# AssafSinger94/dino-tracker

Hardware: NVIDIA H100
Metric: query-points/sec (854x476, T=50) (higher is better)
Workload: dtype f32

## Files before the change

dino_tracker_b200/_lib.py:

```python
import ctypes
import os
import struct
import warnings
from ctypes import POINTER, Structure, c_char_p, c_float, c_int, c_size_t, c_ulonglong, c_void_p

import torch

from . import build as _build

_LIB = None


class Geom(Structure):
    _fields_ = [("H", c_int), ("W", c_int), ("patch", c_int), ("stride", c_int), ("radius", c_int),
                ("h", c_int), ("w", c_int)]


class HeadWeights(Structure):
    _fields_ = [("w1", c_float * 9 * 16), ("b1", c_float * 16), ("w2", c_float * 9 * 16), ("b2", c_float)]


class Features(Structure):
    _fields_ = [("tpc", c_void_p), ("norms", c_void_p), ("hi", c_void_p), ("lo", c_void_p), ("T", c_int), ("C", c_int),
                ("q8", c_void_p), ("q_fac", c_void_p), ("q_rho", c_void_p), ("hilo", c_void_p)]


class VitConfig(Structure):
    _fields_ = [("depth", c_int), ("dim", c_int), ("heads", c_int), ("tap_layer", c_int), ("patch", c_int), ("stride", c_int),
                ("attn_materialized", c_int), ("gemm_f16", c_int), ("gemm_pair", c_int), ("swiglu_hidden", c_int),
                ("facet", c_int)]


class VitWeights(Structure):
    _fields_ = [("patch_w", c_void_p), ("patch_b", c_void_p), ("cls_pos", c_void_p), ("pos", c_void_p),
                ("blocks", POINTER(c_void_p))]


class FlowVideo(Structure):
    _fields_ = [("fwd", c_void_p), ("bwd", c_void_p), ("T", c_int), ("H", c_int), ("W", c_int)]


RAFT_NCONV = 45


class RaftWeights(Structure):
    _fields_ = [("w_hi", c_void_p * RAFT_NCONV), ("w_lo", c_void_p * RAFT_NCONV), ("bias", c_void_p * RAFT_NCONV),
                ("scale", c_float * RAFT_NCONV)]


class DinotrkError(RuntimeError):
    pass


_P = c_void_p
SIGNATURES = {
    "dinotrk_version": (c_int, []),
    "dinotrk_last_error": (c_char_p, []),
    "dinotrk_launch_count": (c_ulonglong, []),
    "dinotrk_make_geom": (c_int, [c_int, c_int, c_int, c_int, c_int, POINTER(Geom)]),
    "dinotrk_pack_features": (c_int, [_P, _P, _P, c_int, c_int, c_int, _P]),
    "dinotrk_unpack_features": (c_int, [_P, _P, c_int, c_int, c_int, _P]),
    "dinotrk_token_norms": (c_int, [_P, _P, c_int, c_int, c_int, _P]),
    "dinotrk_sample_descriptors": (c_int, [_P, c_int, c_int, POINTER(Geom), _P, c_int, _P, c_int, c_int, _P, _P, _P]),
    "dinotrk_split_fp16": (c_int, [_P, _P, _P, c_size_t, _P]),
    "dinotrk_split_hilo": (c_int, [_P, _P, c_size_t, c_int, _P]),
    "dinotrk_quantise_s8": (c_int, [_P, _P, c_size_t, c_int, c_int, _P, _P, _P, _P, _P]),
    "dinotrk_split_range": (c_int, [_P, c_size_t, _P, c_size_t, _P, _P]),
    "dinotrk_split_faithful": (c_int, [c_float, c_float, c_int]),
    "dinotrk_corr_track_workspace_bytes": (c_size_t, [c_int, c_int, c_int, POINTER(Geom)]),
    "dinotrk_corr_track": (c_int, [POINTER(Features), POINTER(Geom), POINTER(HeadWeights), _P, _P, _P, _P, _P, _P,
                                   c_int, c_int, c_int, _P, _P, c_int, c_int, _P, c_size_t, _P]),
    "dinotrk_corr_maps_workspace_bytes": (c_size_t, [c_int, c_int, c_int]),
    "dinotrk_map_stride": (c_int, [POINTER(Geom)]),
    "dinotrk_corr_maps": (c_int, [POINTER(Features), POINTER(Geom), _P, _P, _P, _P, _P, _P, c_int, c_int, c_int,
                                  _P, _P, c_size_t, _P]),
    "dinotrk_head": (c_int, [_P, c_int, POINTER(Geom), POINTER(HeadWeights), _P, _P, c_int, c_int, _P, _P, _P]),
    "dinotrk_sample_backward": (c_int, [c_int, c_int, POINTER(Geom), _P, c_int, _P, c_int, c_int, _P, _P, _P]),
    "dinotrk_track_backward_workspace_bytes": (c_size_t, [c_int, c_int, POINTER(Geom)]),
    "dinotrk_track_backward": (c_int, [POINTER(Features), POINTER(Geom), POINTER(HeadWeights), _P, _P, c_int, _P, _P, _P, _P, _P,
                                       _P, c_int, _P, _P, _P, c_size_t, _P]),
    "dinotrk_infer_workspace_bytes": (c_size_t, [c_int, c_int, POINTER(Geom), c_int, c_int]),
    "dinotrk_infer_set_overlap": (c_int, [c_int]),
    "dinotrk_infer_set_path": (c_int, [c_int]),
    "dinotrk_xw_head_set_window_only": (c_int, [c_int]),
    "dinotrk_infer_set_coarse": (c_int, [c_int]),
    "dinotrk_infer_last_stats": (c_int, [POINTER(ctypes.c_longlong), c_int]),
    "dinotrk_infer_max_chunks": (c_size_t, [c_int, c_int, c_int]),
    "dinotrk_xw_coarse_keys_workspace_bytes": (c_size_t, [c_int, c_int, POINTER(Geom)]),
    "dinotrk_xw_coarse_keys": (c_int, [POINTER(Features), POINTER(Geom), _P, c_int, _P, _P, _P, _P, c_int, _P, _P, _P, c_size_t,
                                       _P]),
    "dinotrk_xw_coarse_keys_i8": (c_int, [POINTER(Features), POINTER(Geom), _P, _P, _P, c_int, _P, _P, _P, c_int, _P, _P, _P, _P,
                                          c_size_t, _P]),
    "dinotrk_xw_box_gemm": (c_int, [POINTER(Features), POINTER(Geom), _P, _P, c_int, _P, _P, _P, _P, c_int, c_int, _P, _P]),
    "dinotrk_infer_plan": (c_int, [c_int, c_int, c_int, _P, c_int, _P, _P, c_int, _P]),
    "dinotrk_infer_anchor_gcap": (c_int, [c_int, c_int]),
    "dinotrk_infer_plan_anchors": (c_int, [c_int, c_int, _P, _P, _P, c_int, c_int, _P, _P, c_int, _P]),
    "dinotrk_infer": (c_int, [POINTER(Features), POINTER(Geom), POINTER(HeadWeights), _P, c_int, c_float, c_float,
                              c_int, c_int, c_int, c_int, _P, _P, _P, _P, _P, c_size_t, _P]),
    "dinotrk_traj_cos_sims": (c_int, [_P, c_int, c_int, POINTER(Geom), _P, _P, c_int, _P, _P, c_size_t, _P]),
    "dinotrk_delta_workspace_bytes": (c_size_t, [c_int, c_int, c_int, POINTER(c_int)]),
    "dinotrk_delta_refine": (c_int, [_P, c_int, c_int, c_int, POINTER(c_int), POINTER(c_void_p), POINTER(c_void_p), _P,
                                     _P, _P, c_int, c_int, _P, _P, _P, c_size_t, _P]),
    "dinotrk_vit_workspace_bytes": (c_size_t, [POINTER(VitConfig), POINTER(Geom), c_int]),
    "dinotrk_vit_attention": (c_int, [_P, _P, _P, c_int, c_int, c_int, c_int, _P, _P]),
    "dinotrk_vit_attention_f16": (c_int, [_P, _P, _P, c_int, c_int, c_int, c_int, _P, _P]),
    "dinotrk_vit_stage": (c_int, [c_int, POINTER(VitConfig), POINTER(Geom), c_int, _P, _P, _P, _P, _P, _P, _P, _P, c_size_t,
                                  _P]),
    "dinotrk_vit_forward": (c_int, [_P, c_int, POINTER(Geom), POINTER(VitConfig), POINTER(VitWeights), _P, _P, c_size_t, _P]),
    "dinotrk_best_buddies_workspace_bytes": (c_size_t, [c_int, c_int]),
    "dinotrk_best_buddies_pairs": (c_int, [POINTER(Features), POINTER(Geom), _P, _P, c_int, _P, _P, _P, c_size_t, _P]),
    "dinotrk_bb_mutual": (c_int, [_P, _P, c_int, c_int, _P, _P]),
    "dinotrk_bb_nms": (c_int, [_P, c_int, POINTER(Geom), c_float, c_float, c_int, _P, _P, _P]),
    "dinotrk_profile_classes": (c_int, []),
    "dinotrk_profile_class_name": (c_char_p, [c_int]),
    "dinotrk_profile_enable": (None, [c_int]),
    "dinotrk_profile_collect": (c_int, [POINTER(ctypes.c_double), POINTER(c_ulonglong), c_int]),
    "dinotrk_delta_refine_allgather": (c_int, [_P, c_int, c_int, c_int, POINTER(c_int), POINTER(c_void_p), POINTER(c_void_p), _P,
                                               _P, _P, c_int, c_int, _P, _P, _P, c_size_t, POINTER(c_void_p), c_int, c_size_t, _P]),
    "dinotrk_delta_refine_tc": (c_int, [_P, c_int, c_int, c_int, POINTER(c_int), POINTER(c_void_p), POINTER(c_void_p),
                                        POINTER(c_void_p), _P, _P, _P, c_int, c_int, _P, _P, _P, c_size_t, POINTER(c_void_p),
                                        c_int, c_size_t, _P]),
    "dinotrk_delta_train_saved_bytes": (c_size_t, [c_int, c_int, c_int, POINTER(c_int)]),
    "dinotrk_delta_train_forward_workspace_bytes": (c_size_t, [c_int, c_int, c_int, POINTER(c_int)]),
    "dinotrk_delta_train_backward_workspace_bytes": (c_size_t, [c_int, c_int, c_int, POINTER(c_int)]),
    "dinotrk_delta_train_forward": (c_int, [_P, c_int, c_int, c_int, POINTER(c_int), POINTER(c_void_p), POINTER(c_void_p),
                                            POINTER(c_void_p), POINTER(c_void_p), POINTER(c_void_p), POINTER(c_void_p),
                                            POINTER(c_void_p), c_int, c_float, c_float, _P, _P, c_int, c_int, _P, _P, c_size_t,
                                            _P, c_size_t, _P]),
    "dinotrk_delta_train_backward": (c_int, [_P, c_int, c_int, c_int, POINTER(c_int), POINTER(c_void_p), POINTER(c_void_p),
                                             POINTER(c_void_p), POINTER(c_void_p), c_int, _P, _P, c_int, c_int, _P, _P, c_size_t,
                                             POINTER(c_void_p), POINTER(c_void_p), POINTER(c_void_p), POINTER(c_void_p), _P,
                                             c_size_t, _P]),
    "dinotrk_peer_alloc": (c_int, [c_size_t, POINTER(c_void_p), ctypes.c_char_p]),
    "dinotrk_peer_open": (c_int, [ctypes.c_char_p, POINTER(c_void_p)]),
    "dinotrk_peer_close": (c_int, [_P]),
    "dinotrk_peer_free": (c_int, [_P]),
    "dinotrk_occlusion": (c_int, [_P, _P, _P, c_int, c_int, c_float, c_float, _P, _P]),
    "dinotrk_flow_masks": (c_int, [POINTER(FlowVideo), c_float, _P, _P]),
    "dinotrk_traj_workspace_bytes": (c_size_t, [c_int, c_int, c_int]),
    "dinotrk_traj_chain": (c_int, [POINTER(FlowVideo), _P, c_int, c_float, c_int, _P, _P, c_float, _P, _P, c_size_t, _P]),
    "dinotrk_traj_emit": (c_int, [POINTER(FlowVideo), c_int, _P, _P, c_size_t, _P]),
    "dinotrk_traj_nearest_workspace_bytes": (c_size_t, [c_int, c_int, c_int, c_int]),
    "dinotrk_traj_nearest": (c_int, [_P, c_int, c_int, c_int, c_int, c_float, c_float, _P, _P, c_size_t, _P]),
    "dinotrk_of_filter": (c_int, [_P, c_int, c_int, _P, c_int, c_int, c_int, _P, _P, _P, _P, _P, c_int, c_int, _P, _P]),
    "dinotrk_pca_workspace_bytes": (c_size_t, [ctypes.c_longlong, c_int, c_int]),
    "dinotrk_pca_stats": (c_int, [_P, ctypes.c_longlong, c_int, c_int, _P, _P, _P, c_size_t, _P]),
    "dinotrk_pca_power": (c_int, [_P, ctypes.c_longlong, c_int, c_int, _P, _P, _P, _P, _P, _P, c_size_t, _P]),
    "dinotrk_fg_mask": (c_int, [_P, c_int, c_int, c_int, c_int, c_int, _P, _P, c_float, c_int, c_int, _P, _P, _P, _P, c_size_t,
                                _P]),
    "dinotrk_mask_upsample": (c_int, [_P, c_int, c_int, c_int, c_int, c_int, _P, _P]),
    "dinotrk_traj_split_workspace_bytes": (c_size_t, [c_int]),
    "dinotrk_traj_split_count": (c_int, [_P, c_int, c_int, _P, c_int, c_int, c_int, POINTER(c_int), _P, c_size_t, _P]),
    "dinotrk_traj_split_emit": (c_int, [_P, c_int, c_int, _P, _P, _P, c_size_t, _P]),
    "dinotrk_bb_contrastive_cos_stride": (c_int, [c_int]),
    "dinotrk_bb_contrastive_forward_workspace_bytes": (c_size_t, [c_int, c_int, c_int, c_int, c_int]),
    "dinotrk_bb_contrastive_forward": (c_int, [_P, c_int, c_int, c_int, _P, _P, c_int, _P, _P, _P, _P, c_int, c_float, _P, _P,
                                               _P, c_size_t, _P]),
    "dinotrk_bb_contrastive_backward_workspace_bytes": (c_size_t, [c_int, c_int, c_int, c_int, _P, _P, _P, _P, c_int]),
    "dinotrk_bb_contrastive_backward": (c_int, [_P, c_int, c_int, c_int, _P, _P, c_int, _P, _P, _P, _P, c_int, c_float, _P, _P,
                                                _P, _P, _P, _P, _P, _P, _P, _P, c_size_t, _P]),
    "dinotrk_sampler_workspace_bytes": (c_size_t, [c_int]),
    "dinotrk_sampler_prepare_count": (c_int, [_P, c_int, c_int, POINTER(c_int), _P, c_size_t, _P]),
    "dinotrk_sampler_prepare_emit": (c_int, [_P, c_int, c_int, _P, _P, _P, c_size_t, _P]),
    "dinotrk_sampler_count": (c_int, [_P, c_int, c_int, _P, c_int, POINTER(c_int), _P, c_size_t, _P]),
    "dinotrk_sampler_select": (c_int, [_P, c_int, c_int, _P, c_int, _P, c_int, _P, _P, _P, c_size_t, _P]),
    "dinotrk_sampler_gather": (c_int, [_P, c_int, _P, _P, c_int, _P, _P, _P]),
    "dinotrk_randperm_prefix": (c_int, [_P, c_size_t, ctypes.c_int64, ctypes.c_int64, _P]),
    "dinotrk_cycle_mask_workspace_bytes": (c_size_t, [c_int, c_int]),
    "dinotrk_cycle_mask_scan": (c_int, [_P, c_int, c_int, _P, _P, _P, c_size_t, _P]),
    "dinotrk_cycle_select": (c_int, [_P, c_int, c_int, c_int, _P, _P, c_int, _P, _P, _P]),
    "dinotrk_cycle_unnorm": (c_int, [_P, _P, c_int, c_int, c_int, _P, _P, _P]),
    "dinotrk_cycle_keep": (c_int, [_P, _P, c_int, c_int, c_int, c_float, _P, _P, _P, _P]),
    "dinotrk_emb_reg_workspace_bytes": (c_size_t, [c_int, c_int]),
    "dinotrk_emb_reg_forward": (c_int, [_P, _P, c_int, c_int, c_int, _P, _P, _P, c_size_t, _P]),
    "dinotrk_emb_reg_backward": (c_int, [_P, _P, c_int, c_int, c_int, _P, _P, _P, _P, _P]),
    "dinotrk_raft_encode_workspace_bytes": (c_size_t, [c_int, c_int]),
    "dinotrk_raft_encode": (c_int, [_P, c_int, c_int, c_int, c_int, POINTER(RaftWeights), _P, _P, _P, c_size_t, _P]),
    "dinotrk_raft_flow_workspace_bytes": (c_size_t, [c_int, c_int, c_int]),
    "dinotrk_raft_flow": (c_int, [_P, _P, _P, _P, c_int, c_int, c_int, c_int, POINTER(c_int), c_int, c_int,
                                  POINTER(RaftWeights), _P, _P, c_size_t, _P]),
}


def lib_path():
    return _build.LIB_PATH


def load(build_if_missing=True):
    global _LIB
    if _LIB is not None:
        return _LIB
    path = lib_path()
    if not os.path.exists(path):
        if not build_if_missing:
            raise DinotrkError(f"{path} is missing: run `python -c 'import __graft_entry__ as g; g.build()'`")
        _build.build()
    lib = ctypes.CDLL(path)
    for name, (res, args) in SIGNATURES.items():
        fn = getattr(lib, name)
        fn.restype = res
        fn.argtypes = args
    if lib.dinotrk_version() < 100:
        raise DinotrkError("libdinotrk.so is older than the Python binding")
    _LIB = lib
    return lib


def check(rc, what="dinotrk"):
    if rc != 0:
        raise DinotrkError(f"{what} failed ({rc}): {load().dinotrk_last_error().decode()}")


def ptr(t):
    if t is None:
        return None
    assert t.is_cuda and t.is_contiguous(), "device pointers must come from contiguous CUDA tensors"
    return c_void_p(t.data_ptr())


def stream_ptr(device=None):
    return c_void_p(torch.cuda.current_stream(device).cuda_stream)


def on_device(fn):
    import functools

    @functools.wraps(fn)
    def wrapped(self, *a, **kw):
        with torch.cuda.device(self._dev):
            return fn(self, *a, **kw)
    return wrapped


def require_cuda(device):
    if not torch.cuda.is_available():
        raise DinotrkError("dino_tracker_b200 needs a CUDA device (sm_90a); there is no CPU fallback")
    dev = torch.device(device)
    if dev.type != "cuda":
        raise DinotrkError(f"dino_tracker_b200 runs on CUDA only, got device={device!r}")
    return dev


def make_features(tpc, norms, hi=None, lo=None, quant=None, hilo=None):
    f = Features()
    f.tpc, f.norms = tpc.data_ptr(), norms.data_ptr()
    f.hi = hi.data_ptr() if hi is not None else None
    f.lo = lo.data_ptr() if lo is not None else None
    f.T, f.C = tpc.shape[0], tpc.shape[2]
    if quant is not None:
        f.q8, f.q_fac, f.q_rho = (t.data_ptr() for t in quant)
    f.hilo = hilo.data_ptr() if hilo is not None else None
    f._keep = (tpc, norms, hi, lo, quant, hilo)
    return f


def quantise_s8(x, norms, rows_per_group, stream):
    C = x.shape[-1]
    rows = x.numel() // C
    q = torch.empty(x.shape, device=x.device, dtype=torch.int8)
    fac = torch.empty(x.shape[:-1], device=x.device, dtype=torch.float32)
    rho = torch.empty(x.shape[:-1], device=x.device, dtype=torch.float32)
    rho_max = torch.empty(-(-rows // rows_per_group), device=x.device, dtype=torch.float32)
    check(load().dinotrk_quantise_s8(ptr(x), ptr(norms), rows, C, rows_per_group, ptr(q), ptr(fac), ptr(rho), ptr(rho_max),
                                     stream), "quantise_s8")
    return q, fac, rho, rho_max


S8_MAX_C = 2048


def quantise_features(tpc, norms, stream):
    T, P, C = tpc.shape
    if C % 16 or C > S8_MAX_C:
        return None
    q, fac, _, rho_f = quantise_s8(tpc, norms, P, stream)
    return q, fac, rho_f


def split_range(tpc, norms, stream):
    lib = load()
    rng = torch.empty(2, device=tpc.device, dtype=torch.float32)
    check(lib.dinotrk_split_range(ptr(tpc), tpc.numel(), ptr(norms), norms.numel(), ptr(rng), stream), "split_range")
    max_abs, min_norm = rng.tolist()
    return max_abs, min_norm, bool(lib.dinotrk_split_faithful(max_abs, min_norm, tpc.shape[-1]))


def split_fp16(x, stream):
    hi = torch.empty(x.shape, device=x.device, dtype=torch.float16)
    lo = torch.empty(x.shape, device=x.device, dtype=torch.float16)
    check(load().dinotrk_split_fp16(ptr(x), ptr(hi), ptr(lo), x.numel(), stream), "split_fp16")
    return hi, lo


def split_hilo(x, stream):
    C = x.shape[-1]
    hilo = torch.empty(x.shape[:-1] + (64 * (-(-C // 32)),), device=x.device, dtype=torch.float16)
    check(load().dinotrk_split_hilo(ptr(x), ptr(hilo), x.numel() // C, C, stream), "split_hilo")
    return hilo


def split_features(tpc, norms, stream):
    max_abs, min_norm, ok = split_range(tpc, norms, stream)
    if not ok:
        warnings.warn(f"feature video outside the fp16 split's faithful range (max |x| = {max_abs:.3g}, smallest token "
                      f"norm = {min_norm:.3g}, C = {tpc.shape[-1]}): its contractions run on the exact-fp32 path",
                      RuntimeWarning, stacklevel=3)
        return None, None
    return split_fp16(tpc, stream)


def make_geom(H, W, patch=14, stride=7, radius=35):
    g = Geom()
    check(load().dinotrk_make_geom(H, W, patch, stride, radius, ctypes.byref(g)), "make_geom")
    return g


def profile_enable(on=True):
    load().dinotrk_profile_enable(1 if on else 0)


def profile_collect():
    lib = load()
    n = lib.dinotrk_profile_classes()
    ms = (ctypes.c_double * n)()
    cnt = (c_ulonglong * n)()
    check(lib.dinotrk_profile_collect(ms, cnt, n), "profile_collect")
    return {lib.dinotrk_profile_class_name(i).decode(): (ms[i], int(cnt[i])) for i in range(n) if cnt[i]}


def infer_stats():
    a = (ctypes.c_longlong * 10)()
    check(load().dinotrk_infer_last_stats(a, 10), "infer_last_stats")
    rho_f = struct.unpack("<f", struct.pack("<I", int(a[7])))[0]
    return {"anchor_maps": int(a[0]), "exact_window": int(a[1]), "full_map": int(a[2]), "pipeline": "exact-window" if a[3] else "full-map",
            "full_map_by_certificate": int(a[4]), "contraction": "fp16x3" if a[5] else "fp32",
            "coarse": "int8" if a[6] else "fp16", "coarse_rho_f": rho_f, "desc_in_place": int(a[8]), "desc_gathered": int(a[9])}


def launch_count():
    return int(load().dinotrk_launch_count())
```

dino_tracker_b200/csrc/inference.cu:

```cuda
#include <algorithm>
#include <vector>

#include "common.cuh"
#include "corr.cuh"
#include "head.cuh"
#include "sample.cuh"
#include "xwin.cuh"

namespace dtk {

constexpr int TC2_BM_ROWS = 256;

__global__ void sample_query_kernel(const float* __restrict__ tpc, int T, int C, int P, int h, int w, PointAffine pa,
                                    const float* __restrict__ qp, float* __restrict__ desc, float* __restrict__ dnorm) {
  int n = blockIdx.x;
  float x = __fadd_rn(__fmul_rn(pa.aw, qp[n * 3 + 0]), pa.bw);
  float y = __fadd_rn(__fmul_rn(pa.ah, qp[n * 3 + 1]), pa.bh);
  int tq = (int)qp[n * 3 + 2];
  tq = min(max(tq, 0), T - 1);
  TriCorners c = tri_setup(x, y, 0.f, 2, h, w);
  sample_point(tpc, C, P, c, tq, -1, desc + (size_t)n * C, dnorm + n);
}

__global__ void index_traj_kernel(const int* __restrict__ grp_frame, const int* __restrict__ grp_row0,
                                  const int* __restrict__ grp_map0, int n_groups, int n_maps, int T,
                                  int* __restrict__ out_index, float* __restrict__ traj) {
  int j = blockIdx.x * blockDim.x + threadIdx.x;
  if (j >= n_maps) return;
  const int lo = last_le(n_groups, j, grp_map0);
  int n = grp_row0[lo] + (j - grp_map0[lo]);
  int t = grp_frame[lo];
  out_index[j] = n * T + t;
  traj[((size_t)n * T + t) * 3 + 2] = (float)t;
}

__global__ void traj_cos_kernel(const float* __restrict__ tpc, int T, int C, int P, int h, int w, PointAffine pa,
                                const float* __restrict__ traj, const float* __restrict__ qp,
                                float* __restrict__ cos_out) {
  extern __shared__ __align__(16) float sm[];
  __shared__ float nrm[2];
  __shared__ float red[SAMPLE_THREADS / 32];
  const int n = blockIdx.y, i = blockIdx.x;
  int tq = (int)qp[n * 3 + 2];
  tq = min(max(tq, 0), T - 1);
  for (int which = 0; which < 2; ++which) {
    const float* pt = traj + ((size_t)n * T + (which == 0 ? tq : i)) * 3;
    float x = __fadd_rn(__fmul_rn(pa.aw, pt[0]), pa.bw);
    float y = __fadd_rn(__fmul_rn(pa.ah, pt[1]), pa.bh);
    TriCorners c = tri_setup(x, y, pt[2], T, h, w);
    sample_point(tpc, C, P, c, c.z0, c.z1, sm + which * C, nrm + which);
    __syncthreads();
  }
  const float nq = fmaxf(nrm[0], 1e-8f), ni = fmaxf(nrm[1], 1e-8f);
  float acc = 0.f;
  for (int c = threadIdx.x; c < C; c += SAMPLE_THREADS) acc = fmaf(__fdiv_rn(sm[c], nq), __fdiv_rn(sm[C + c], ni), acc);
  acc = warp_sum(acc);
  if ((threadIdx.x & 31) == 0) red[threadIdx.x >> 5] = acc;
  __syncthreads();
  if (threadIdx.x == 0) {
    float s = 0.f;
    for (int k = 0; k < SAMPLE_THREADS / 32; ++k) s += red[k];
    cos_out[(size_t)n * T + i] = s;
  }
}

constexpr int ANCHOR_LIST_THREADS = 256;
__global__ void __launch_bounds__(ANCHOR_LIST_THREADS)
anchor_lists_kernel(const float* __restrict__ cos_sims, int N, int T, float th, int* __restrict__ cnt,
                    int* __restrict__ qlist) {
  const int a = blockIdx.x;
  int base = 0;
  for (int n0 = 0; n0 < N; n0 += ANCHOR_LIST_THREADS) {
    const int n = n0 + threadIdx.x;
    const bool v = n < N && cos_sims[(size_t)n * T + a] >= th;
    int total;
    const int rank = block_rank<ANCHOR_LIST_THREADS>(v, &total);
    if (v) qlist[(size_t)a * N + base + rank] = n;
    base += total;
    __syncthreads();
  }
  if (threadIdx.x == 0) cnt[a] = base;
}

struct AnchorItem { int a, slot, i, n; };
__device__ __forceinline__ AnchorItem anchor_item(int j, int lo, int T, const int* __restrict__ qlist, int N,
                                                  const int* __restrict__ grp_frame, const int* __restrict__ grp_map0,
                                                  const int* __restrict__ grp_item0) {
  AnchorItem it;
  it.a = grp_frame[lo];
  const int uu = grp_item0[lo] + (j - grp_map0[lo]);
  it.slot = uu / T; it.i = uu - it.slot * T;
  it.n = qlist[(size_t)it.a * N + it.slot];
  return it;
}

struct NoAnchor {};
__device__ __forceinline__ int slot_frame(int z, int i0, int a) { return z == 0 ? a : i0 + z - 1; }
__device__ __forceinline__ int slot_frame(int z, int i0, NoAnchor) { return i0 + z - 1; }
struct SetSample { TriCorners c; int f0, f1; };
template <class Anchor>
__device__ __forceinline__ SetSample frame_set_sample(const float* __restrict__ pt, int i, int T, int frame_batch, int h, int w,
                                                      const PointAffine& pa, Anchor a) {
  const int i0 = (i / frame_batch) * frame_batch, e = min(i0 + frame_batch, T);
  float x = __fadd_rn(__fmul_rn(pa.aw, pt[0]), pa.bw);
  float y = __fadd_rn(__fmul_rn(pa.ah, pt[1]), pa.bh);
  SetSample s;
  s.c = tri_setup(x, y, (float)(i - i0 + 1), e - i0 + 1, h, w);
  s.f0 = slot_frame(s.c.z0, i0, a);
  s.f1 = s.c.z1 < 0 ? -1 : slot_frame(s.c.z1, i0, a);
  return s;
}

__global__ void sample_anchor_kernel(const float* __restrict__ tpc, int T, int C, int P, int h, int w, PointAffine pa,
                                     const float* __restrict__ traj, const int* __restrict__ qlist, int N,
                                     const int* __restrict__ grp_frame, const int* __restrict__ grp_map0,
                                     const int* __restrict__ grp_item0, int n_groups, int frame_batch,
                                     float* __restrict__ desc, float* __restrict__ dnorm, int* __restrict__ out_index,
                                     __half* __restrict__ desc_hi, __half* __restrict__ desc_lo) {
  const int j = blockIdx.x;
  const AnchorItem it = anchor_item(j, last_le(n_groups, j, grp_map0), T, qlist, N, grp_frame, grp_map0, grp_item0);
  const SetSample s = frame_set_sample(traj + ((size_t)it.n * T + it.i) * 3, it.i, T, frame_batch, h, w, pa, it.a);
  sample_point(tpc, C, P, s.c, s.f0, s.f1, desc + (size_t)j * C, dnorm + j, desc_hi ? desc_hi + (size_t)j * C : nullptr,
               desc_lo ? desc_lo + (size_t)j * C : nullptr);
  if (threadIdx.x == 0) out_index[j] = (it.n * T + it.a) * T + it.i;
}

__device__ __forceinline__ float quant_desc(const __half* hi, const __half* lo, int C, const float* norm, int8_t* q, float* fac) {
  __syncthreads();
  if (threadIdx.x >= 32) return 0.f;
  const float nrm = *norm;
  return xw_quant_row([&](int k) {
    const uint2 a = *reinterpret_cast<const uint2*>(hi + k), b = *reinterpret_cast<const uint2*>(lo + k);
    const float2 a0 = __half22float2(*reinterpret_cast<const __half2*>(&a.x)), a1 = __half22float2(*reinterpret_cast<const __half2*>(&a.y));
    const float2 b0 = __half22float2(*reinterpret_cast<const __half2*>(&b.x)), b1 = __half22float2(*reinterpret_cast<const __half2*>(&b.y));
    return make_float4(a0.x + b0.x, a0.y + b0.y, a1.x + b1.x, a1.y + b1.y);
  }, C, nrm, q, fac);
}

__global__ void sample_unique_kernel(const float* __restrict__ tpc, int T, int C, int P, int h, int w, PointAffine pa,
                                     const float* __restrict__ traj, int frame_batch, __half* __restrict__ u_hi,
                                     __half* __restrict__ u_lo, float* __restrict__ u_norm, int* __restrict__ u_flag,
                                     int8_t* __restrict__ u_q8, float* __restrict__ u_fac, float* __restrict__ u_rho) {
  const int u = blockIdx.x;
  const SetSample s = frame_set_sample(traj + (size_t)u * 3, u % T, T, frame_batch, h, w, pa, NoAnchor{});
  bool slot0 = false;
#pragma unroll
  for (int k = 0; k < 4; ++k) slot0 = slot0 || (s.c.z0 == 0 && s.c.tok[k] >= 0 && s.c.wxy[k][0] != 0.f);
  if (threadIdx.x == 0) u_flag[u] = slot0 ? 1 : 0;
  if (slot0) return;
  sample_point(tpc, C, P, s.c, s.f0, s.f1, nullptr, u_norm + u, u_hi + (size_t)u * C, u_lo + (size_t)u * C);
  if (u_q8) {
    const float r = quant_desc(u_hi + (size_t)u * C, u_lo + (size_t)u * C, C, u_norm + u, u_q8 + (size_t)u * C, u_fac + u);
    if (threadIdx.x == 0) u_rho[u] = r;
  }
}

__global__ void anchor_scalars_kernel(int T, const int* __restrict__ qlist, int N, const int* __restrict__ grp_frame,
                                      const int* __restrict__ grp_row0, const int* __restrict__ grp_map0,
                                      const int* __restrict__ grp_item0, int n_groups, int n_maps, int n_unique, int chunk_row0,
                                      const float* __restrict__ u_norm, const int* __restrict__ u_flag,
                                      const float* __restrict__ u_rho, const float* __restrict__ rho_f, float eps_slack, bool with_eps,
                                      int* __restrict__ out_index, int* __restrict__ arow, float* __restrict__ dnorm,
                                      float* __restrict__ desc_eps) {
  const int j = blockIdx.x * blockDim.x + threadIdx.x;
  if (j >= n_maps) return;
  const int lo = last_le(n_groups, j, grp_map0);
  const AnchorItem it = anchor_item(j, lo, T, qlist, N, grp_frame, grp_map0, grp_item0);
  const size_t u = (size_t)it.n * T + it.i;
  out_index[j] = (it.n * T + it.a) * T + it.i;
  const int r0 = grp_row0[lo];
  arow[j] = r0 < n_unique ? r0 + (j - grp_map0[lo]) : chunk_row0 + j;
  if (u_flag[u]) return;
  dnorm[j] = u_norm[u];
  if (with_eps) desc_eps[j] = xw_eps_s8(u_rho[u], rho_f[it.a], eps_slack);
}

__global__ void gather_anchor_kernel(const float* __restrict__ tpc, int T, int C, int P, int h, int w, PointAffine pa,
                                     const float* __restrict__ traj, const int* __restrict__ qlist, int N,
                                     const int* __restrict__ grp_frame, const int* __restrict__ grp_row0,
                                     const int* __restrict__ grp_map0, const int* __restrict__ grp_item0, int n_groups,
                                     int n_unique, int map_lo, int frame_batch, const __half* __restrict__ u_hi,
                                     const __half* __restrict__ u_lo, const int* __restrict__ u_flag,
                                     float* __restrict__ dnorm, __half* __restrict__ desc_hi,
                                     __half* __restrict__ desc_lo, const int8_t* __restrict__ u_q8,
                                     const float* __restrict__ u_fac, const float* __restrict__ rho_f, float eps_slack,
                                     int8_t* __restrict__ desc_q8, float* __restrict__ desc_fac,
                                     float* __restrict__ desc_eps) {
  const int j = map_lo + blockIdx.x;
  const int lo = last_le(n_groups, j, grp_map0);
  if (grp_row0[lo] < n_unique) return;
  const AnchorItem it = anchor_item(j, lo, T, qlist, N, grp_frame, grp_map0, grp_item0);
  const size_t u = (size_t)it.n * T + it.i;
  if (!u_flag[u]) {
    const uint4* sh = reinterpret_cast<const uint4*>(u_hi + u * C);
    const uint4* sl = reinterpret_cast<const uint4*>(u_lo + u * C);
    uint4* dh = reinterpret_cast<uint4*>(desc_hi + (size_t)j * C);
    uint4* dl = reinterpret_cast<uint4*>(desc_lo + (size_t)j * C);
    for (int k = threadIdx.x; k < C / 8; k += blockDim.x) { dh[k] = __ldg(sh + k); dl[k] = __ldg(sl + k); }
    if (desc_q8) {
      const uint4* sq = reinterpret_cast<const uint4*>(u_q8 + u * C);
      uint4* dq = reinterpret_cast<uint4*>(desc_q8 + (size_t)j * C);
      for (int k = threadIdx.x; k < C / 16; k += blockDim.x) dq[k] = __ldg(sq + k);
      if (threadIdx.x == 0) desc_fac[j] = u_fac[u];
    }
    return;
  }
  const SetSample s = frame_set_sample(traj + u * 3, it.i, T, frame_batch, h, w, pa, it.a);
  sample_point(tpc, C, P, s.c, s.f0, s.f1, nullptr, dnorm + j, desc_hi + (size_t)j * C, desc_lo + (size_t)j * C);
  if (desc_q8) {
    const float r = quant_desc(desc_hi + (size_t)j * C, desc_lo + (size_t)j * C, C, dnorm + j, desc_q8 + (size_t)j * C, desc_fac + j);
    if (threadIdx.x == 0) desc_eps[j] = xw_eps_s8(r, rho_f[it.a], eps_slack);
  }
}

constexpr int OCC_THREADS = 256;
__global__ void occlusion_kernel(const float* __restrict__ traj, const float* __restrict__ cos_sims,
                                 const float* __restrict__ anchors, int T, float anchor_th, float cos_th,
                                 uint8_t* __restrict__ occ) {
  extern __shared__ float sm[];
  float* med = sm;
  int* alist = reinterpret_cast<int*>(sm + T);
  float* ax = sm + 2 * T;
  float* ay = sm + 3 * T;
  const int lane = threadIdx.x & 31, warp = threadIdx.x >> 5, nw = OCC_THREADS / 32;
  float* col = sm + 4 * T + warp * T;
  __shared__ int M;
  __shared__ float th_s;
  const int n = blockIdx.x;
  if (threadIdx.x == 0) {
    int m = 0;
    for (int a = 0; a < T; ++a)
      if (cos_sims[(size_t)n * T + a] >= anchor_th) {
        alist[m] = a;
        ax[m] = traj[((size_t)n * T + a) * 3 + 0];
        ay[m] = traj[((size_t)n * T + a) * 3 + 1];
        ++m;
      }
    M = m;
  }
  __syncthreads();
  const int m = M, want = (m - 1) / 2;
  for (int i = warp; i < T; i += nw) {
    for (int p = lane; p < m; p += 32) {
      const float* g = anchors + (((size_t)n * T + alist[p]) * T + i) * 2;
      float dx = __fsub_rn(g[0], ax[p]), dy = __fsub_rn(g[1], ay[p]);
      col[p] = sqrtf(__fadd_rn(__fmul_rn(dx, dx), __fmul_rn(dy, dy)));
    }
    __syncwarp();
    for (int p = lane; p < m; p += 32) {
      const float dp = col[p];
      int rank = 0;
      for (int q = 0; q < m; ++q) {
        float dq = col[q];
        rank += (dq < dp) || (dq == dp && q < p);
      }
      if (rank == want) med[i] = dp;
    }
    __syncwarp();
  }
  __syncthreads();
  if (threadIdx.x == 0) {
    float th = -INFINITY;
    for (int p = 0; p < m; ++p) th = fmaxf(th, med[alist[p]]);
    th_s = th;
  }
  __syncthreads();
  for (int i = threadIdx.x; i < T; i += blockDim.x)
    occ[(size_t)n * T + i] = (m > 0 && (med[i] > th_s || cos_sims[(size_t)n * T + i] < cos_th)) ? 1 : 0;
}

struct GroupBuf {
  std::vector<int> v;
  int cap, n;
  bool overflow = false;
  explicit GroupBuf(int c) : v((size_t)5 * c), cap(c), n(0) {}
  void clear() { n = 0; }
  void push(int frame, int row0, int m, int map0, int item0) {
    if (n >= cap) { overflow = true; return; }
    v[n] = frame; v[cap + n] = row0; v[2 * cap + n] = m; v[3 * cap + n] = map0; v[4 * cap + n] = item0; ++n;
  }
};

struct ChunkMeta { int used, maxm, n_groups; bool no_thin; int n_gathered, gather_lo, gather_hi; };
constexpr int XW_INPLACE_PAD_DIV = 16;
constexpr int XW_INPLACE_MIN_ROWS = TC2_BM_ROWS - TC2_BM_ROWS / (XW_INPLACE_PAD_DIV + 1);
struct AnchorRows { const int* qlist; const unsigned char* qflag; int gather_row0, ring, ring_stride; };
static bool plan_chunks(int kind, int T, int N, const int* cnt, int ch_all, int gcap, std::vector<ChunkMeta>& metas,
                        std::vector<int>& plan_host, int align = 1, int first_cap = 0, const AnchorRows* rows = nullptr) {
  int ch = ch_all;
  metas.clear(); plan_host.clear();
  GroupBuf gb(gcap);
  int n_gathered = 0, gather_lo = 0, gather_hi = 0;
  auto commit_chunk = [&](int used) {
    bool no_thin = true;
    int maxm = 0;
    for (int k = 0; k < gb.n; ++k) {
      no_thin = no_thin && gb.v[2 * gb.cap + k] > STREAM_MAX_M;
      maxm = std::max(maxm, gb.v[2 * gb.cap + k]);
    }
    metas.push_back(ChunkMeta{used, maxm, gb.n, no_thin, n_gathered, gather_lo, gather_hi});
    plan_host.insert(plan_host.end(), gb.v.begin(), gb.v.end());
    n_gathered = gather_lo = gather_hi = 0;
  };
  auto push_span = [&](int a, int map0, int m, int item0) {
    if (!rows) { gb.push(a, map0, m, map0, item0); return; }
    const int* ql = rows->qlist + (size_t)a * N;
    const int chunk_row0 = rows->gather_row0 + (int)(metas.size() % rows->ring) * rows->ring_stride;
    const int s0 = item0 / T, s1 = (item0 + m) / T;
    int gs = -1;
    auto close_gathered = [&](int s_end) {
      if (gs < 0) return;
      const int gm = (s_end - gs) * T, gmap = map0 + (gs - s0) * T;
      gb.push(a, chunk_row0 + gmap, gm, gmap, gs * T);
      if (n_gathered == 0) gather_lo = gmap;
      n_gathered += gm; gather_hi = gmap + gm;
      gs = -1;
    };
    for (int s = s0; s < s1;) {
      const bool flagged = rows->qflag[ql[s]] != 0;
      int e = s + 1;
      while (!flagged && e < s1 && ql[e] == ql[e - 1] + 1 && !rows->qflag[ql[e]]) ++e;
      const int r = (e - s) * T, pad = (r + TC2_BM_ROWS - 1) / TC2_BM_ROWS * TC2_BM_ROWS - r;
      if (!flagged && (long long)pad * XW_INPLACE_PAD_DIV <= r) {
        close_gathered(s);
        gb.push(a, ql[s] * T, r, map0 + (s - s0) * T, s * T);
      } else if (gs < 0) {
        gs = s;
      }
      s = e;
    }
    close_gathered(s1);
  };
  if (kind == 0) {
    int t = 0, row = 0;
    while (t < T) {
      gb.clear();
      int used = 0;
      while (t < T && used < ch && gb.n < gcap) {
        int m = N - row;
        if (m > ch - used) m = ch - used;
        gb.push(t, row, m, used, 0);
        used += m; row += m;
        if (row == N) { row = 0; ++t; }
      }
      commit_chunk(used);
    }
  } else {
    int a = 0;
    long long item = 0;
    while (a < T) {
      gb.clear();
      int used = 0;
      ch = (metas.empty() && first_cap > 0 && first_cap < ch_all) ? first_cap : ch_all;
      while (a < T && used < ch && gb.n < gcap) {
        long long tot = (long long)cnt[a] * T;
        long long m = tot - item;
        if (m > ch - used) {
          m = (long long)((ch - used) / align) * align;
          if (m == 0 && used > 0) break;
          if (m == 0) m = align;
        }
        if (m > 0) {
          push_span(a, used, (int)m, (int)item);
          used += (int)m; item += m;
        }
        if (item >= tot) { item = 0; ++a; }
      }
      if (used == 0) break;
      commit_chunk(used);
    }
  }
  return !gb.overflow;
}

struct CellPlan {
  std::vector<int> v;
  std::vector<size_t> first;
  std::vector<int> tiles;
  int max_m = 0;
};
static void plan_cells(int T, int gcap, const std::vector<ChunkMeta>& metas, const std::vector<int>& plan_host, CellPlan& cp) {
  const int nb = (T + XW_MAX_CELL - 1) / XW_MAX_CELL, rb = (T + nb - 1) / nb;
  cp.v.clear(); cp.first.assign(1, 0); cp.tiles.clear(); cp.max_m = 0;
  std::vector<int> r0, mm, fr, gr, ar;
  for (size_t k = 0; k < metas.size(); ++k) {
    const int* gb = plan_host.data() + k * 5 * gcap;
    r0.clear(); mm.clear(); fr.clear(); gr.clear(); ar.clear();
    int pre = 0;
    for (int g = 0; g < metas[k].n_groups; ++g) {
      const int frame = gb[g], row0 = gb[gcap + g], m = gb[2 * gcap + g], map0 = gb[3 * gcap + g];
      cp.tiles.push_back(pre);
      pre += (m + TC2_BM_ROWS - 1) / TC2_BM_ROWS;
      for (int s0 = 0; s0 < m; s0 += T)
        for (int b = 0; b < T; b += rb) {
          const int cm = std::min(rb, T - b);
          r0.push_back(map0 + s0 + b); mm.push_back(cm); fr.push_back(frame); gr.push_back(g); ar.push_back(row0 + s0 + b);
          cp.max_m = std::max(cp.max_m, cm);
        }
    }
    for (int g = metas[k].n_groups; g <= gcap; ++g) cp.tiles.push_back(pre);
    const size_t n = r0.size();
    cp.v.insert(cp.v.end(), r0.begin(), r0.end());
    cp.v.insert(cp.v.end(), mm.begin(), mm.end());
    cp.v.insert(cp.v.end(), fr.begin(), fr.end());
    cp.v.insert(cp.v.end(), gr.begin(), gr.end());
    cp.v.insert(cp.v.end(), ar.begin(), ar.end());
    cp.first.push_back(cp.first.back() + n);
  }
}

struct InferAsync {
  cudaStream_t side;
  cudaEvent_t fork, join, sample[2], gemm[2];
};
static int g_overlap_mode = -1;
struct InferAsyncSlot { InferAsync ia; int state; };
static InferAsync* infer_async() {
  static PerDev<InferAsyncSlot> slots;
  if (g_overlap_mode == 0) return nullptr;
  InferAsyncSlot& slot = slots.get();
  InferAsync& ia = slot.ia;
  if (slot.state == 0) {
    slot.state = -1;
    if (cudaStreamCreateWithFlags(&ia.side, cudaStreamNonBlocking) != cudaSuccess) return nullptr;
    cudaEvent_t* evs[] = {&ia.fork, &ia.join, &ia.sample[0], &ia.sample[1], &ia.gemm[0], &ia.gemm[1]};
    for (cudaEvent_t* ev : evs)
      if (cudaEventCreateWithFlags(ev, cudaEventDisableTiming) != cudaSuccess) return nullptr;
    slot.state = 1;
  }
  return slot.state == 1 ? &ia : nullptr;
}

constexpr int XW_RING = 4;
constexpr int XW_PROBE_MAPS = 4096;
constexpr int INFER_A_COUNTED = 16;
constexpr int XW_CNT_A = 2 * XW_RING, XW_CNT_MINNORM = XW_CNT_A + INFER_A_COUNTED;
struct XwAsync {
  int state;
  cudaEvent_t sample[XW_RING], done[XW_RING], freed[XW_RING];
  int* host_cnt;
};
static XwAsync* xw_async() {
  static PerDev<XwAsync> slots;
  XwAsync& xa = slots.get();
  if (xa.state == 0) {
    xa.state = -1;
    for (int k = 0; k < XW_RING; ++k) {
      if (cudaEventCreateWithFlags(&xa.sample[k], cudaEventDisableTiming) != cudaSuccess) return nullptr;
      if (cudaEventCreateWithFlags(&xa.done[k], cudaEventDisableTiming) != cudaSuccess) return nullptr;
      if (cudaEventCreateWithFlags(&xa.freed[k], cudaEventDisableTiming) != cudaSuccess) return nullptr;
    }
    if (cudaHostAlloc(&xa.host_cnt, (XW_CNT_MINNORM + 4) * sizeof(int), cudaHostAllocDefault) != cudaSuccess) return nullptr;
    xa.state = 1;
  }
  return xa.state == 1 ? &xa : nullptr;
}
static int g_xw_path = -1;
static int g_xw_coarse = -1;
namespace infer_stat {
enum { anchor_maps, exact_window, full_map, pipeline, full_map_by_certificate, contraction, coarse, coarse_rho_f,
       desc_in_place, desc_gathered, count };
}
static long long g_infer_stats[infer_stat::count] = {};
constexpr int XW_S8_PROBE_QUEUE_DIV = 16;

struct AnchorChoice {
  XwAsync* xa = nullptr;
  bool xw = false;
  bool probe = false;
  bool s8 = false;

  AnchorChoice(const FeatView& fv, const dinotrk_geom& g) {
    if (fv.tensor() && disc_fits_box(g) && g_xw_path != 0) xa = xw_async();
    xw = xa != nullptr;
    probe = g_xw_path < 0;
  }
  static bool q8_rows(const FeatView& fv) { return fv.s8() && g_xw_coarse != 0 && fv.C % 16 == 0 && fv.C <= XW_S8_MAX_C; }
  void after_sync(int C, int n_counted_A, long long maps_A) {
    if (!xw) return;
    float mn;
    memcpy(&mn, xa->host_cnt + XW_CNT_MINNORM, sizeof(float));
    if (!(mn >= split_min_norm(C))) xw = false;
    if (xw && probe && n_counted_A > 0) {
      long long unc = 0;
      for (int k = 0; k < n_counted_A; ++k) unc += xa->host_cnt[XW_CNT_A + k];
      if (unc * 4 > maps_A) xw = false;
    }
  }
  int coarse_pass(const FeatView& fv, float rho_max) {
    DTK_CHECK_ARG(g_xw_coarse != 1 || !xw || fv.s8(), "infer: int8 coarse pass forced without the int8 features");
    s8 = xw && fv.s8() && g_xw_coarse != 0;
    DTK_CHECK_ARG(!s8 || (fv.C % 16 == 0 && fv.C <= XW_S8_MAX_C), "infer: int8 coarse pass needs C %% 16 == 0 and C <= %d",
                  XW_S8_MAX_C);
    if (g_xw_coarse < 0 && !(rho_max <= XW_S8_RHO_MAX)) s8 = false;
    return DINOTRK_OK;
  }
  bool probe_says_full_maps(long long by_certificate, long long queued, int maps) {
    if (by_certificate * 4 > maps) return true;
    if (s8 && g_xw_coarse < 0 && queued * XW_S8_PROBE_QUEUE_DIV > maps) s8 = false;
    return false;
  }
};

struct CorrTrackWs {
  float* maps; CorrMapsWs corr; int* hscratch;
  CorrTrackWs(Arena& ar, int total_maps, int n_groups, int C, int map_stride)
      : maps(ar.take<float>((size_t)total_maps * map_stride)), corr(ar, total_maps, n_groups, C),
        hscratch(ar.take<int>(total_maps + 1)) {}
};

struct ChunkBufs {
  float* maps; float* desc; float* norm; int* plan; float* split; int* hscratch; unsigned long long* tkeys;
  ChunkBufs() = default;
  ChunkBufs(Arena& ar, int C, int N, int P, int ms, int ch, int gcap) {
    maps = ar.take<float>((size_t)ch * ms);
    desc = ar.take<float>((size_t)ch * C);
    norm = ar.take<float>(ch);
    plan = ar.take<int>(gcap + 1);
    split = ar.take<float>(corr_tc_workspace_bytes(ch > N ? ch : N, C) / 4);
    hscratch = ar.take<int>(ch + 1);
    tkeys = ar.take<unsigned long long>((size_t)ch * cdiv(P, CORR_TILE));
  }
};

struct XwSet {
  int row0; float* norm; int* out_index; int* arow; float* eps; XwChunk xc;
  XwSet() = default;
  XwSet(Arena& ar, int row0_, float* u_norm, int P, int ch, int gcap) : row0(row0_), norm(u_norm + row0_) {
    out_index = ar.take<int>(ch);
    arow = ar.take<int>(ch);
    eps = ar.take<float>(ch);
    xc = XwChunk(ar, ch, (size_t)ch + 2, cdiv(P, XW_TILE), gcap);
  }
};

struct InferWs {
  float* descA; float* normA;
  ChunkBufs cb[2];
  int* out_index_ring[4];
  int* d_groups; int* d_cnt; int* d_qlist;
  size_t xw_rows;
  __half* u_hi; __half* u_lo; int8_t* u_q8; float* u_norm; float* u_fac; int* u_flag; float* u_rho;
  float* d_rnorms; unsigned* d_minnorm;
  XwSet xr[XW_RING];
  int cell_nb;
  int* d_cells; int* d_tiles;
  int sg_cap;
  int* d_cgrp; int* d_splan; int* d_cntA;
  InferWs(Arena& ar, int T, int C, int N, int P, int ms, int ch, int gcap, size_t max_chunks) {
    descA = ar.take<float>((size_t)N * C);
    normA = ar.take<float>(N);
    for (ChunkBufs& b : cb) b = ChunkBufs(ar, C, N, P, ms, ch, gcap);
    for (int*& r : out_index_ring) r = ar.take<int>(ch);
    d_groups = ar.take<int>(max_chunks * 5 * gcap);
    d_cnt = ar.take<int>(T);
    d_qlist = ar.take<int>((size_t)T * N);
    const int n_unique = N * T;
    xw_rows = (size_t)n_unique + (size_t)XW_RING * ch;
    u_hi = ar.take<__half>(xw_rows * C);
    u_lo = ar.take<__half>(xw_rows * C);
    u_q8 = ar.take<int8_t>(xw_rows * C);
    u_norm = ar.take<float>(xw_rows);
    u_fac = ar.take<float>(xw_rows);
    u_flag = ar.take<int>((size_t)N * T);
    u_rho = ar.take<float>((size_t)N * T);
    d_rnorms = ar.take<float>((size_t)T * P);
    d_minnorm = ar.take<unsigned>(4);
    for (int k = 0; k < XW_RING; ++k) xr[k] = XwSet(ar, n_unique + k * ch, u_norm, P, ch, gcap);
    cell_nb = (T + XW_MAX_CELL - 1) / XW_MAX_CELL;
    d_cells = ar.take<int>((size_t)N * T * cell_nb * 5 + 16);
    d_tiles = ar.take<int>(max_chunks * (gcap + 1));
    sg_cap = (int)std::min<size_t>(max_chunks * (size_t)gcap, 16384);
    d_cgrp = ar.take<int>((size_t)4 * sg_cap);
    d_splan = ar.take<int>((size_t)sg_cap + 1);
    d_cntA = ar.take<int>(64);
  }
};

struct InferCtx {
  const FeatView& fv; const dinotrk_geom& g; const dinotrk_head_weights& hw;
  InferWs& ws; cudaStream_t st;
  int T, C, N, P, ms, ch, gcap, fb;
  size_t max_chunks;
  PointAffine pa;
  std::vector<ChunkMeta> metas;
  std::vector<int> plan_host;
  int upload_plan() {
    DTK_CHECK_ARG(metas.size() <= max_chunks, "infer: chunk plan exceeds its bound (%zu > %zu)", metas.size(), max_chunks);
    if (!plan_host.empty())
      DTK_CUDA(cudaMemcpyAsync(ws.d_groups, plan_host.data(), plan_host.size() * sizeof(int), cudaMemcpyHostToDevice, st));
    return DINOTRK_OK;
  }
  struct Grp { const int *f, *r, *m, *map0, *item; };
  Grp grp_of(size_t k) const {
    const int* b = ws.d_groups + k * 5 * gcap;
    return Grp{b, b + gcap, b + 2 * gcap, b + 3 * gcap, b + 4 * gcap};
  }
};

static int infer_trajectories(InferCtx& c, const float* query_points, float* traj, int& n_counted) {
  NvtxRange nv("dinotrk.infer.A.trajectories");
  InferWs& ws = c.ws;
  const bool tensor = c.fv.tensor();
  {
    ProfRange pr(PROF_SAMPLE, c.st);
    sample_query_kernel<<<c.N, SAMPLE_THREADS, 0, c.st>>>(c.fv.tpc, c.T, c.C, c.P, c.g.h, c.g.w, c.pa, query_points, ws.descA,
                                                           ws.normA);
    DTK_LAUNCHED();
  }
  if (tensor) {
    for (int k = 0; k < 2; ++k) {
      const DescSplit a(ws.cb[k].split, c.N, c.C);
      int rc = corr_hilo(c.fv) ? launch_split_hilo(ws.descA, a.hi, c.N, c.C, c.st)
                               : launch_split_f16(ws.descA, a.hi, a.lo, (size_t)c.N * c.C, c.st);
      if (rc) return rc;
    }
  }
  plan_chunks(0, c.T, c.N, nullptr, c.ch, c.gcap, c.metas, c.plan_host);
  int rc = c.upload_plan();
  if (rc) return rc;
  for (size_t k = 0; k < c.metas.size(); ++k) {
    const ChunkMeta& cm = c.metas[k];
    const ChunkBufs& b = ws.cb[k & 1];
    const InferCtx::Grp gp = c.grp_of(k);
    {
      ProfRange pr(PROF_MISC, c.st);
      index_traj_kernel<<<cdiv(cm.used, 256), 256, 0, c.st>>>(gp.f, gp.r, gp.map0, cm.n_groups, cm.used, c.T,
                                                              ws.out_index_ring[k & 3], traj);
      DTK_LAUNCHED();
    }
    CorrAssist as;
    as.tkeys = tensor ? b.tkeys : nullptr; as.zero_word = b.hscratch; as.split_ready = tensor; as.no_thin = cm.no_thin;
    rc = launch_corr_maps(c.fv, ws.descA, c.N, ws.normA, gp.f, gp.r, gp.m, gp.map0, cm.n_groups, cm.used, cm.maxm, b.maps, c.ms,
                          b.plan, b.split, c.st, as);
    if (rc) return rc;
    rc = launch_head(b.maps, cm.used, c.ms, c.g, c.hw, ws.out_index_ring[k & 3], traj, 3, 0, nullptr, b.hscratch, c.st, as.tkeys,
                     true);
    if (rc) return rc;
    if (k < INFER_A_COUNTED)
      DTK_CUDA(cudaMemcpyAsync(ws.d_cntA + k, b.hscratch, sizeof(int), cudaMemcpyDeviceToDevice, c.st));
  }
  n_counted = (int)std::min<size_t>(c.metas.size(), INFER_A_COUNTED);
  return DINOTRK_OK;
}

struct ExactWindow {
  InferCtx& c;
  const AnchorChoice& choice;
  const CellPlan& cp;
  bool ovl;
  cudaStream_t sb;
  const float* traj;
  float* anchors;
  int q_rows = 0, q_groups = 0;

  XwCells cells_of(size_t k) const {
    XwCells x;
    const int n = (int)(cp.first[k + 1] - cp.first[k]);
    const int* base = c.ws.d_cells + 5 * cp.first[k];
    x.row0 = base; x.m = base + n; x.frame = base + 2 * n; x.group = base + 3 * n; x.arow = base + 4 * n;
    x.n_cells = n; x.max_m = cp.max_m;
    return x;
  }
  int sample(size_t k) {
    InferWs& ws = c.ws;
    const ChunkMeta& cm = c.metas[k];
    const XwSet& x = ws.xr[k % XW_RING];
    const InferCtx::Grp gp = c.grp_of(k);
    if (ovl && k >= XW_RING) DTK_CUDA(cudaStreamWaitEvent(sb, choice.xa->freed[k % XW_RING], 0));
    {
      ProfRange pr(PROF_SAMPLE, sb);
      anchor_scalars_kernel<<<cdiv(cm.used, 256), 256, 0, sb>>>(c.T, ws.d_qlist, c.N, gp.f, gp.r, gp.map0, gp.item, cm.n_groups,
                                                               cm.used, c.N * c.T, x.row0, ws.u_norm, ws.u_flag, ws.u_rho,
                                                               c.fv.q_rho, xw_s8_slack(c.C), choice.s8, x.out_index, x.arow,
                                                               x.norm, x.eps);
      DTK_LAUNCHED();
      if (cm.n_gathered > 0) {
        const size_t r0 = (size_t)x.row0;
        gather_anchor_kernel<<<cm.gather_hi - cm.gather_lo, SAMPLE_THREADS, 0, sb>>>(
            c.fv.tpc, c.T, c.C, c.P, c.g.h, c.g.w, c.pa, traj, ws.d_qlist, c.N, gp.f, gp.r, gp.map0, gp.item, cm.n_groups,
            c.N * c.T, cm.gather_lo, c.fb, ws.u_hi, ws.u_lo, ws.u_flag, x.norm, ws.u_hi + r0 * c.C, ws.u_lo + r0 * c.C, ws.u_q8,
            ws.u_fac, c.fv.q_rho, xw_s8_slack(c.C), choice.s8 ? ws.u_q8 + r0 * c.C : nullptr, ws.u_fac + r0, x.eps);
        DTK_LAUNCHED();
      }
    }
    if (ovl) DTK_CUDA(cudaEventRecord(choice.xa->sample[k % XW_RING], sb));
    return DINOTRK_OK;
  }
  int flush() {
    if (q_rows == 0) return DINOTRK_OK;
    const ChunkBufs& b = c.ws.cb[0];
    CorrAssist as;
    as.tkeys = b.tkeys; as.zero_word = b.hscratch; as.split_ready = true; as.no_thin = true; as.all_wide = true; as.small_tiles = true;
    const int* cg = c.ws.d_cgrp;
    const int sg = c.ws.sg_cap;
    int rc = launch_corr_maps(c.fv, nullptr, c.ch, b.norm, cg, cg + sg, cg + 2 * sg, cg + 3 * sg, q_groups, q_rows, q_rows,
                              b.maps, c.ms, c.ws.d_splan, b.split, c.st, as);
    if (rc) return rc;
    rc = launch_head(b.maps, q_rows, c.ms, c.g, c.hw, c.ws.out_index_ring[0], anchors, 2, 0, nullptr, b.hscratch, c.st, b.tkeys,
                     true);
    q_rows = q_groups = 0;
    return rc;
  }
  int finish(size_t j) {
    InferWs& ws = c.ws;
    XwAsync* xa = choice.xa;
    DTK_CUDA(cudaEventSynchronize(xa->done[j % XW_RING]));
    const int n_slow = xa->host_cnt[2 * (j % XW_RING)];
    g_infer_stats[infer_stat::full_map_by_certificate] += xa->host_cnt[2 * (j % XW_RING) + 1];
    const ChunkMeta& cm = c.metas[j];
    const XwSet& x = ws.xr[j % XW_RING];
    const InferCtx::Grp gp = c.grp_of(j);
    DTK_CHECK_ARG(n_slow >= 0 && n_slow <= cm.used, "infer: corrupt full-map queue (%d of %d)", n_slow, cm.used);
    g_infer_stats[infer_stat::exact_window] += cm.used - n_slow; g_infer_stats[infer_stat::full_map] += n_slow;
    if (n_slow > 0) {
      if (q_rows + n_slow > c.ch || q_groups + cm.n_groups > ws.sg_cap) {
        int rc = flush();
        if (rc) return rc;
      }
      const ChunkBufs& b = ws.cb[0];
      const DescSplit d(b.split, c.ch, c.C);
      int rc = launch_xw_compact(nullptr, ws.u_hi, ws.u_lo, x.arow, x.norm, x.out_index, c.C, gp.f, gp.map0, cm.n_groups, n_slow,
                                 x.xc, nullptr, d.hi, d.lo, b.norm, ws.out_index_ring[0], ws.d_cgrp, ws.sg_cap, c.st, q_rows,
                                 q_groups, corr_hilo(c.fv));
      if (rc) return rc;
      q_rows += n_slow; q_groups += cm.n_groups;
    }
    DTK_CUDA(cudaEventRecord(xa->freed[j % XW_RING], c.st));
    return DINOTRK_OK;
  }
};

static int anchors_exact_window(InferCtx& c, AnchorChoice& choice, const float* traj, float* anchors, size_t& done) {
  InferWs& ws = c.ws;
  const cudaStream_t st = c.st;
  XwAsync* xa = choice.xa;
  CellPlan cp;
  plan_cells(c.T, c.gcap, c.metas, c.plan_host, cp);
  DTK_CHECK_ARG(cp.first.back() * 5 <= (size_t)c.N * c.T * ws.cell_nb * 5 + 16, "infer: cell plan exceeds its bound");
  if (!cp.v.empty()) DTK_CUDA(cudaMemcpyAsync(ws.d_cells, cp.v.data(), cp.v.size() * sizeof(int), cudaMemcpyHostToDevice, st));
  if (!cp.tiles.empty()) DTK_CUDA(cudaMemcpyAsync(ws.d_tiles, cp.tiles.data(), cp.tiles.size() * sizeof(int), cudaMemcpyHostToDevice, st));
  InferAsync* ia = infer_async();
  const bool ovl = ia != nullptr && c.metas.size() > 1;
  ExactWindow pipe{c, choice, cp, ovl, ovl ? ia->side : st, traj, anchors};
  if (ovl) {
    DTK_CUDA(cudaEventRecord(ia->fork, st));
    DTK_CUDA(cudaStreamWaitEvent(pipe.sb, ia->fork, 0));
  }
  int rc;
  if (!c.metas.empty() && (rc = pipe.sample(0))) return rc;
  size_t n_finished = 0;
  done = c.metas.size();
  for (size_t k = 0; k < c.metas.size(); ++k) {
    const ChunkMeta& cm = c.metas[k];
    const XwSet& x = ws.xr[k % XW_RING];
    const InferCtx::Grp gp = c.grp_of(k);
    const XwCells cells = pipe.cells_of(k);
    if (ovl) DTK_CUDA(cudaStreamWaitEvent(st, xa->sample[k % XW_RING], 0));
    const float* eps = choice.s8 ? x.eps : nullptr;
    g_infer_stats[infer_stat::desc_in_place] += cm.used - cm.n_gathered; g_infer_stats[infer_stat::desc_gathered] += cm.n_gathered;
    if ((rc = launch_xw_coarse(c.fv, ws.u_hi, (int)ws.xw_rows, ws.u_norm, gp.f, gp.r, gp.m, gp.map0, ws.d_tiles + k * (c.gcap + 1),
                               cm.n_groups, cm.used / TC2_BM_ROWS + cm.n_groups, x.xc, st, ws.d_rnorms,
                               choice.s8 ? ws.u_q8 : nullptr, ws.u_fac))) return rc;
    if ((rc = launch_xw_plan(cells, x.norm, cm.n_groups, c.g, x.xc, st, cm.used, split_min_norm(c.C), eps))) return rc;
    if ((rc = launch_xw_gemm(c.fv, c.g, ws.u_hi, ws.u_lo, (int)ws.xw_rows, cells, x.xc, st))) return rc;
    if ((rc = launch_xw_head(c.fv, c.g, c.hw, cells, x.norm, gp.map0, cm.used, x.out_index, anchors, 2, 0, x.xc, st, cm.n_groups,
                             eps)))
      return rc;
    DTK_CUDA(cudaMemcpyAsync(xa->host_cnt + 2 * (k % XW_RING), x.xc.slow_cnt + cm.n_groups, 2 * sizeof(int), cudaMemcpyDeviceToHost, st));
    DTK_CUDA(cudaEventRecord(xa->done[k % XW_RING], st));
    if (k == 0 && choice.probe && c.metas.size() > 1) {
      if ((rc = pipe.finish(0))) return rc;
      n_finished = 1;
      if (choice.probe_says_full_maps(g_infer_stats[infer_stat::full_map_by_certificate], g_infer_stats[infer_stat::full_map], cm.used)) {
        done = 1;
        break;
      }
      g_infer_stats[infer_stat::coarse] = choice.s8 ? 1 : 0;
    }
    if (k + 1 < c.metas.size() && (rc = pipe.sample(k + 1))) return rc;
    while (n_finished + 2 <= k)
      if ((rc = pipe.finish(n_finished++))) return rc;
  }
  while (n_finished < done)
    if ((rc = pipe.finish(n_finished++))) return rc;
  if ((rc = pipe.flush())) return rc;
  if (ovl) {
    DTK_CUDA(cudaEventRecord(ia->join, pipe.sb));
    DTK_CUDA(cudaStreamWaitEvent(st, ia->join, 0));
  }
  return DINOTRK_OK;
}

static int anchors_full_map(InferCtx& c, size_t k0, const float* traj, float* anchors) {
  InferWs& ws = c.ws;
  const cudaStream_t st = c.st;
  const bool tensor = c.fv.tensor();
  FeatView fv_split = c.fv;
  fv_split.hilo = nullptr;
  InferAsync* ia = infer_async();
  const bool ovl = ia != nullptr && c.metas.size() > k0 + 1;
  const cudaStream_t sb = ovl ? ia->side : st;
  if (ovl) {
    DTK_CUDA(cudaEventRecord(ia->fork, st));
    DTK_CUDA(cudaStreamWaitEvent(sb, ia->fork, 0));
  }
  auto sample = [&](size_t k) -> int {
    const ChunkMeta& cm = c.metas[k];
    const ChunkBufs& b = ws.cb[k & 1];
    const InferCtx::Grp gp = c.grp_of(k);
    if (ovl && k >= k0 + 2) DTK_CUDA(cudaStreamWaitEvent(sb, ia->gemm[k & 1], 0));
    {
      ProfRange pr(PROF_SAMPLE, sb);
      const DescSplit d(b.split, cm.used, c.C);
      __half* d_hi = tensor ? reinterpret_cast<__half*>(d.hi) : nullptr;
      __half* d_lo = tensor ? reinterpret_cast<__half*>(d.lo) : nullptr;
      sample_anchor_kernel<<<cm.used, SAMPLE_THREADS, 0, sb>>>(c.fv.tpc, c.T, c.C, c.P, c.g.h, c.g.w, c.pa, traj, ws.d_qlist, c.N,
                                                              gp.f, gp.map0, gp.item, cm.n_groups, c.fb, b.desc, b.norm,
                                                              ws.out_index_ring[k & 3], d_hi, d_lo);
      DTK_LAUNCHED();
    }
    if (ovl) DTK_CUDA(cudaEventRecord(ia->sample[k & 1], sb));
    return DINOTRK_OK;
  };
  auto head_full = [&](size_t j) {
    const ChunkBufs& b = ws.cb[j & 1];
    return launch_head(b.maps, c.metas[j].used, c.ms, c.g, c.hw, ws.out_index_ring[j & 3], anchors, 2, 0, nullptr, b.hscratch,
                       st, tensor ? b.tkeys : nullptr, true, 2);
  };
  int rc;
  if (k0 < c.metas.size() && (rc = sample(k0))) return rc;
  for (size_t k = k0; k < c.metas.size(); ++k) {
    const ChunkMeta& cm = c.metas[k];
    const ChunkBufs& b = ws.cb[k & 1];
    const InferCtx::Grp gp = c.grp_of(k);
    if (ovl) DTK_CUDA(cudaStreamWaitEvent(st, ia->sample[k & 1], 0));
    if (k >= k0 + 2 && (rc = head_full(k - 2))) return rc;
    CorrAssist as;
    as.tkeys = tensor ? b.tkeys : nullptr; as.zero_word = b.hscratch; as.split_ready = tensor; as.no_thin = cm.no_thin;
    rc = launch_corr_maps(fv_split, b.desc, cm.used, b.norm, gp.f, gp.r, gp.m, gp.map0, cm.n_groups, cm.used, cm.maxm, b.maps,
                          c.ms, b.plan, b.split, st, as);
    if (rc) return rc;
    if (ovl) DTK_CUDA(cudaEventRecord(ia->gemm[k & 1], st));
    if (k + 1 < c.metas.size() && (rc = sample(k + 1))) return rc;
    rc = launch_head(b.maps, cm.used, c.ms, c.g, c.hw, ws.out_index_ring[k & 3], anchors, 2, 0, nullptr, b.hscratch, st, as.tkeys,
                     true, 1);
    if (rc) return rc;
  }
  for (size_t j = std::max(k0, c.metas.size() >= 2 ? c.metas.size() - 2 : 0); j < c.metas.size(); ++j)
    if ((rc = head_full(j))) return rc;
  return DINOTRK_OK;
}

static int infer_anchors(InferCtx& c, const float* traj, const float* cos_sims, float anchor_th, float* anchors, int n_counted_A) {
  NvtxRange nv("dinotrk.infer.C.anchors");
  InferWs& ws = c.ws;
  const cudaStream_t st = c.st;
  const int T = c.T, N = c.N;
  {
    ProfRange pr(PROF_ANCHOR_LIST, st);
    anchor_lists_kernel<<<T, ANCHOR_LIST_THREADS, 0, st>>>(cos_sims, N, T, anchor_th, ws.d_cnt, ws.d_qlist);
    DTK_LAUNCHED();
  }
  AnchorChoice choice(c.fv, c.g);
  XwAsync* xa = choice.xa;
  if (xa) {
    int rc = launch_xw_rnorms(c.fv, ws.d_rnorms, ws.d_minnorm, st);
    if (rc) return rc;
    DTK_CUDA(cudaMemcpyAsync(xa->host_cnt + XW_CNT_MINNORM, ws.d_minnorm, sizeof(unsigned), cudaMemcpyDeviceToHost, st));
    if (n_counted_A > 0)
      DTK_CUDA(cudaMemcpyAsync(xa->host_cnt + XW_CNT_A, ws.d_cntA, (size_t)n_counted_A * sizeof(int), cudaMemcpyDeviceToHost, st));
  }
  std::vector<int> cnt(T);
  DTK_CUDA(cudaMemcpyAsync(cnt.data(), ws.d_cnt, (size_t)T * sizeof(int), cudaMemcpyDeviceToHost, st));
  std::vector<float> rho_f(c.fv.s8() ? T : 0);
  if (c.fv.s8()) DTK_CUDA(cudaMemcpyAsync(rho_f.data(), c.fv.q_rho, (size_t)T * sizeof(float), cudaMemcpyDeviceToHost, st));
  std::vector<int> qlist_h, uflag_h;
  if (choice.xw) {
    {
      ProfRange pr(PROF_SAMPLE, st);
      sample_unique_kernel<<<N * T, SAMPLE_THREADS, 0, st>>>(c.fv.tpc, T, c.C, c.P, c.g.h, c.g.w, c.pa, traj, c.fb, ws.u_hi, ws.u_lo,
                                                             ws.u_norm, ws.u_flag, AnchorChoice::q8_rows(c.fv) ? ws.u_q8 : nullptr,
                                                             ws.u_fac, ws.u_rho);
      DTK_LAUNCHED();
    }
    qlist_h.resize((size_t)T * N); uflag_h.resize((size_t)N * T);
    DTK_CUDA(cudaMemcpyAsync(qlist_h.data(), ws.d_qlist, qlist_h.size() * sizeof(int), cudaMemcpyDeviceToHost, st));
    DTK_CUDA(cudaMemcpyAsync(uflag_h.data(), ws.u_flag, uflag_h.size() * sizeof(int), cudaMemcpyDeviceToHost, st));
  }
  DTK_CUDA(cudaStreamSynchronize(st));
  choice.after_sync(c.C, n_counted_A, (long long)N * T);
  long long maps_C = 0;
  for (int a = 0; a < T; ++a) maps_C += (long long)cnt[a] * T;
  long long* stats = g_infer_stats;
  stats[infer_stat::anchor_maps] = maps_C; stats[infer_stat::exact_window] = 0; stats[infer_stat::full_map] = 0;
  stats[infer_stat::pipeline] = choice.xw ? 1 : 0; stats[infer_stat::full_map_by_certificate] = 0;
  stats[infer_stat::contraction] = c.fv.tensor() ? 1 : 0; stats[infer_stat::desc_in_place] = 0; stats[infer_stat::desc_gathered] = 0;
  float rho_max = 0.f;
  for (float r : rho_f) rho_max = std::max(rho_max, r);
  int rc = choice.coarse_pass(c.fv, rho_max);
  if (rc) return rc;
  unsigned bits;
  memcpy(&bits, &rho_max, sizeof(bits));
  stats[infer_stat::coarse] = choice.s8 ? 1 : 0; stats[infer_stat::coarse_rho_f] = bits;
  const int probe_cap = choice.probe ? std::max(T, (XW_PROBE_MAPS / T) * T) : 0;
  size_t k0 = 0;
  if (choice.xw) {
    std::vector<unsigned char> qflag(N, 0);
    for (size_t u = 0; u < uflag_h.size(); ++u)
      if (uflag_h[u]) qflag[u / T] = 1;
    const AnchorRows rows{qlist_h.data(), qflag.data(), N * T, XW_RING, c.ch};
    DTK_CHECK_ARG(plan_chunks(1, T, N, cnt.data(), c.ch, c.gcap, c.metas, c.plan_host, T, probe_cap, &rows),
                  "infer: a chunk of the anchor phase has more than %d groups", c.gcap);
    if ((rc = c.upload_plan())) return rc;
    if ((rc = anchors_exact_window(c, choice, traj, anchors, k0))) return rc;
    if (k0 == c.metas.size()) return DINOTRK_OK;
    stats[infer_stat::pipeline] = 0; stats[infer_stat::coarse] = 0;
    plan_chunks(1, T, N, cnt.data(), c.ch, c.gcap, c.metas, c.plan_host, T, probe_cap);
  } else {
    plan_chunks(1, T, N, cnt.data(), c.ch, c.gcap, c.metas, c.plan_host);
  }
  if ((rc = c.upload_plan())) return rc;
  return anchors_full_map(c, k0, traj, anchors);
}

}

using namespace dtk;

extern "C" {

int dinotrk_infer_set_path(int path) {
  DTK_CHECK_ARG(path >= -1 && path <= 1, "infer_set_path: -1 (automatic), 0 (full-map GEMM + head) or 1 (coarse pass + exact window)");
  g_xw_path = path;
  return DINOTRK_OK;
}

int dinotrk_infer_set_coarse(int mode) {
  DTK_CHECK_ARG(mode >= -1 && mode <= 1, "infer_set_coarse: -1 (automatic), 0 (fp16) or 1 (int8)");
  g_xw_coarse = mode;
  return DINOTRK_OK;
}

int dinotrk_infer_last_stats(long long* out, int n) {
  DTK_CHECK_ARG(out && n >= 4, "infer_last_stats: need at least 4 slots");
  for (int i = 0; i < (n < infer_stat::count ? n : infer_stat::count); ++i) out[i] = g_infer_stats[i];
  return DINOTRK_OK;
}

static int infer_chunk_maps(int chunk_maps) { return chunk_maps > 0 ? chunk_maps : 4096; }
static int infer_chunk_eff(int chunk_maps, int T) { const int c = infer_chunk_maps(chunk_maps); return c > T ? c : T; }
static int infer_gcap(int T, int ch) { return T + 2 + 2 * (ch / XW_INPLACE_MIN_ROWS + 1); }
static size_t infer_max_chunks(int T, int N, size_t ch) {
  size_t cap = (ch / (size_t)T) * (size_t)T;
  if (cap < (size_t)T) cap = T;
  return ((size_t)N * T * T + cap - 1) / cap + 2;
}

size_t dinotrk_infer_max_chunks(int T, int N, int chunk_maps) {
  const size_t ch = (size_t)infer_chunk_maps(chunk_maps);
  return ((size_t)N * T * T + ch - 1) / ch + 2;
}

int dinotrk_infer_plan(int kind, int T, int N, const int* anchor_counts, int chunk_maps, int* groups, int* meta,
                       int max_chunks, int* n_chunks) {
  DTK_CHECK_ARG((kind == 0 || kind == 1) && T > 0 && N >= 0 && n_chunks, "infer_plan: bad arguments");
  DTK_CHECK_ARG(kind == 0 || anchor_counts, "infer_plan: kind 1 needs the per-frame anchor counts");
  const int ch = infer_chunk_maps(chunk_maps), gcap = T + 2;
  std::vector<ChunkMeta> metas;
  std::vector<int> plan_host;
  plan_chunks(kind, T, N, anchor_counts, ch, gcap, metas, plan_host);
  *n_chunks = (int)metas.size();
  DTK_CHECK_ARG((int)metas.size() <= max_chunks || (!groups && !meta), "infer_plan: %zu chunks, room for %d", metas.size(), max_chunks);
  if (groups) std::copy(plan_host.begin(), plan_host.end(), groups);
  if (meta)
    for (size_t k = 0; k < metas.size(); ++k) {
      meta[4 * k] = metas[k].used; meta[4 * k + 1] = metas[k].maxm; meta[4 * k + 2] = metas[k].n_groups;
      meta[4 * k + 3] = metas[k].no_thin ? 1 : 0;
    }
  return DINOTRK_OK;
}

int dinotrk_infer_anchor_gcap(int T, int chunk_maps) { return T > 0 ? infer_gcap(T, infer_chunk_eff(chunk_maps, T)) : 0; }

int dinotrk_infer_plan_anchors(int T, int N, const int* anchor_counts, const int* qlist, const unsigned char* query_flag,
                               int chunk_maps, int probe, int* groups, int* meta, int max_chunks, int* n_chunks) {
  DTK_CHECK_ARG(T > 0 && N >= 0 && anchor_counts && qlist && query_flag && n_chunks, "infer_plan_anchors: bad arguments");
  for (int a = 0; a < T; ++a) {
    DTK_CHECK_ARG(anchor_counts[a] >= 0 && anchor_counts[a] <= N, "infer_plan_anchors: count of frame %d out of range", a);
    for (int k = 0; k < anchor_counts[a]; ++k)
      DTK_CHECK_ARG(qlist[(size_t)a * N + k] >= 0 && qlist[(size_t)a * N + k] < N, "infer_plan_anchors: query out of range");
  }
  const int ch = infer_chunk_eff(chunk_maps, T), gcap = infer_gcap(T, ch);
  const AnchorRows rows{qlist, query_flag, N * T, XW_RING, ch};
  std::vector<ChunkMeta> metas;
  std::vector<int> plan_host;
  const bool fits = plan_chunks(1, T, N, anchor_counts, ch, gcap, metas, plan_host, T,
                                probe ? std::max(T, (XW_PROBE_MAPS / T) * T) : 0, &rows);
  DTK_CHECK_ARG(fits, "infer_plan_anchors: a chunk has more than %d groups", gcap);
  *n_chunks = (int)metas.size();
  DTK_CHECK_ARG((int)metas.size() <= max_chunks || (!groups && !meta), "infer_plan_anchors: %zu chunks, room for %d", metas.size(), max_chunks);
  if (groups) std::copy(plan_host.begin(), plan_host.end(), groups);
  if (meta)
    for (size_t k = 0; k < metas.size(); ++k) {
      meta[5 * k] = metas[k].used; meta[5 * k + 1] = metas[k].maxm; meta[5 * k + 2] = metas[k].n_groups;
      meta[5 * k + 3] = metas[k].no_thin ? 1 : 0; meta[5 * k + 4] = metas[k].n_gathered;
    }
  return DINOTRK_OK;
}

int dinotrk_infer_set_overlap(int mode) {
  DTK_CHECK_ARG(mode >= -1 && mode <= 1, "infer_set_overlap: mode must be -1 (default), 0 or 1");
  g_overlap_mode = mode;
  return DINOTRK_OK;
}

size_t dinotrk_corr_track_workspace_bytes(int total_maps, int n_groups, int C, const dinotrk_geom* g) {
  if (!g) return 0;
  return align_up(layout_end<CorrTrackWs>(total_maps, n_groups, C, dinotrk_map_stride(g)), 256) + 1024;
}

int dinotrk_corr_track(const dinotrk_features* feat, const dinotrk_geom* g,
                       const dinotrk_head_weights* hw, const float* desc, const float* desc_norm,
                       const int* grp_frame, const int* grp_row0, const int* grp_m, const int* grp_map0,
                       int n_groups, int total_maps, int max_group_m, const int* out_index, float* out,
                       int out_stride, int out_mode, void* workspace, size_t workspace_bytes, void* stream) {
  DTK_CHECK_ARG(feat && feat->tpc && feat->norms && g && hw && desc && desc_norm && grp_frame && grp_row0 && grp_m &&
                grp_map0 && out, "corr_track: null pointer");
  const int C = feat->C;
  DTK_CHECK_ARG(feat->T > 0 && C > 0 && C % 4 == 0 && n_groups >= 0 && total_maps >= 0, "corr_track: bad sizes");
  DTK_CHECK_ARG((feat->hi == nullptr) == (feat->lo == nullptr), "corr_track: hi and lo must be given together");
  DTK_CHECK_ARG(workspace && workspace_bytes >= dinotrk_corr_track_workspace_bytes(total_maps, n_groups, C, g),
                "corr_track: workspace too small");
  if (total_maps == 0) return DINOTRK_OK;
  const int ms = dinotrk_map_stride(g);
  Arena ar(workspace);
  const CorrTrackWs ws(ar, total_maps, n_groups, C, ms);
  cudaStream_t st = (cudaStream_t)stream;
  int rc = launch_corr_maps(make_view(*feat, *g), desc, total_maps, desc_norm, grp_frame, grp_row0, grp_m, grp_map0,
                            n_groups, total_maps, max_group_m, ws.maps, ms, ws.corr.plan, ws.corr.split, st);
  if (rc) return rc;
  return launch_head(ws.maps, total_maps, ms, *g, *hw, out_index, out, out_stride, out_mode, nullptr, ws.hscratch, st);
}


size_t dinotrk_infer_workspace_bytes(int T, int C, const dinotrk_geom* g, int N, int chunk_maps) {
  if (!g) return 0;
  const int ch = infer_chunk_eff(chunk_maps, T);
  const size_t end = layout_end<InferWs>(T, C, N, g->h * g->w, dinotrk_map_stride(g), ch, infer_gcap(T, ch),
                                         infer_max_chunks(T, N, (size_t)ch));
  return align_up(end, 256) + 25088;
}

int dinotrk_traj_cos_sims(const float* tpc, int T, int C, const dinotrk_geom* g, const float* traj,
                          const float* query_points, int N, float* cos_sims, void* workspace,
                          size_t workspace_bytes, void* stream) {
  (void)workspace; (void)workspace_bytes;
  DTK_CHECK_ARG(tpc && g && traj && query_points && cos_sims, "traj_cos_sims: null pointer");
  DTK_CHECK_ARG(T > 0 && C > 0 && C % 4 == 0 && N >= 0, "traj_cos_sims: bad sizes");
  if (N == 0) return DINOTRK_OK;
  size_t smem = (size_t)2 * C * sizeof(float);
  static PerDev<size_t> attr_dev;
  size_t& attr = attr_dev.get();
  if (smem > 48 * 1024 && smem > attr) {
    DTK_CUDA(cudaFuncSetAttribute(traj_cos_kernel, cudaFuncAttributeMaxDynamicSharedMemorySize, (int)smem));
    attr = smem;
  }
  ProfRange pr(PROF_COS, (cudaStream_t)stream);
  traj_cos_kernel<<<dim3(T, N), SAMPLE_THREADS, smem, (cudaStream_t)stream>>>(
      tpc, T, C, g->h * g->w, g->h, g->w, make_point_affine(*g), traj, query_points, cos_sims);
  DTK_LAUNCHED();
  return DINOTRK_OK;
}

int dinotrk_occlusion(const float* traj, const float* cos_sims, const float* anchors, int N, int T,
                      float anchor_th, float cos_th, uint8_t* occ, void* stream) {
  DTK_CHECK_ARG(traj && cos_sims && anchors && occ && N >= 0 && T > 0, "occlusion: bad args");
  if (N == 0) return DINOTRK_OK;
  size_t smem = (size_t)(4 + OCC_THREADS / 32) * T * sizeof(float);
  DTK_CHECK_ARG(smem <= 200 * 1024, "occlusion: T=%d too large", T);
  static PerDev<size_t> attr_dev;
  size_t& attr = attr_dev.get();
  if (smem > 48 * 1024 && smem > attr) {
    DTK_CUDA(cudaFuncSetAttribute(occlusion_kernel, cudaFuncAttributeMaxDynamicSharedMemorySize, (int)smem));
    attr = smem;
  }
  ProfRange pr(PROF_OCCLUSION, (cudaStream_t)stream);
  occlusion_kernel<<<N, OCC_THREADS, smem, (cudaStream_t)stream>>>(traj, cos_sims, anchors, T, anchor_th, cos_th, occ);
  DTK_LAUNCHED();
  return DINOTRK_OK;
}

int dinotrk_infer(const dinotrk_features* feat, const dinotrk_geom* g,
                  const dinotrk_head_weights* hw, const float* query_points, int N, float anchor_th, float cos_th,
                  int frame_batch, int start_phase, int stop_after, int chunk_maps, float* traj, float* cos_sims,
                  float* anchors,
                  uint8_t* occ, void* workspace, size_t workspace_bytes, void* stream) {
  DTK_CHECK_ARG(feat && feat->tpc && feat->norms && g && hw && query_points && traj, "infer: null pointer");
  const int T = feat->T, C = feat->C;
  DTK_CHECK_ARG(T > 0 && C > 0 && C % 4 == 0 && N >= 0, "infer: bad sizes");
  DTK_CHECK_GRID(*g, "infer");
  DTK_CHECK_ARG((feat->hi == nullptr) == (feat->lo == nullptr), "infer: hi and lo must be given together");
  const FeatView fv = make_view(*feat, *g);
  DTK_CHECK_ARG(start_phase >= 0 && start_phase <= stop_after && stop_after <= 3,
                "infer: need 0 <= start_phase <= stop_after <= 3");
  DTK_CHECK_ARG((stop_after < 1 || cos_sims) && (stop_after < 2 || anchors) && (stop_after < 3 || occ),
                "infer: missing output buffer for the requested phases");
  DTK_CHECK_ARG(workspace && workspace_bytes >= dinotrk_infer_workspace_bytes(T, C, g, N, chunk_maps),
                "infer: workspace too small (%zu < %zu)", workspace_bytes,
                dinotrk_infer_workspace_bytes(T, C, g, N, chunk_maps));
  if (N == 0) return DINOTRK_OK;
  const int P = g->h * g->w, ms = dinotrk_map_stride(g);
  const int ch = infer_chunk_eff(chunk_maps, T);
  const int fb = frame_batch > 0 ? (frame_batch < T ? frame_batch : T) : T;
  const int gcap = infer_gcap(T, ch);
  const size_t max_chunks = infer_max_chunks(T, N, (size_t)ch);
  Arena ar(workspace);
  InferWs ws(ar, T, C, N, P, ms, ch, gcap, max_chunks);
  DTK_CHECK_ARG(ws.xw_rows <= 0x7fffffffu, "infer: %zu descriptor rows exceed the row index", ws.xw_rows);
  InferCtx c{fv, *g, *hw, ws, (cudaStream_t)stream, T, C, N, P, ms, ch, gcap, fb, max_chunks, make_point_affine(*g)};

  int rc, n_counted_A = 0;
  if (start_phase <= 0 && (rc = infer_trajectories(c, query_points, traj, n_counted_A))) return rc;
  if (stop_after < 1) return DINOTRK_OK;
  if (start_phase <= 1) {
    NvtxRange nv("dinotrk.infer.B.cos_sims");
    if ((rc = dinotrk_traj_cos_sims(feat->tpc, T, C, g, traj, query_points, N, cos_sims, nullptr, 0, stream))) return rc;
  }
  if (stop_after < 2) return DINOTRK_OK;
  if (start_phase <= 2 && (rc = infer_anchors(c, traj, cos_sims, anchor_th, anchors, n_counted_A))) return rc;
  if (stop_after < 3) return DINOTRK_OK;
  NvtxRange nv("dinotrk.infer.D.occlusion");
  return dinotrk_occlusion(traj, cos_sims, anchors, N, T, anchor_th, cos_th, occ, stream);
}

}
```

dino_tracker_b200/csrc/xwin.cu:

```cuda
#include <cuda_fp16.h>

#include "common.cuh"
#include "corr.cuh"
#include "head.cuh"
#include "tcgemm.cuh"
#include "xwin.cuh"

namespace dtk {

constexpr int XW_GEMM_BN = 2 * XW_TILE;

template <class Acc>
struct CoarseEpi {
  static constexpr bool kFragment = true;
  static constexpr bool kS8 = std::is_same<Acc, int>::value;
  const float* rnorms;
  const float* desc_norm;
  const int* grp_map0;
  unsigned long long* key1;
  float* max2;
  int n_tiles, P;

  struct Pre { float2 col; float dv; int map0; };
  __device__ __forceinline__ Pre begin(const TcTile& tl, int t, int r) const {
    const float* rn = rnorms + (size_t)tl.batch * P;
    const int c0 = tl.n0 + t, c1 = c0 + XW_TILE;
    const int rr = r + 8 * ((threadIdx.x & 3) >> 1);
    Pre p;
    p.col = make_float2(c0 < P ? __ldg(rn + c0) : 0.f, c1 < P ? __ldg(rn + c1) : 0.f);
    p.dv = rr < tl.m ? __ldg(desc_norm + tl.row0 + rr) : 0.f;
    p.map0 = __ldg(grp_map0 + tl.g);
    return p;
  }
  static __device__ __forceinline__ float as_float(Acc a) {
    if constexpr (kS8) return __int_as_float(a); else return a;
  }
  static __device__ __forceinline__ Acc from_float(float v) {
    if constexpr (kS8) return __float_as_int(v); else return v;
  }
  template <bool EDGE>
  __device__ __forceinline__ void fold_max(float (&m1)[2], int kh, const float* cols, int n0, int fc,
                                           Acc (&acc)[XW_GEMM_BN / 2]) const {
#pragma unroll
    for (int ii = 0; ii < XW_TILE / 8; ++ii) {
      const int i = kh * XW_TILE / 8 + ii;
      const float2 rnv = tc::lds_f2(tc::smem_u32(cols + fc + 8 * i));
      const int col = n0 + 8 * i + fc;
      const bool ok0 = !EDGE || col < P, ok1 = !EDGE || col + 1 < P;
#pragma unroll
      for (int h = 0; h < 2; ++h) {
        const float a = ok0 ? (float)acc[4 * i + 2 * h] * rnv.x : -INFINITY;
        const float b = ok1 ? (float)acc[4 * i + 2 * h + 1] * rnv.y : -INFINITY;
        acc[4 * i + 2 * h] = from_float(a);
        acc[4 * i + 2 * h + 1] = from_float(b);
        m1[h] = fmaxf(m1[h], fmaxf(a, b));
      }
    }
  }
  __device__ __forceinline__ void scan(float m1, int h, int kh, const Acc (&acc)[XW_GEMM_BN / 2], float& pos,
                                       float& m2) const {
    pos = 0.f;
    m2 = -INFINITY;
#pragma unroll
    for (int ii = XW_TILE / 8 - 1; ii >= 0; --ii) {
      const int i = kh * XW_TILE / 8 + ii;
#pragma unroll
      for (int j = 1; j >= 0; --j)
        asm("{\n\t.reg .pred p;\n\t"
            "setp.eq.f32 p, %2, %3;\n\t"
            "@p fma.rn.f32 %0, %0, 0f3B000000, %4;\n\t"
            "@!p max.f32 %1, %1, %2;\n\t}"
            : "+f"(pos), "+f"(m2)
            : "f"(as_float(acc[4 * i + 2 * h + j])), "f"(m1), "f"((float)(8 * i + j + 1)));
    }
  }
  __device__ __forceinline__ void fragment(const TcTile& tl, int r, int fc, Acc (&acc)[XW_GEMM_BN / 2], const float* cols,
                                           const Pre& pre) const {
    const int q = threadIdx.x & 3, n0 = tl.n0;
    const bool edge = n0 + XW_GEMM_BN > P;
    float o1, o2;
    int otok;
#pragma unroll
    for (int kh = 0; kh < 2; ++kh) {
      float m1[2] = {-INFINITY, -INFINITY};
      if (edge) fold_max<true>(m1, kh, cols, n0, fc, acc);
      else fold_max<false>(m1, kh, cols, n0, fc, acc);
#pragma unroll
      for (int h = 0; h < 2; ++h) {
#pragma unroll
        for (int sh = 1; sh <= 2; sh <<= 1) m1[h] = fmaxf(m1[h], __shfl_xor_sync(0xffffffffu, m1[h], sh));
        float pos, m2;
        scan(m1[h], h, kh, acc, pos, m2);
        const int ip = (int)pos;
        int tok = ip ? n0 + fc + ip - 1 : 0x7fffffff;
        int cnt = (ip != 0) + ((float)ip != pos);
#pragma unroll
        for (int sh = 1; sh <= 2; sh <<= 1) {
          tok = min(tok, __shfl_xor_sync(0xffffffffu, tok, sh));
          cnt += __shfl_xor_sync(0xffffffffu, cnt, sh);
          m2 = fmaxf(m2, __shfl_xor_sync(0xffffffffu, m2, sh));
        }
        if ((q & 1) == kh && (q >> 1) == h) {
          o1 = m1[h];
          o2 = cnt > 1 ? m1[h] : m2;
          otok = tok;
        }
      }
    }
    const int rr = r + 8 * (q >> 1), nt = n0 / XW_TILE + (q & 1);
    if (rr >= tl.m || nt >= n_tiles) return;
    const float rdn = kS8 ? pre.dv : __fdividef(1.f, fmaxf(pre.dv, XW_MIN_NORM));
    const size_t off = (size_t)(pre.map0 + rr) * n_tiles + nt;
    key1[off] = ((unsigned long long)__float_as_uint(fmaxf(o1 * rdn, 0.f)) << 32) | (unsigned)(0x7fffffff - otok);
    max2[off] = fmaxf(o2 * rdn, 0.f);
  }
};

__global__ void xw_rnorm_kernel(const float* __restrict__ norms, float* __restrict__ rnorms, size_t n, unsigned* __restrict__ min_bits) {
  float mn = INFINITY;
  for (size_t i = (size_t)blockIdx.x * blockDim.x + threadIdx.x; i < n; i += (size_t)gridDim.x * blockDim.x) {
    const float v = norms[i];
    rnorms[i] = __fdiv_rn(1.f, fmaxf(v, XW_MIN_NORM));
    mn = fminf(mn, v);
  }
#pragma unroll
  for (int o = 16; o > 0; o >>= 1) mn = fminf(mn, __shfl_xor_sync(0xffffffffu, mn, o));
  if ((threadIdx.x & 31) == 0) atomicMin(min_bits, __float_as_uint(fmaxf(mn, 0.f)));
}

int launch_xw_rnorms(const FeatView& fv, float* rnorms, unsigned* min_bits, cudaStream_t st) {
  const size_t n = (size_t)fv.T * fv.P;
  DTK_CUDA(cudaMemsetAsync(min_bits, 0x7f, sizeof(unsigned), st));
  ProfRange pr(PROF_XW_PLAN, st);
  xw_rnorm_kernel<<<num_sms() * 4, 256, 0, st>>>(fv.norms, rnorms, n, min_bits);
  DTK_LAUNCHED();
  return DINOTRK_OK;
}

int launch_xw_coarse(const FeatView& fv, const void* desc_hi, int desc_rows, const float* desc_norm, const int* grp_frame,
                     const int* grp_row0, const int* grp_m, const int* grp_map0, const int* tile_start, int n_groups,
                     int max_tiles, const XwChunk& xc, cudaStream_t st, const float* rnorms, const void* desc_q8,
                     const float* desc_fac) {
  static_assert(XW_GEMM_BN == 256 && XW_TILE == 128, "one m64n256 GEMM N tile = two 128-token key tiles (CoarseEpi::fragment)");
  TcProblem pb{grp_frame, grp_row0, grp_m, tile_start, n_groups, fv.P, fv.C};
  if (desc_q8) {
    DTK_CHECK_ARG(fv.s8() && fv.C % 16 == 0 && fv.C <= XW_S8_MAX_C, "int8 coarse pass: needs the int8 features, C %% 16 == 0 "
                  "and C <= %d", XW_S8_MAX_C);
    CoarseEpi<int> epi{fv.q_fac, desc_fac, grp_map0, xc.key1, xc.max2, cdiv(fv.P, XW_TILE), fv.P};
    return tc_launch<TcMode::S8, CoarseEpi<int>, XW_GEMM_BN, true>({desc_q8, nullptr, (uint64_t)desc_rows, 0, fv.q8, nullptr,
                                                                    (uint64_t)fv.T, 0}, pb, max_tiles, epi, st, PROF_XW_COARSE);
  }
  CoarseEpi<float> epi{rnorms, desc_norm, grp_map0, xc.key1, xc.max2, cdiv(fv.P, XW_TILE), fv.P};
  return tc_launch<TcMode::F16, CoarseEpi<float>, XW_GEMM_BN, true>({desc_hi, nullptr, (uint64_t)desc_rows, 0, fv.hi, nullptr,
                                                                     (uint64_t)fv.T, 0}, pb, max_tiles, epi, st, PROF_XW_COARSE);
}

constexpr int PLAN_WARPS = 8;
template <int KPL>
__global__ void __launch_bounds__(PLAN_WARPS * 32)
xw_cand_kernel(int n_maps, const float* __restrict__ desc_norm, float min_norm, int n_groups, int n_tiles,
               const unsigned long long* __restrict__ key1, const float* __restrict__ eps_map,
               const float* __restrict__ max2, int* __restrict__ cand, int* __restrict__ pinfo, int* __restrict__ slow_cnt) {
  const int lane = threadIdx.x & 31;
  const int gw = blockIdx.x * PLAN_WARPS + (threadIdx.x >> 5), nw = gridDim.x * PLAN_WARPS;
  if (gw == 0)
    for (int i = lane; i <= n_groups + 1; i += 32) slow_cnt[i] = 0;
  for (int map = gw; map < n_maps; map += nw) {
    const unsigned long long* k1 = key1 + (size_t)map * n_tiles;
    const float* k2 = max2 + (size_t)map * n_tiles;
    unsigned long long kk[KPL] = {};
    float v2[KPL] = {};
#pragma unroll
    for (int q = 0; q < KPL; ++q) {
      const int t = lane + 32 * q;
      if (t < n_tiles) { kk[q] = __ldg(k1 + t); v2[q] = __ldg(k2 + t); }
    }
    unsigned long long gk = kk[0];
#pragma unroll
    for (int q = 1; q < KPL; ++q) gk = gk > kk[q] ? gk : kk[q];
#pragma unroll
    for (int o = 16; o > 0; o >>= 1) { unsigned long long t = __shfl_xor_sync(0xffffffffu, gk, o); gk = t > gk ? t : gk; }
    const float gmax = __uint_as_float((unsigned)(gk >> 32));
    const int ptok = 0x7fffffff - (int)(gk & 0xffffffffu);
    const float eps = eps_map ? eps_map[map] : XW_EPS;
    const float th = gmax - 2.f * eps;
    bool amb = false;
    int ncand = 0;
#pragma unroll
    for (int q = 0; q < KPL; ++q) {
      const int t = lane + 32 * q;
      const bool in = t < n_tiles;
      const bool isc = in && __uint_as_float((unsigned)(kk[q] >> 32)) >= th;
      const unsigned cm = __ballot_sync(0xffffffffu, isc);
      amb = amb || __any_sync(0xffffffffu, in && v2[q] >= th);
      const int rank = ncand + __popc(cm & ((1u << lane) - 1u));
      if (isc && rank < XW_MAX_CAND) cand[(size_t)map * XW_MAX_CAND + rank] = 0x7fffffff - (int)(kk[q] & 0xffffffffu);
      ncand += __popc(cm);
    }
    amb = amb || ncand > XW_MAX_CAND || !(gmax > 4.f * eps) || !(desc_norm[map] >= min_norm);
    if (lane >= ncand && lane < XW_MAX_CAND) cand[(size_t)map * XW_MAX_CAND + lane] = -1;
    if (lane == 0) pinfo[map] = amb ? -1 - ptok : ptok;
  }
}

__global__ void __launch_bounds__(PLAN_WARPS * 32)
xw_cell_kernel(XwCells cells, int w, const int* __restrict__ cand, const int* __restrict__ pinfo, int* __restrict__ stat,
               int* __restrict__ cell_of, int2* __restrict__ box_org) {
  __shared__ short s_r[PLAN_WARPS][XW_MAX_CELL], s_c[PLAN_WARPS][XW_MAX_CELL];
  __shared__ unsigned char s_ok[PLAN_WARPS][XW_MAX_CELL];
  const int lane = threadIdx.x & 31, wid = threadIdx.x >> 5;
  const int gw = blockIdx.x * PLAN_WARPS + wid, nw = gridDim.x * PLAN_WARPS;
  for (int cell = gw; cell < cells.n_cells; cell += nw) {
    const int row0 = cells.row0[cell], m = cells.m[cell];
    int nv = 0;
    for (int r = lane; r < m; r += 32) {
      const int pi = __ldg(pinfo + row0 + r);
      const int ptok = pi >= 0 ? pi : -1 - pi;
      s_r[wid][r] = (short)(ptok / w);
      s_c[wid][r] = (short)(ptok - (ptok / w) * w);
      s_ok[wid][r] = pi >= 0 ? 1 : 0;
      nv += pi >= 0 ? 1 : 0;
      cell_of[row0 + r] = cell;
    }
    __syncwarp();
#pragma unroll
    for (int o = 16; o > 0; o >>= 1) nv += __shfl_xor_sync(0xffffffffu, nv, o);
    int med_r = -1, med_c = -1;
    if (nv > 0) {
      const int want = (nv - 1) / 2;
      for (int r = lane; r < m; r += 32) {
        if (!s_ok[wid][r]) continue;
        int rk_r = 0, rk_c = 0;
        const int vr = s_r[wid][r], vc = s_c[wid][r];
        for (int q = 0; q < m; ++q) {
          if (!s_ok[wid][q]) continue;
          rk_r += (s_r[wid][q] < vr) || (s_r[wid][q] == vr && q < r);
          rk_c += (s_c[wid][q] < vc) || (s_c[wid][q] == vc && q < r);
        }
        if (rk_r == want) med_r = vr;
        if (rk_c == want) med_c = vc;
      }
#pragma unroll
      for (int o = 16; o > 0; o >>= 1) {
        med_r = max(med_r, __shfl_xor_sync(0xffffffffu, med_r, o));
        med_c = max(med_c, __shfl_xor_sync(0xffffffffu, med_c, o));
      }
    }
    int n_fit = 0;
    for (int r = lane; r < m; r += 32) {
      const int map = row0 + r;
      bool fit = s_ok[wid][r] != 0;
      if (fit) {
        const int4 cd = __ldg(reinterpret_cast<const int4*>(cand) + map);
        const int ct[4] = {cd.x, cd.y, cd.z, cd.w};
#pragma unroll
        for (int q = 0; q < XW_MAX_CAND; ++q)
          if (ct[q] >= 0) {
            const int tr = ct[q] / w, tc_ = ct[q] - tr * w;
            fit = fit && abs(tr - med_r) <= XW_SLACK && abs(tc_ - med_c) <= XW_SLACK;
          }
      }
      stat[map] = fit ? 0 : 1;
      n_fit += fit ? 1 : 0;
    }
#pragma unroll
    for (int o = 16; o > 0; o >>= 1) n_fit += __shfl_xor_sync(0xffffffffu, n_fit, o);
    if (lane == 0)
      box_org[cell] = n_fit > 0 ? make_int2(med_r - XW_BOX / 2, med_c - XW_BOX / 2) : make_int2(0, INT_MIN);
    __syncwarp();
  }
}

int launch_xw_plan(const XwCells& cells, const float* desc_norm, int n_groups, const dinotrk_geom& g, const XwChunk& xc,
                   cudaStream_t st, int n_maps, float min_norm, const float* eps) {
  static_assert(XW_MAX_CAND == 4, "candidates are read as one int4");
  const int n_tiles = cdiv(g.h * g.w, XW_TILE);
  DTK_CHECK_GRID(g, "exact-window path");
  static_assert(DTK_GRID_MAX_TOKENS <= 256 * XW_TILE, "xw_cand_kernel keeps at most 8 keys per lane");
  DTK_CHECK_ARG(cells.max_m <= XW_MAX_CELL, "exact-window path: cell of %d rows", cells.max_m);
  if (cells.n_cells <= 0 || n_maps <= 0) return DINOTRK_OK;
  ProfRange pr(PROF_XW_PLAN, st);
  int grid = cdiv(n_maps, PLAN_WARPS);
  if (grid > num_sms() * 8) grid = num_sms() * 8;
  auto cand_kernel = n_tiles <= 64 ? xw_cand_kernel<2> : n_tiles <= 128 ? xw_cand_kernel<4> : xw_cand_kernel<8>;
  cand_kernel<<<grid, PLAN_WARPS * 32, 0, st>>>(n_maps, desc_norm, min_norm, n_groups, n_tiles, xc.key1, eps, xc.max2, xc.cand, xc.pinfo, xc.slow_cnt);
  DTK_LAUNCHED();
  grid = cdiv(cells.n_cells, PLAN_WARPS);
  if (grid > num_sms() * 8) grid = num_sms() * 8;
  xw_cell_kernel<<<grid, PLAN_WARPS * 32, 0, st>>>(cells, g.w, xc.cand, xc.pinfo, xc.stat, xc.cell_of, xc.box_org);
  DTK_LAUNCHED();
  return DINOTRK_OK;
}

template <int MB, bool HILO>
struct XwCfg {
  static constexpr int kBK = 32;
  static constexpr int kRow = 2 * kBK;
  static constexpr int kTokRow = HILO ? 2 * kRow : kRow;
  static constexpr int kBoxes = HILO ? 1 : 2;
  static constexpr int kDescBytes = MB * kRow;
  static constexpr int kTok0Bytes = XW_N0 * kTokRow, kTok1Bytes = XW_N1 * kTokRow;
  static constexpr int kTok0Tx = XW_ROWS0 * XW_BOX * kTokRow, kTok1Tx = XW_ROWS1 * XW_BOX * kTokRow;
  static constexpr int kTokOff = 2 * kDescBytes;
  static constexpr int kStageBytes = kTokOff + kBoxes * (MB == 64 ? kTok0Bytes + kTok1Bytes : kTok0Bytes);
  static constexpr int kStages = MB == 64 ? 3 : 4;
  static constexpr int kSmem = kStages * kStageBytes + 1024 + 256;
  static_assert(kStages * kStageBytes + 1024 + 256 <= 227 * 1024, "shared-memory ring too large");
  static_assert(kTokOff % 1024 == 0 && kTok0Bytes % 1024 == 0 && kTok1Bytes % 1024 == 0 && kStageBytes % 1024 == 0,
                "token boxes must start 1024-byte aligned");
};

template <int MB, bool HILO, int N>
__device__ __forceinline__ void xw_part(uint8_t* smem, uint64_t* full, uint64_t* empty, int& stage, int& phase, int KB,
                                        uint32_t d_off, uint32_t t_off, uint32_t t_half, float* __restrict__ xbox, int map0,
                                        int r0, int m) {
  using Cfg = XwCfg<MB, HILO>;
  constexpr int kTok = (N == XW_N0 ? XW_ROWS0 : XW_ROWS1) * XW_BOX;
  constexpr int kCol0 = N == XW_N0 ? 0 : XW_ROWS0 * XW_BOX;
  const int warp = threadIdx.x >> 5, lane = threadIdx.x & 31, t = threadIdx.x & 127;
  float acc[N / 2];
#pragma unroll
  for (int i = 0; i < N / 2; ++i) acc[i] = 0.f;
  int prev = -1;
  for (int kb = 0; kb < KB; ++kb) {
    tc::mbar_wait(&full[stage], phase);
    tc::wgmma_fence();
    const uint32_t sd = tc::smem_u32(smem + stage * Cfg::kStageBytes) + d_off;
    const uint32_t st = tc::smem_u32(smem + stage * Cfg::kStageBytes) + t_off;
#pragma unroll
    for (int ks = 0; ks < Cfg::kBK / 16; ++ks) {
      const uint32_t koff = ks * 32;
      const uint64_t d_hi = tc::smem_desc_sw64(sd + koff), d_lo = tc::smem_desc_sw64(sd + Cfg::kDescBytes + koff);
      const uint64_t t_hi = HILO ? tc::smem_desc_sw128(st + koff) : tc::smem_desc_sw64(st + koff);
      const uint64_t t_lo = HILO ? tc::smem_desc_sw128(st + Cfg::kRow + koff) : tc::smem_desc_sw64(st + t_half + koff);
      tc::wgmma_ss<false, N>(acc, d_lo, t_hi, 1u);
      tc::wgmma_ss<false, N>(acc, d_hi, t_lo, 1u);
      tc::wgmma_ss<false, N>(acc, d_hi, t_hi, 1u);
    }
    tc::wgmma_commit();
    tc::wgmma_wait<1>();
    if (prev >= 0 && t == 0) tc::mbar_arrive(&empty[prev]);
    prev = stage;
    if (++stage == Cfg::kStages) { stage = 0; phase ^= 1; }
  }
  tc::wgmma_wait<0>();
  tc::reg_fence(acc);
  if (prev >= 0 && t == 0) tc::mbar_arrive(&empty[prev]);
  const int fr = (warp & 3) * 16 + (lane >> 2), fc = 2 * (lane & 3);
#pragma unroll
  for (int h = 0; h < 2; ++h) {
    const int r = r0 + fr + 8 * h;
    if (r >= m) continue;
    float* dst = xbox + (size_t)(map0 + r) * XW_COLS + kCol0;
#pragma unroll
    for (int i = 0; i < N / 8; ++i) {
      const int j = 8 * i + fc;
      if (j + 1 < kTok) *reinterpret_cast<float2*>(dst + j) = make_float2(acc[4 * i + 2 * h], acc[4 * i + 2 * h + 1]);
      else if (j < kTok) dst[j] = acc[4 * i + 2 * h];
    }
  }
}

template <int MB, bool HILO>
__global__ void __launch_bounds__(TC_THREADS, 1)
xw_gemm_kernel(const __grid_constant__ CUtensorMap tmD_hi, const __grid_constant__ CUtensorMap tmD_lo,
               const __grid_constant__ CUtensorMap tm0_hi, const __grid_constant__ CUtensorMap tm0_lo,
               const __grid_constant__ CUtensorMap tm1_hi, const __grid_constant__ CUtensorMap tm1_lo, XwCells cells,
               const int2* __restrict__ box_org, float* __restrict__ xbox, int K) {
  using Cfg = XwCfg<MB, HILO>;
  extern __shared__ uint8_t smem_raw[];
  uint8_t* smem = reinterpret_cast<uint8_t*>((reinterpret_cast<uintptr_t>(smem_raw) + 1023) & ~(uintptr_t)1023);
  uint64_t* full = reinterpret_cast<uint64_t*>(smem + Cfg::kStages * Cfg::kStageBytes);
  uint64_t* empty = full + Cfg::kStages;

  const int warp = threadIdx.x >> 5, wg = threadIdx.x >> 7;
  const int KB = (K + Cfg::kBK - 1) / Cfg::kBK;

  if (threadIdx.x == 0) {
    tc::prefetch_tmap(&tmD_hi); tc::prefetch_tmap(&tmD_lo); tc::prefetch_tmap(&tm0_hi);
    if (!HILO) tc::prefetch_tmap(&tm0_lo);
    tc::prefetch_tmap(&tm1_hi);
    if (!HILO) tc::prefetch_tmap(&tm1_lo);
    for (int s = 0; s < Cfg::kStages; ++s) { tc::mbar_init(&full[s], 1); tc::mbar_init(&empty[s], 2); }
    tc::mbar_fence_init();
  }
  __syncthreads();

  if (wg == 0) {
    tc::regs_dealloc<40>();
    if (warp == 0 && tc::elect_one()) {
      int stage = 0, phase = 0;
      for (int cell = blockIdx.x; cell < cells.n_cells; cell += gridDim.x) {
        const int2 org = box_org[cell];
        if (org.y == INT_MIN) continue;
        const int drow = cells.arow[cell], frame = cells.frame[cell];
        for (int part = 0; part < (MB == 64 ? 1 : 2); ++part) {
          for (int kb = 0; kb < KB; ++kb) {
            const int k0 = kb * Cfg::kBK, kt = HILO ? 2 * k0 : k0;
            tc::mbar_wait(&empty[stage], phase ^ 1);
            uint8_t* st = smem + stage * Cfg::kStageBytes;
            uint8_t* s0 = st + Cfg::kTokOff;
            if constexpr (MB == 64) {
              tc::mbar_expect_tx(&full[stage], 2 * Cfg::kDescBytes + Cfg::kBoxes * (Cfg::kTok0Tx + Cfg::kTok1Tx));
              uint8_t* s1 = s0 + Cfg::kBoxes * Cfg::kTok0Bytes;
              tc::tma_load_4d(&tm0_hi, &full[stage], s0, kt, org.y, org.x, frame);
              if (!HILO) tc::tma_load_4d(&tm0_lo, &full[stage], s0 + Cfg::kTok0Bytes, kt, org.y, org.x, frame);
              tc::tma_load_4d(&tm1_hi, &full[stage], s1, kt, org.y, org.x + XW_ROWS0, frame);
              if (!HILO) tc::tma_load_4d(&tm1_lo, &full[stage], s1 + Cfg::kTok1Bytes, kt, org.y, org.x + XW_ROWS0, frame);
            } else {
              tc::mbar_expect_tx(&full[stage], 2 * Cfg::kDescBytes + Cfg::kBoxes * (part ? Cfg::kTok1Tx : Cfg::kTok0Tx));
              const int by = org.x + (part ? XW_ROWS0 : 0);
              tc::tma_load_4d(part ? &tm1_hi : &tm0_hi, &full[stage], s0, kt, org.y, by, frame);
              if (!HILO) tc::tma_load_4d(part ? &tm1_lo : &tm0_lo, &full[stage], s0 + Cfg::kTok0Bytes, kt, org.y, by, frame);
            }
            tc::tma_load_2d(&tmD_hi, &full[stage], st, k0, drow);
            tc::tma_load_2d(&tmD_lo, &full[stage], st + Cfg::kDescBytes, k0, drow);
            if (++stage == Cfg::kStages) { stage = 0; phase ^= 1; }
          }
        }
      }
    }
  } else {
    tc::regs_alloc<232>();
    const int cw = wg - 1;
    int stage = 0, phase = 0;
    for (int cell = blockIdx.x; cell < cells.n_cells; cell += gridDim.x) {
      if (box_org[cell].y == INT_MIN) continue;
      const int m = cells.m[cell], map0 = cells.row0[cell];
      if constexpr (MB == 64) {
        if (cw == 0)
          xw_part<MB, HILO, XW_N0>(smem, full, empty, stage, phase, KB, 0, Cfg::kTokOff, Cfg::kTok0Bytes, xbox, map0, 0, m);
        else
          xw_part<MB, HILO, XW_N1>(smem, full, empty, stage, phase, KB, 0, Cfg::kTokOff + Cfg::kBoxes * Cfg::kTok0Bytes,
                                   Cfg::kTok1Bytes, xbox, map0, 0, m);
      } else {
        const uint32_t d_off = cw * 64 * Cfg::kRow;
        xw_part<MB, HILO, XW_N0>(smem, full, empty, stage, phase, KB, d_off, Cfg::kTokOff, Cfg::kTok0Bytes, xbox, map0, 64 * cw, m);
        xw_part<MB, HILO, XW_N1>(smem, full, empty, stage, phase, KB, d_off, Cfg::kTokOff, Cfg::kTok0Bytes, xbox, map0, 64 * cw, m);
      }
    }
  }
}

template <int MB, bool HILO>
static int run_xw_gemm(const CUtensorMap (&tm)[6], const XwCells& cells, const XwChunk& xc, int C, cudaStream_t st) {
  static PerDev<bool> attr_dev;
  bool& attr = attr_dev.get();
  if (!attr) {
    DTK_CUDA(cudaFuncSetAttribute(xw_gemm_kernel<MB, HILO>, cudaFuncAttributeMaxDynamicSharedMemorySize, XwCfg<MB, HILO>::kSmem));
    attr = true;
  }
  const int sms = num_sms();
  const int grid = cells.n_cells < sms ? cells.n_cells : sms;
  ProfRange pr(PROF_XW_GEMM, st);
  xw_gemm_kernel<MB, HILO><<<grid, TC_THREADS, XwCfg<MB, HILO>::kSmem, st>>>(tm[0], tm[1], tm[2], tm[3], tm[4], tm[5], cells,
                                                                              xc.box_org, xc.xbox, C);
  DTK_LAUNCHED();
  return DINOTRK_OK;
}

int launch_xw_gemm(const FeatView& fv, const dinotrk_geom& g, const void* desc_hi, const void* desc_lo, int desc_rows,
                   const XwCells& cells, const XwChunk& xc, cudaStream_t st) {
  if (cells.n_cells <= 0) return DINOTRK_OK;
  DTK_CHECK_ARG(fv.C % 8 == 0 && cells.max_m <= XW_MAX_CELL, "exact-window GEMM: bad sizes");
  const bool small = cells.max_m <= 64, hilo = fv.hilo != nullptr;
  constexpr int BK = XwCfg<64, false>::kBK, SW = 2 * BK;
  CUtensorMap tm[6];
  int rc;
  if ((rc = make_tmap_2d(&tm[0], desc_hi, desc_rows, fv.C, small ? 64 : 128, BK, TMAP_F16, 0, SW))) return rc;
  if ((rc = make_tmap_2d(&tm[1], desc_lo, desc_rows, fv.C, small ? 64 : 128, BK, TMAP_F16, 0, SW))) return rc;
  const uint64_t row = hilo ? (uint64_t)hilo_row(fv.C) : (uint64_t)fv.C;
  const uint64_t dims[4] = {row, (uint64_t)g.w, (uint64_t)g.h, (uint64_t)fv.T};
  const uint64_t strides[3] = {row * 2, (uint64_t)g.w * row * 2, (uint64_t)fv.P * row * 2};
  const uint32_t ib = hilo ? 2 * BK : BK, tsw = hilo ? 128 : SW;
  const uint32_t box0[4] = {ib, XW_BOX, XW_ROWS0, 1}, box1[4] = {ib, XW_BOX, XW_ROWS1, 1};
  if ((rc = make_tmap_4d(&tm[2], hilo ? fv.hilo : fv.hi, dims, strides, box0, TMAP_F16, tsw))) return rc;
  if ((rc = make_tmap_4d(&tm[4], hilo ? fv.hilo : fv.hi, dims, strides, box1, TMAP_F16, tsw))) return rc;
  if (hilo) {
    tm[3] = tm[2];
    tm[5] = tm[4];
    return small ? run_xw_gemm<64, true>(tm, cells, xc, fv.C, st) : run_xw_gemm<128, true>(tm, cells, xc, fv.C, st);
  }
  if ((rc = make_tmap_4d(&tm[3], fv.lo, dims, strides, box0, TMAP_F16, tsw))) return rc;
  if ((rc = make_tmap_4d(&tm[5], fv.lo, dims, strides, box1, TMAP_F16, tsw))) return rc;
  return small ? run_xw_gemm<64, false>(tm, cells, xc, fv.C, st) : run_xw_gemm<128, false>(tm, cells, xc, fv.C, st);
}

constexpr int XH_WARPS = 8;
constexpr int XH_WP = 16;
constexpr int XH_WIN = WM * XH_WP;
constexpr int XH_RP = 20;
constexpr int XH_RED = 240;
constexpr int XH_ZB = 128;
constexpr int XH_RAW = 2 * XH_WIN + 4 * XH_RED + 2 * XH_ZB;
constexpr int XH_PER_WARP = XH_RAW + 4 * XH_WIN;
constexpr int XH_SMEM = XH_WARPS * XH_PER_WARP * 4;
static_assert(XH_WIN % 32 == 16 && XH_RED % 32 == 16 && WB * XH_RP <= XH_RED && WB * WB <= XH_ZB, "head buffer layout");

constexpr int XH_KEYS = 4;

struct XhGather {
  int amax;
  float dn, mout;
  unsigned ok;
};

__device__ __forceinline__ void xh_cp4(float* dst, const float* src) {
  asm volatile("cp.async.ca.shared.global [%0], [%1], 4;\n" ::"r"((unsigned)__cvta_generic_to_shared(dst)), "l"(src) : "memory");
}
__device__ __forceinline__ void xh_cp_wait() { asm volatile("cp.async.wait_all;\n" ::: "memory"); }

__device__ __forceinline__ void xh_gather(XhGather& gt, int map, int n_maps, int l, int h, int w, int P, int n_tiles,
                                          const float* __restrict__ norms, const float* __restrict__ desc_norm,
                                          const int* __restrict__ cell_frame, const int* __restrict__ cell_of,
                                          const int2* __restrict__ box_org, const int* __restrict__ stat,
                                          const int* __restrict__ cand, const unsigned long long* __restrict__ key1,
                                          const float* __restrict__ max2, const float* __restrict__ xbox,
                                          const float* __restrict__ eps_map, float* __restrict__ racc, float* __restrict__ rfn) {
  gt.amax = -1;
  gt.ok = 0;
  if (map >= n_maps) return;
  const int st = __ldg(stat + map), cell = __ldg(cell_of + map);
  const float dn = __ldg(desc_norm + map);
  const int4 cd = __ldg(reinterpret_cast<const int4*>(cand) + map);
  const float eps = eps_map ? __ldg(eps_map + map) : XW_EPS;
  const unsigned long long* k1 = key1 + (size_t)map * n_tiles;
  const float* k2 = max2 + (size_t)map * n_tiles;
  unsigned long long kk[XH_KEYS];
  float kv2[XH_KEYS];
#pragma unroll
  for (int q = 0; q < XH_KEYS; ++q) {
    const int t = l + 16 * q;
    kk[q] = t < n_tiles ? __ldg(k1 + t) : 0ull;
    kv2[q] = t < n_tiles ? __ldg(k2 + t) : 0.f;
  }
  if (st != 0) return;
  const int2 org = __ldg(box_org + cell);
  const float* fn = norms + (size_t)__ldg(cell_frame + cell) * P;
  const float* xr = xbox + (size_t)map * XW_COLS;
  const int ct[4] = {cd.x, cd.y, cd.z, cd.w};
  float best = -1.f;
  int amax = -1;
#pragma unroll
  for (int q = 0; q < XW_MAX_CAND; ++q)
    if (ct[q] >= 0) {
      const int tr = ct[q] / w, tcn = ct[q] - tr * w;
      const float v = fmaxf(corr_cos(__ldg(xr + xw_col(tr - org.x, tcn - org.y)), dn, __ldg(fn + ct[q])), 0.f);
      if (v > best || (v == best && ct[q] < amax)) { best = v; amax = ct[q]; }
    }
  const int arow = amax / w, acol = amax - arow * w;
  float mout = 0.f;
  auto fold = [&](unsigned long long k, float m2) {
    const int tk = 0x7fffffff - (int)(k & 0xffffffffu);
    const int tr = tk / w, tcn = tk - tr * w;
    const bool in_core = abs(tr - arow) <= 3 && abs(tcn - acol) <= 3;
    mout = fmaxf(mout, (in_core ? m2 : __uint_as_float((unsigned)(k >> 32))) + eps);
  };
#pragma unroll
  for (int q = 0; q < XH_KEYS; ++q)
    if (l + 16 * q < n_tiles) fold(kk[q], kv2[q]);
  for (int t = l + 16 * XH_KEYS; t < n_tiles; t += 16) fold(__ldg(k1 + t), __ldg(k2 + t));
  const int c = acol - 7 + l;
  const bool col_in = l < WM && c >= 0 && c < w;
  unsigned ok = 0;
#pragma unroll
  for (int y = 0; y < WM; ++y) {
    const int r = arow - 7 + y;
    if (col_in && r >= 0 && r < h) {
      xh_cp4(racc + y * XH_WP + l, xr + xw_col(r - org.x, c - org.y));
      xh_cp4(rfn + y * XH_WP + l, fn + r * w + c);
      ok |= 1u << y;
    }
  }
  gt.amax = amax;
  gt.dn = dn;
  gt.mout = mout;
  gt.ok = ok;
}

__device__ __forceinline__ float xh_window(const XhGather& gt, const float* __restrict__ racc, const float* __restrict__ rfn,
                                           float* __restrict__ win, int l) {
  xh_cp_wait();
  float mout = gt.mout;
#pragma unroll
  for (int y = 0; y < WM; ++y) {
    float v = 0.f;
    if ((gt.ok >> y) & 1u) {
      v = fmaxf(corr_cos(racc[y * XH_WP + l], gt.dn, rfn[y * XH_WP + l]), 0.f);
      if (!(abs(y - 7) <= 3 && abs(l - 7) <= 3)) mout = fmaxf(mout, v);
    }
    win[y * XH_WP + l] = v;
  }
  return mout;
}

__device__ __forceinline__ float xh_tap3(const float* wk, float v0, float v1, float v2) {
  return __fmaf_rn(wk[2], v2, __fmaf_rn(wk[1], v1, __fmul_rn(wk[0], v0)));
}

template <bool INTERIOR>
__device__ __forceinline__ void xh_step(int j, const float (&A0in)[WB], const float (&Sin)[WB], float (&A0out)[WB],
                                        float (&Sout)[WB], const float* __restrict__ win, float* __restrict__ red,
                                        float* __restrict__ zb, const float (&w1)[9], float b1, const float (&w2)[9], float b2,
                                        bool row_in, unsigned cmask, int l) {
  float in[3][16];
#pragma unroll
  for (int ky = 0; ky < 3; ++ky)
#pragma unroll
    for (int q = 0; q < 4; ++q) {
      const float4 v = *reinterpret_cast<const float4*>(win + (j + ky) * XH_WP + 4 * q);
      in[ky][4 * q] = v.x; in[ky][4 * q + 1] = v.y; in[ky][4 * q + 2] = v.z; in[ky][4 * q + 3] = v.w;
    }
  float hr[WH];
#pragma unroll
  for (int x = 0; x < WH; ++x) {
    float a0 = __fmaf_rn(w1[0], in[0][x], b1), a1 = __fmul_rn(w1[3], in[1][x]), a2 = __fmul_rn(w1[6], in[2][x]);
    a0 = __fmaf_rn(w1[1], in[0][x + 1], a0); a1 = __fmaf_rn(w1[4], in[1][x + 1], a1); a2 = __fmaf_rn(w1[7], in[2][x + 1], a2);
    a0 = __fmaf_rn(w1[2], in[0][x + 2], a0); a1 = __fmaf_rn(w1[5], in[1][x + 2], a1); a2 = __fmaf_rn(w1[8], in[2][x + 2], a2);
    const float a = __fadd_rn(__fadd_rn(a0, a1), a2);
    hr[x] = INTERIOR || (row_in && ((cmask >> x) & 1u)) ? fmaxf(a, 0.f) : 0.f;
  }
  if (j < WB) {
#pragma unroll
    for (int x = 0; x < WB; ++x) A0out[x] = xh_tap3(w2, hr[x], hr[x + 1], hr[x + 2]);
  }
  if (j >= 1 && j <= WB) {
#pragma unroll
    for (int x = 0; x < WB; ++x) Sout[x] = __fadd_rn(A0in[x], xh_tap3(w2 + 3, hr[x], hr[x + 1], hr[x + 2]));
  }
  if (j >= 2) {
    float* rb = red + (j & 1) * (2 * XH_RED);
#pragma unroll
    for (int x = 0; x < WB; ++x) rb[x * XH_RP + l] = __fadd_rn(Sin[x], xh_tap3(w2 + 6, hr[x], hr[x + 1], hr[x + 2]));
    __syncwarp();
    if (l < WB) {
      float p[16];
#pragma unroll
      for (int q = 0; q < 4; ++q) {
        const float4 v = *reinterpret_cast<const float4*>(rb + l * XH_RP + 4 * q);
        p[4 * q] = v.x; p[4 * q + 1] = v.y; p[4 * q + 2] = v.z; p[4 * q + 3] = v.w;
      }
      float v[8];
#pragma unroll
      for (int i = 0; i < 8; ++i) v[i] = __fadd_rn(p[i], p[i + 8]);
      const float t = __fadd_rn(__fadd_rn(__fadd_rn(v[0], v[4]), __fadd_rn(v[2], v[6])),
                                __fadd_rn(__fadd_rn(v[1], v[5]), __fadd_rn(v[3], v[7])));
      zb[(j - 2) * WB + l] = __fadd_rn(t, b2);
    }
  }
}

template <bool INTERIOR>
__device__ __forceinline__ void xh_refine(const float* __restrict__ win, float* __restrict__ red, float* __restrict__ zb,
                                          const float (&w1)[9], float b1, const float (&w2)[9], float b2, int arow, int acol,
                                          int h, int w, int l) {
  unsigned cmask = 0;
#pragma unroll
  for (int x = 0; x < WH; ++x) cmask |= (acol - 6 + x >= 0 && acol - 6 + x < w) ? 1u << x : 0u;
  float A0a[WB], Sa[WB], A0b[WB], Sb[WB];
#pragma unroll
  for (int x = 0; x < WB; ++x) { A0a[x] = 0.f; Sa[x] = 0.f; }
#pragma unroll 1
  for (int j = 0; j < WH; j += 2) {
    xh_step<INTERIOR>(j, A0a, Sa, A0b, Sb, win, red, zb, w1, b1, w2, b2, arow - 6 + j >= 0 && arow - 6 + j < h, cmask, l);
    if (j + 1 < WH)
      xh_step<INTERIOR>(j + 1, A0b, Sb, A0a, Sa, win, red, zb, w1, b1, w2, b2, arow - 5 + j >= 0 && arow - 5 + j < h, cmask, l);
  }
}

__device__ __forceinline__ void xh_sums(const HeadParams& hp, const float* __restrict__ zb, int arow, int acol, int l,
                                        float& zmax, float (&tot)[5]) {
  float z[8];
  bool valid[8];
  zmax = -INFINITY;
#pragma unroll
  for (int k = 0; k < 8; ++k) {
    const int p = l + 16 * k;
    const int y = p / WB, x = p - y * WB, r = arow - 5 + y, c = acol - 5 + x;
    valid[k] = p < WB * WB && r >= 0 && r < hp.h && c >= 0 && c < hp.w;
    z[k] = valid[k] ? zb[p] : -INFINITY;
    zmax = fmaxf(zmax, z[k]);
  }
#pragma unroll
  for (int o = 8; o > 0; o >>= 1) zmax = fmaxf(zmax, __shfl_xor_sync(0xffffffffu, zmax, o));
  float s[2][5] = {};
#pragma unroll
  for (int k = 0; k < 8; ++k) {
    const int p = l + 16 * k;
    const int y = p / WB, x = p - y * WB, r = arow - 5 + y, c = acol - 5 + x;
    const float e = valid[k] ? expf(z[k] - zmax) : 0.f;
    float (&t)[5] = s[k & 1];
    t[0] += e;
    if (valid[k] && in_disc(hp, r, c, arow, acol)) {
      t[1] += e; t[2] = fmaf(token_px(hp, c), e, t[2]); t[3] = fmaf(token_px(hp, r), e, t[3]);
    }
    t[4] += valid[k] ? 1.f : 0.f;
  }
#pragma unroll
  for (int i = 0; i < 5; ++i) {
    float v = s[0][i] + s[1][i];
#pragma unroll
    for (int o = 8; o > 0; o >>= 1) v += __shfl_xor_sync(0xffffffffu, v, o);
    tot[i] = v;
  }
}

template <bool REFINE>
__global__ void __launch_bounds__(XH_WARPS * 32, 2)
xw_head_kernel(int n_maps, HeadParams hp, dinotrk_head_weights wts, int n_tiles, const float* __restrict__ norms,
               const float* __restrict__ desc_norm, const int* __restrict__ cell_frame, const int* __restrict__ cell_group,
               const int* __restrict__ cell_of, const int2* __restrict__ box_org, const int* __restrict__ stat,
               const int* __restrict__ cand, const unsigned long long* __restrict__ key1, const float* __restrict__ max2,
               const float* __restrict__ xbox, const float* __restrict__ eps_map, const int* __restrict__ grp_map0,
               const int* __restrict__ out_index, float* __restrict__ out, int* __restrict__ slow_cnt,
               int* __restrict__ slow_list, int n_groups) {
  extern __shared__ __align__(16) float xh_smem[];
  const int lane = threadIdx.x & 31, wid = __shfl_sync(0xffffffffu, (int)(threadIdx.x >> 5), 0);
  const int hf = lane >> 4, l = lane & 15;
  float* ws = xh_smem + wid * XH_PER_WARP;
  float* win = ws + hf * XH_WIN;
  float* red = ws + 2 * XH_WIN + hf * XH_RED;
  float* zb = ws + 2 * XH_WIN + 4 * XH_RED + hf * XH_ZB;
  float* racc = ws + XH_RAW + hf * XH_WIN;
  float* rfn = racc + 2 * XH_WIN;
  float w1[9], w2[9];
#pragma unroll
  for (int k = 0; k < 9; ++k) { w1[k] = wts.w1[l][k]; w2[k] = wts.w2[l][k]; }
  const float b1 = wts.b1[l];
  const int h = hp.h, w = hp.w;
  const int n_pairs = (n_maps + 1) >> 1, stride = gridDim.x * XH_WARPS;

  int pair = blockIdx.x * XH_WARPS + wid;
  XhGather gt;
  if (pair < n_pairs)
    xh_gather(gt, 2 * pair + hf, n_maps, l, h, w, hp.P, n_tiles, norms, desc_norm, cell_frame, cell_of, box_org, stat, cand,
              key1, max2, xbox, eps_map, racc, rfn);
  for (; pair < n_pairs; pair += stride) {
    const int map = 2 * pair + hf, amax = gt.amax;
    const bool exact = amax >= 0;
    const int arow = exact ? amax / w : 7, acol = exact ? amax - arow * w : 7;
    float mout = xh_window(gt, racc, rfn, win, l);
#pragma unroll
    for (int o = 8; o > 0; o >>= 1) mout = fmaxf(mout, __shfl_xor_sync(0xffffffffu, mout, o));
    const bool any = __any_sync(0xffffffffu, exact);
    const bool interior = __all_sync(0xffffffffu, !exact || (arow >= 7 && arow + 7 < h && acol >= 7 && acol + 7 < w));
    if (pair + stride < n_pairs)
      xh_gather(gt, 2 * (pair + stride) + hf, n_maps, l, h, w, hp.P, n_tiles, norms, desc_norm, cell_frame, cell_of, box_org,
                stat, cand, key1, max2, xbox, eps_map, racc, rfn);
    __syncwarp();
    if constexpr (!REFINE) {
      if (l == 0 && exact) out[(size_t)(out_index ? out_index[map] : map) * hp.out_stride] = mout;
      continue;
    }
    float zmax = 0.f;
    float tot[5] = {0.f, 0.f, 0.f, 0.f, 0.f};
    if (any) {
      if (interior) xh_refine<true>(win, red, zb, w1, b1, w2, wts.b2, arow, acol, h, w, l);
      else xh_refine<false>(win, red, zb, w1, b1, w2, wts.b2, arow, acol, h, w, l);
      __syncwarp();
      xh_sums(hp, zb, arow, acol, l, zmax, tot);
    }
    if (l == 0 && map < n_maps) {
      if (exact && head_certified(hp, wts, mout, zmax, tot)) {
        head_store_point(hp, __fdiv_rn(tot[2], tot[1]), __fdiv_rn(tot[3], tot[1]), out_index, out, map);
      } else {
        const int g = cell_group[cell_of[map]];
        const int pos = atomicAdd(slow_cnt + g, 1);
        slow_list[grp_map0[g] + pos] = map;
        atomicAdd(slow_cnt + n_groups, 1);
        if (exact) atomicAdd(slow_cnt + n_groups + 1, 1);
      }
    }
    __syncwarp();
  }
}

static int g_xw_head_window_only = 0;

int launch_xw_head(const FeatView& fv, const dinotrk_geom& g, const dinotrk_head_weights& hw, const XwCells& cells,
                   const float* desc_norm, const int* grp_map0, int n_maps, const int* out_index, float* out, int out_stride,
                   int out_mode, const XwChunk& xc, cudaStream_t st, int n_groups, const float* eps) {
  if (n_maps <= 0) return DINOTRK_OK;
  DTK_CHECK_ARG(disc_fits_box(g), "exact-window path: disc radius %d exceeds 5 tokens", g.radius);
  const HeadParams hp = make_head_params(g, hw, dinotrk_map_stride(&g), out_stride, out_mode);
  const int sms = num_sms();
  int grid = cdiv(cdiv(n_maps, 2), XH_WARPS);
  if (grid > sms * 2) grid = sms * 2;
  static PerDev<bool> attr_dev;
  bool& attr = attr_dev.get();
  if (!attr) {
    DTK_CUDA(cudaFuncSetAttribute(xw_head_kernel<true>, cudaFuncAttributeMaxDynamicSharedMemorySize, XH_SMEM));
    DTK_CUDA(cudaFuncSetAttribute(xw_head_kernel<false>, cudaFuncAttributeMaxDynamicSharedMemorySize, XH_SMEM));
    attr = true;
  }
  ProfRange pr(PROF_XW_HEAD, st);
  (g_xw_head_window_only ? xw_head_kernel<false> : xw_head_kernel<true>)<<<grid, XH_WARPS * 32, XH_SMEM, st>>>(n_maps, hp, hw, cdiv(hp.P, XW_TILE), fv.norms, desc_norm, cells.frame,
                                                       cells.group, xc.cell_of, xc.box_org, xc.stat, xc.cand, xc.key1, xc.max2,
                                                       xc.xbox, eps, grp_map0, out_index, out, xc.slow_cnt, xc.slow_list,
                                                       n_groups);
  DTK_LAUNCHED();
  return DINOTRK_OK;
}

template <bool HILO>
__global__ void __launch_bounds__(128)
xw_compact_kernel(const float4* __restrict__ desc, const uint4* __restrict__ dhi, const uint4* __restrict__ dlo,
                  const int* __restrict__ arow, const float* __restrict__ desc_norm, const int* __restrict__ out_index, int C, const int* __restrict__ grp_frame,
                  const int* __restrict__ grp_map0, int n_groups, const int* __restrict__ slow_cnt,
                  const int* __restrict__ slow_list, float4* __restrict__ c_desc, uint4* __restrict__ c_hi, uint4* __restrict__ c_lo,
                  float* __restrict__ c_norm, int* __restrict__ c_out_index, int* __restrict__ cgrp, int gcap, int row_base,
                  int grp_base) {
  __shared__ int s_g, s_pos;
  const int bb = blockIdx.x;
  if (threadIdx.x == 0) {
    int pre = 0, gsel = -1, psel = 0;
    for (int g = 0; g < n_groups; ++g) {
      const int c = slow_cnt[g];
      if (bb == 0) {
        cgrp[grp_base + g] = grp_frame[g]; cgrp[gcap + grp_base + g] = row_base + pre; cgrp[2 * gcap + grp_base + g] = c;
        cgrp[3 * gcap + grp_base + g] = row_base + pre;
      }
      if (gsel < 0 && bb < pre + c) { gsel = g; psel = bb - pre; }
      pre += c;
    }
    s_g = gsel; s_pos = psel;
  }
  __syncthreads();
  if (s_g < 0) return;
  const int b = row_base + bb;
  const int src = slow_list[grp_map0[s_g] + s_pos];
  const size_t srow = arow ? arow[src] : src;
  if (desc != nullptr)
    for (int i = threadIdx.x; i < C / 4; i += blockDim.x) c_desc[(size_t)b * (C / 4) + i] = desc[srow * (C / 4) + i];
  if (dhi != nullptr)
    for (int i = threadIdx.x; i < C / 8; i += blockDim.x) {
      if (HILO) {
        const size_t o = (size_t)b * (C / 4) + (i >> 2) * 8 + (i & 3);
        c_hi[o] = dhi[srow * (C / 8) + i];
        c_hi[o + 4] = dlo[srow * (C / 8) + i];
      } else {
        c_hi[(size_t)b * (C / 8) + i] = dhi[srow * (C / 8) + i];
        c_lo[(size_t)b * (C / 8) + i] = dlo[srow * (C / 8) + i];
      }
    }
  if (threadIdx.x == 0) { c_norm[b] = desc_norm[src]; c_out_index[b] = out_index[src]; }
}

int launch_xw_compact(const float* desc, const void* desc_hi, const void* desc_lo, const int* arow, const float* desc_norm,
                      const int* out_index, int C, const int* grp_frame, const int* grp_map0, int n_groups, int n_slow,
                      const XwChunk& xc, float* c_desc, void* c_hi, void* c_lo, float* c_norm, int* c_out_index, int* cgrp,
                      int gcap, cudaStream_t st, int row_base, int grp_base, bool hilo) {
  if (n_slow <= 0) return DINOTRK_OK;
  DTK_CHECK_ARG(!hilo || C % 32 == 0, "xw_compact: interleaved rows need C %% 32 == 0");
  ProfRange pr(PROF_MISC, st);
  (hilo ? xw_compact_kernel<true> : xw_compact_kernel<false>)<<<n_slow, 128, 0, st>>>(reinterpret_cast<const float4*>(desc), reinterpret_cast<const uint4*>(desc_hi),
                                            reinterpret_cast<const uint4*>(desc_lo), arow, desc_norm, out_index, C, grp_frame, grp_map0,
                                            n_groups, xc.slow_cnt, xc.slow_list, reinterpret_cast<float4*>(c_desc),
                                            reinterpret_cast<uint4*>(c_hi), reinterpret_cast<uint4*>(c_lo), c_norm, c_out_index, cgrp,
                                            gcap, row_base, grp_base);
  DTK_LAUNCHED();
  return DINOTRK_OK;
}

__global__ void xw_tile_prefix_kernel(const int* __restrict__ grp_m, int n_groups, int* __restrict__ tile_start) {
  const int lane = threadIdx.x;
  int base = 0;
  for (int g0 = 0; g0 < n_groups; g0 += 32) {
    const int g = g0 + lane;
    const int v = g < n_groups ? (grp_m[g] + TC2_BM - 1) / TC2_BM : 0;
    int inc = v;
#pragma unroll
    for (int o = 1; o < 32; o <<= 1) {
      const int u = __shfl_up_sync(0xffffffffu, inc, o);
      if (lane >= o) inc += u;
    }
    if (g < n_groups) tile_start[g] = base + inc - v;
    base += __shfl_sync(0xffffffffu, inc, 31);
  }
  if (lane == 0) tile_start[n_groups] = base;
}

struct XwKeysWs {
  float* rnorms; int* tile_start; unsigned* min_bits;
  XwKeysWs(Arena& ar, size_t tokens, int n_groups) {
    rnorms = ar.take<float>(tokens);
    tile_start = ar.take<int>(n_groups + 1);
    min_bits = ar.take<unsigned>(1);
  }
};

__global__ void xw_eps_kernel(const int* __restrict__ grp_frame, const int* __restrict__ grp_row0, const int* __restrict__ grp_m,
                              const float* __restrict__ rho, const float* __restrict__ rho_f, float slack, float* __restrict__ eps) {
  const int g = blockIdx.x, r0 = grp_row0[g];
  const float rf = rho_f[grp_frame[g]];
  for (int r = threadIdx.x; r < grp_m[g]; r += blockDim.x) eps[r0 + r] = xw_eps_s8(rho[r0 + r], rf, slack);
}

}

using namespace dtk;

extern "C" {

size_t dinotrk_xw_coarse_keys_workspace_bytes(int T, int n_groups, const dinotrk_geom* g) {
  return align_up(layout_end<XwKeysWs>((size_t)T * (g ? (size_t)g->h * g->w : 0), n_groups), 256) + 1024;
}

int dinotrk_xw_coarse_keys(const dinotrk_features* feat, const dinotrk_geom* g, const void* desc_hi, int desc_rows,
                           const float* desc_norm, const int* grp_frame, const int* grp_row0, const int* grp_m, int n_groups,
                           unsigned long long* key1, float* max2, void* workspace, size_t workspace_bytes, void* stream) {
  DTK_CHECK_ARG(feat && feat->norms && feat->hi && g && desc_hi && desc_norm && grp_frame && grp_row0 && grp_m && key1 && max2,
                "xw_coarse_keys: null pointer (the fp16 split of the features is required)");
  DTK_CHECK_ARG(feat->T > 0 && feat->C > 0 && feat->C % 8 == 0 && desc_rows > 0 && n_groups >= 0,
                "xw_coarse_keys: bad sizes (C must be a multiple of 8)");
  DTK_CHECK_ARG(workspace && workspace_bytes >= dinotrk_xw_coarse_keys_workspace_bytes(feat->T, n_groups, g),
                "xw_coarse_keys: workspace too small");
  if (n_groups == 0) return DINOTRK_OK;
  cudaStream_t st = (cudaStream_t)stream;
  const FeatView fv = make_view(*feat, *g);
  Arena ar(workspace);
  const XwKeysWs ws(ar, (size_t)fv.T * fv.P, n_groups);
  int rc = launch_xw_rnorms(fv, ws.rnorms, ws.min_bits, st);
  if (rc) return rc;
  {
    ProfRange pr(PROF_MISC, st);
    xw_tile_prefix_kernel<<<1, 32, 0, st>>>(grp_m, n_groups, ws.tile_start);
    DTK_LAUNCHED();
  }
  XwChunk xc{};
  xc.key1 = key1;
  xc.max2 = max2;
  return launch_xw_coarse(fv, desc_hi, desc_rows, desc_norm, grp_frame, grp_row0, grp_m, grp_row0, ws.tile_start, n_groups,
                          desc_rows / TC2_BM + n_groups, xc, st, ws.rnorms);
}

int dinotrk_xw_coarse_keys_i8(const dinotrk_features* feat, const dinotrk_geom* g, const void* desc_q8, const float* desc_fac,
                              const float* desc_rho, int desc_rows, const int* grp_frame, const int* grp_row0, const int* grp_m,
                              int n_groups, unsigned long long* key1, float* max2, float* eps, void* workspace,
                              size_t workspace_bytes, void* stream) {
  DTK_CHECK_ARG(feat && feat->norms && feat->q8 && feat->q_fac && feat->q_rho && g && desc_q8 && desc_fac && desc_rho &&
                grp_frame && grp_row0 && grp_m && key1 && max2, "xw_coarse_keys_i8: null pointer (the int8 features are required)");
  DTK_CHECK_ARG(feat->T > 0 && feat->C > 0 && feat->C % 16 == 0 && feat->C <= XW_S8_MAX_C && desc_rows > 0 && n_groups >= 0,
                "xw_coarse_keys_i8: bad sizes (C must be a multiple of 16, <= %d)", XW_S8_MAX_C);
  DTK_CHECK_ARG(workspace && workspace_bytes >= dinotrk_xw_coarse_keys_workspace_bytes(feat->T, n_groups, g),
                "xw_coarse_keys_i8: workspace too small");
  if (n_groups == 0) return DINOTRK_OK;
  cudaStream_t st = (cudaStream_t)stream;
  const FeatView fv = make_view(*feat, *g);
  Arena ar(workspace);
  const XwKeysWs ws(ar, (size_t)fv.T * fv.P, n_groups);
  {
    ProfRange pr(PROF_MISC, st);
    xw_tile_prefix_kernel<<<1, 32, 0, st>>>(grp_m, n_groups, ws.tile_start);
    DTK_LAUNCHED();
    if (eps) {
      xw_eps_kernel<<<n_groups, 128, 0, st>>>(grp_frame, grp_row0, grp_m, desc_rho, fv.q_rho, xw_s8_slack(fv.C), eps);
      DTK_LAUNCHED();
    }
  }
  XwChunk xc{};
  xc.key1 = key1;
  xc.max2 = max2;
  return launch_xw_coarse(fv, nullptr, desc_rows, nullptr, grp_frame, grp_row0, grp_m, grp_row0, ws.tile_start, n_groups,
                          desc_rows / TC2_BM + n_groups, xc, st, nullptr, desc_q8, desc_fac);
}

int dinotrk_xw_head_set_window_only(int on) {
  DTK_CHECK_ARG(on == 0 || on == 1, "xw_head_set_window_only: 0 or 1");
  g_xw_head_window_only = on;
  return DINOTRK_OK;
}

int dinotrk_xw_box_gemm(const dinotrk_features* feat, const dinotrk_geom* g, const void* desc_hi, const void* desc_lo,
                        int desc_rows, const int* cell_row0, const int* cell_m, const int* cell_frame, const int* box_org,
                        int n_cells, int max_m, float* xbox, void* stream) {
  DTK_CHECK_ARG(feat && feat->hi && feat->lo && g && desc_hi && desc_lo && cell_row0 && cell_m && cell_frame && box_org && xbox,
                "xw_box_gemm: null pointer (the fp16 split of the features is required)");
  DTK_CHECK_ARG(feat->T > 0 && feat->C > 0 && feat->C % 8 == 0 && desc_rows > 0 && n_cells >= 0 && max_m > 0 &&
                max_m <= XW_MAX_CELL, "xw_box_gemm: bad sizes (C must be a multiple of 8, cells of 1..%d rows)", XW_MAX_CELL);
  DTK_CHECK_ARG(reinterpret_cast<uintptr_t>(box_org) % 8 == 0, "xw_box_gemm: box_org must be 8-byte aligned");
  const FeatView fv = make_view(*feat, *g);
  const XwCells cells{cell_row0, cell_row0, cell_m, cell_frame, nullptr, n_cells, max_m};
  XwChunk xc{};
  xc.box_org = reinterpret_cast<int2*>(const_cast<int*>(box_org));
  xc.xbox = xbox;
  return launch_xw_gemm(fv, *g, desc_hi, desc_lo, desc_rows, cells, xc, (cudaStream_t)stream);
}

}
```

dino_tracker_b200/csrc/xwin.cuh:

```cuda
#pragma once
#include <type_traits>

#include "common.cuh"
#include "corr.cuh"

namespace dtk {

constexpr float XW_EPS = 1.1e-3f;
constexpr int XW_BOX = 21;
constexpr int XW_SLACK = 3;
constexpr int XW_ROWS0 = 12, XW_ROWS1 = XW_BOX - XW_ROWS0;
constexpr int XW_N0 = 256, XW_N1 = 192;
constexpr int XW_COLS = 448;
constexpr int XW_MAX_CELL = 128;
constexpr int XW_MAX_CAND = 4;
constexpr float XW_MIN_NORM = 1e-4f;
constexpr int XW_TILE = 128;

constexpr float XW_S8_SLACK = 3.0518e-5f;
constexpr int XW_S8_EXACT_C = 1040;
constexpr int XW_S8_MAX_C = 2048;
inline float xw_s8_slack(int C) {
  if (C <= XW_S8_EXACT_C) return XW_S8_SLACK;
  const double s = (double)XW_S8_SLACK + 3.0 * (double)((C + 15) / 16) * 0x1p-23;
  const float f = (float)s;
  return (double)f < s ? nextafterf(f, INFINITY) : f;
}
constexpr float XW_S8_RHO_MAX = 0.03f;
__device__ __forceinline__ float xw_eps_s8(float rho_d, float rho_f, float slack) {
  return __fadd_ru(__fadd_ru(rho_d, __fmul_ru(__fadd_ru(1.f, rho_d), rho_f)), slack);
}

template <class Load>
__device__ __forceinline__ float xw_quant_row(const Load& ld, int C, float norm, int8_t* __restrict__ q, float* __restrict__ fac) {
  const int lane = threadIdx.x & 31;
  float mx = 0.f;
  for (int k = 4 * lane; k < C; k += 128) {
    const float4 v = ld(k);
    mx = fmaxf(mx, fmaxf(fmaxf(fabsf(v.x), fabsf(v.y)), fmaxf(fabsf(v.z), fabsf(v.w))));
  }
#pragma unroll
  for (int o = 16; o > 0; o >>= 1) mx = fmaxf(mx, __shfl_xor_sync(0xffffffffu, mx, o));
  const float s = __fdiv_rn(mx, 127.f);
  double r2 = 0.0, x2 = 0.0;
  for (int k = 4 * lane; k < C; k += 128) {
    const float4 v = ld(k);
    const float vv[4] = {v.x, v.y, v.z, v.w};
    char4 o;
    signed char* oc = reinterpret_cast<signed char*>(&o);
#pragma unroll
    for (int e = 0; e < 4; ++e) {
      const float qf = s > 0.f ? fminf(fmaxf(rintf(__fdiv_rn(vv[e], s)), -127.f), 127.f) : 0.f;
      oc[e] = (signed char)qf;
      const double d = (double)vv[e] - (double)s * (double)qf;
      r2 = fma(d, d, r2);
      x2 = fma((double)vv[e], (double)vv[e], x2);
    }
    *reinterpret_cast<char4*>(q + k) = o;
  }
#pragma unroll
  for (int o = 16; o > 0; o >>= 1) {
    r2 += __shfl_xor_sync(0xffffffffu, r2, o);
    x2 += __shfl_xor_sync(0xffffffffu, x2, o);
  }
  if (lane == 0) *fac = __fdiv_rn(s, fmaxf(norm, XW_MIN_NORM));
  return x2 > 0.0 ? __double2float_ru(__ddiv_ru(__dsqrt_ru(r2), __dsqrt_rd(x2))) : 0.f;
}

__host__ __device__ inline int xw_col(int by, int bx) { return by * XW_BOX + bx; }

struct XwChunk {
  unsigned long long* key1;
  float* max2;
  int* cand;
  int* pinfo;
  int* stat;
  int* cell_of;
  int2* box_org;
  float* xbox;
  int* slow_cnt;
  int* slow_list;
  XwChunk() = default;
  XwChunk(Arena& ar, size_t maps, size_t cells, int n_tiles, int n_groups) {
    key1 = ar.take<unsigned long long>(maps * n_tiles);
    max2 = ar.take<float>(maps * n_tiles);
    cand = ar.take<int>(maps * XW_MAX_CAND);
    stat = ar.take<int>(maps);
    pinfo = ar.take<int>(maps);
    cell_of = ar.take<int>(maps);
    slow_list = ar.take<int>(maps);
    box_org = ar.take<int2>(cells);
    xbox = ar.take<float>(maps * XW_COLS);
    slow_cnt = ar.take<int>((size_t)n_groups + 2);
  }
};

struct XwCells {
  const int* row0;
  const int* arow;
  const int* m;
  const int* frame;
  const int* group;
  int n_cells, max_m;
};

int launch_xw_coarse(const FeatView& fv, const void* desc_hi, int desc_rows, const float* desc_norm, const int* grp_frame,
                     const int* grp_row0, const int* grp_m, const int* grp_map0, const int* tile_start, int n_groups,
                     int max_tiles, const XwChunk& xc, cudaStream_t st, const float* rnorms, const void* desc_q8 = nullptr,
                     const float* desc_fac = nullptr);
int launch_xw_rnorms(const FeatView& fv, float* rnorms, unsigned* min_bits, cudaStream_t st);
int launch_xw_plan(const XwCells& cells, const float* desc_norm, int n_groups, const dinotrk_geom& g, const XwChunk& xc,
                   cudaStream_t st, int n_maps, float min_norm, const float* eps);
int launch_xw_gemm(const FeatView& fv, const dinotrk_geom& g, const void* desc_hi, const void* desc_lo, int desc_rows,
                   const XwCells& cells, const XwChunk& xc, cudaStream_t st);
int launch_xw_head(const FeatView& fv, const dinotrk_geom& g, const dinotrk_head_weights& hw, const XwCells& cells,
                   const float* desc_norm, const int* grp_map0, int n_maps, const int* out_index, float* out, int out_stride,
                   int out_mode, const XwChunk& xc, cudaStream_t st, int n_groups, const float* eps);
int launch_xw_compact(const float* desc, const void* desc_hi, const void* desc_lo, const int* arow, const float* desc_norm,
                      const int* out_index, int C, const int* grp_frame, const int* grp_map0, int n_groups, int n_slow,
                      const XwChunk& xc, float* c_desc, void* c_hi, void* c_lo, float* c_norm, int* c_out_index, int* cgrp,
                      int gcap, cudaStream_t st, int row_base = 0, int grp_base = 0, bool hilo = false);

}
```

include/dinotrk.h:

```cpp
#ifndef DINOTRK_H_
#define DINOTRK_H_

#include <stddef.h>
#include <stdint.h>

#ifdef __cplusplus
extern "C" {
#endif

#define DINOTRK_VERSION 100

#define DINOTRK_OK 0
#define DINOTRK_EINVAL (-22)
#define DINOTRK_ECUDA (-5)
#define DINOTRK_ENOMEM (-12)

typedef struct dinotrk_geom {
  int H, W, patch, stride, radius;
  int h, w;
} dinotrk_geom;

typedef struct dinotrk_head_weights {
  float w1[16][9];
  float b1[16];
  float w2[16][9];
  float b2;
} dinotrk_head_weights;

typedef struct dinotrk_features {
  const float* tpc;
  const float* norms;
  const void* hi;
  const void* lo;
  int T, C;
  const void* q8;
  const float* q_fac;
  const float* q_rho;
  const void* hilo;
} dinotrk_features;

int dinotrk_version(void);
const char* dinotrk_last_error(void);
int dinotrk_make_geom(int H, int W, int patch, int stride, int radius, dinotrk_geom* g);

int dinotrk_pack_features(const float* chw, float* tpc, float* norms, int T, int C, int P,
                          void* stream);
int dinotrk_unpack_features(const float* tpc, float* chw, int T, int C, int P, void* stream);
int dinotrk_token_norms(const float* tpc, float* norms, int T, int C, int P, void* stream);
int dinotrk_quantise_s8(const float* x, const float* norms, size_t rows, int C, int rows_per_group, void* q, float* fac,
                        float* rho, float* rho_max, void* stream);
int dinotrk_split_fp16(const float* x, void* hi, void* lo, size_t n, void* stream);
int dinotrk_split_hilo(const float* x, void* hilo, size_t rows, int C, void* stream);
int dinotrk_split_range(const float* x, size_t n, const float* norms, size_t n_tok, float* range, void* stream);
int dinotrk_split_faithful(float max_abs, float min_norm, int C);

int dinotrk_sample_descriptors(const float* tpc, int T, int C, const dinotrk_geom* g,
                               const float* points, int B, const int* frames_set, int N,
                               int points_normalized, float* desc, float* desc_norm,
                               void* stream);

size_t dinotrk_corr_track_workspace_bytes(int total_maps, int n_groups, int C, const dinotrk_geom* g);
int dinotrk_corr_track(const dinotrk_features* feat, const dinotrk_geom* g,
                       const dinotrk_head_weights* hw, const float* desc, const float* desc_norm,
                       const int* grp_frame, const int* grp_row0, const int* grp_m,
                       const int* grp_map0, int n_groups, int total_maps, int max_group_m,
                       const int* out_index, float* out, int out_stride, int out_mode,
                       void* workspace, size_t workspace_bytes, void* stream);

int dinotrk_map_stride(const dinotrk_geom* g);
size_t dinotrk_corr_maps_workspace_bytes(int total_maps, int n_groups, int C);
int dinotrk_corr_maps(const dinotrk_features* feat, const dinotrk_geom* g,
                      const float* desc, const float* desc_norm, const int* grp_frame,
                      const int* grp_row0, const int* grp_m, const int* grp_map0, int n_groups,
                      int total_maps, int max_group_m, float* maps, void* workspace,
                      size_t workspace_bytes, void* stream);
int dinotrk_head(const float* maps, int n_maps, const dinotrk_geom* g,
                 const dinotrk_head_weights* hw, const int* out_index, float* out,
                 int out_stride, int out_mode, int* aux, int* scratch, void* stream);

size_t dinotrk_track_backward_workspace_bytes(int B, int C, const dinotrk_geom* g);
int dinotrk_track_backward(const dinotrk_features* feat, const dinotrk_geom* g, const dinotrk_head_weights* hw,
                           const float* points, const int* frames_set, int N, const float* desc,
                           const float* desc_norm, const int* tgt_frame, const float* maps, const int* aux,
                           const float* grad_out, int B, float* grad_w, float* grad_tpc, void* workspace,
                           size_t workspace_bytes, void* stream);

int dinotrk_sample_backward(int T, int C, const dinotrk_geom* g, const float* points, int B, const int* frames_set,
                            int N, int points_normalized, const float* grad_desc, float* grad_tpc, void* stream);

size_t dinotrk_infer_workspace_bytes(int T, int C, const dinotrk_geom* g, int N, int chunk_maps);
size_t dinotrk_infer_max_chunks(int T, int N, int chunk_maps);
int dinotrk_infer_plan(int kind, int T, int N, const int* anchor_counts, int chunk_maps, int* groups, int* meta,
                       int max_chunks, int* n_chunks);
int dinotrk_infer_anchor_gcap(int T, int chunk_maps);
int dinotrk_infer_plan_anchors(int T, int N, const int* anchor_counts, const int* qlist, const unsigned char* query_flag,
                               int chunk_maps, int probe, int* groups, int* meta, int max_chunks, int* n_chunks);
int dinotrk_infer_set_overlap(int mode);
int dinotrk_infer_set_path(int path);
int dinotrk_xw_head_set_window_only(int on);
int dinotrk_infer_set_coarse(int mode);
int dinotrk_infer_last_stats(long long* out, int n);
size_t dinotrk_xw_coarse_keys_workspace_bytes(int T, int n_groups, const dinotrk_geom* g);
int dinotrk_xw_coarse_keys(const dinotrk_features* feat, const dinotrk_geom* g, const void* desc_hi, int desc_rows,
                           const float* desc_norm, const int* grp_frame, const int* grp_row0, const int* grp_m, int n_groups,
                           unsigned long long* key1, float* max2, void* workspace, size_t workspace_bytes, void* stream);
int dinotrk_xw_coarse_keys_i8(const dinotrk_features* feat, const dinotrk_geom* g, const void* desc_q8, const float* desc_fac,
                              const float* desc_rho, int desc_rows, const int* grp_frame, const int* grp_row0, const int* grp_m,
                              int n_groups, unsigned long long* key1, float* max2, float* eps, void* workspace,
                              size_t workspace_bytes, void* stream);
int dinotrk_xw_box_gemm(const dinotrk_features* feat, const dinotrk_geom* g, const void* desc_hi, const void* desc_lo,
                        int desc_rows, const int* cell_row0, const int* cell_m, const int* cell_frame, const int* box_org,
                        int n_cells, int max_m, float* xbox, void* stream);
int dinotrk_infer(const dinotrk_features* feat, const dinotrk_geom* g,
                  const dinotrk_head_weights* hw, const float* query_points, int N,
                  float anchor_th, float cos_th, int frame_batch, int start_phase, int stop_after,
                  int chunk_maps,
                  float* traj, float* cos_sims, float* anchors, uint8_t* occ,
                  void* workspace, size_t workspace_bytes, void* stream);
int dinotrk_traj_cos_sims(const float* tpc, int T, int C, const dinotrk_geom* g,
                          const float* traj, const float* query_points, int N, float* cos_sims,
                          void* workspace, size_t workspace_bytes, void* stream);
int dinotrk_occlusion(const float* traj, const float* cos_sims, const float* anchors, int N, int T,
                      float anchor_th, float cos_th, uint8_t* occ, void* stream);

size_t dinotrk_delta_workspace_bytes(int B, int H, int W, const int* channels);
int dinotrk_delta_refine(const float* frames, int B, int H, int W, const int* channels,
                         const float* const* wgt, const float* const* bias, const float* dino_tpc,
                         const float* ixs, const float* iys, int h, int w, float* refined_tpc,
                         float* norms, void* workspace, size_t workspace_bytes, void* stream);

int dinotrk_delta_refine_allgather(const float* frames, int B, int H, int W, const int* channels,
                                   const float* const* wgt, const float* const* bias, const float* dino_tpc,
                                   const float* ixs, const float* iys, int h, int w, float* refined_tpc,
                                   float* norms, void* workspace, size_t workspace_bytes,
                                   float* const* peer_bases, int n_peers, size_t first_frame, void* stream);
int dinotrk_delta_refine_tc(const float* frames, int B, int H, int W, const int* channels,
                            const void* const* wgt_hi, const void* const* wgt_lo, const float* const* bias,
                            const float* dino_tpc, const float* ixs, const float* iys, int h, int w,
                            float* refined_tpc, float* norms, void* workspace, size_t workspace_bytes,
                            float* const* peer_bases, int n_peers, size_t first_frame, void* stream);
int dinotrk_peer_alloc(size_t bytes, void** ptr, unsigned char* handle64);
int dinotrk_peer_open(const unsigned char* handle64, void** ptr);
int dinotrk_peer_close(void* ptr);
int dinotrk_peer_free(void* ptr);

size_t dinotrk_delta_train_saved_bytes(int B, int H, int W, const int* channels);
size_t dinotrk_delta_train_forward_workspace_bytes(int B, int H, int W, const int* channels);
size_t dinotrk_delta_train_backward_workspace_bytes(int B, int H, int W, const int* channels);
int dinotrk_delta_train_forward(const float* frames, int B, int H, int W, const int* channels, const void* const* wgt_hi,
                                const void* const* wgt_lo, const float* const* conv_bias, const float* const* bn_weight,
                                const float* const* bn_bias, float* const* running_mean, float* const* running_var,
                                int training, float momentum, float eps, const float* ixs, const float* iys, int h, int w,
                                float* residual_tpc, void* saved, size_t saved_bytes, void* workspace, size_t workspace_bytes,
                                void* stream);
int dinotrk_delta_train_backward(const float* frames, int B, int H, int W, const int* channels, const void* const* wgtT_hi,
                                 const void* const* wgtT_lo, const float* const* bn_weight, const float* const* bn_bias,
                                 int training, const float* ixs, const float* iys, int h, int w, const float* grad_residual_tpc,
                                 const void* saved, size_t saved_bytes, float* const* grad_wgt, float* const* grad_bias,
                                 float* const* grad_bn_weight, float* const* grad_bn_bias, void* workspace,
                                 size_t workspace_bytes, void* stream);

typedef struct dinotrk_vit_config {
  int depth, dim, heads;
  int tap_layer;
  int patch, stride;
  int attn_materialized;
  int gemm_f16;
  int gemm_pair;
  int swiglu_hidden;
  int facet;
} dinotrk_vit_config;
typedef struct dinotrk_vit_weights {
  const void* patch_w; const float* patch_b; const float* cls_pos; const float* pos;
  const float* const* blocks;
} dinotrk_vit_weights;
size_t dinotrk_vit_workspace_bytes(const dinotrk_vit_config* c, const dinotrk_geom* g, int B);
int dinotrk_vit_forward(const float* frames, int B, const dinotrk_geom* g, const dinotrk_vit_config* c,
                        const dinotrk_vit_weights* wt, float* out_tpc, void* workspace,
                        size_t workspace_bytes, void* stream);
int dinotrk_vit_attention(const void* q16, const void* k16, const void* vT16, int B, int heads, int N1, int N1p,
                          float* out, void* stream);
int dinotrk_vit_attention_f16(const void* q16, const void* k16, const void* vT16, int B, int heads, int N1, int N1p,
                              void* out16, void* stream);
#define DINOTRK_VIT_LAYERNORM 0
#define DINOTRK_VIT_PATCH 1
#define DINOTRK_VIT_QKV 2
#define DINOTRK_VIT_PROJ 3
#define DINOTRK_VIT_FC1 4
#define DINOTRK_VIT_FC2 5
#define DINOTRK_VIT_SWIGLU 6
#define DINOTRK_VIT_STAGE_WORKSPACE_BYTES 4096
int dinotrk_vit_stage(int stage, const dinotrk_vit_config* c, const dinotrk_geom* g, int B, const void* in, const void* w,
                      const float* p0, const float* p1, void* out0, void* out1, void* out2, void* workspace,
                      size_t workspace_bytes, void* stream);

size_t dinotrk_best_buddies_workspace_bytes(int n_pairs, int P);
int dinotrk_best_buddies_pairs(const dinotrk_features* feat, const dinotrk_geom* g, const int* pair_src,
                               const int* pair_tgt, int n_pairs, int* nn_idx, float* nn_cos,
                               void* workspace, size_t workspace_bytes, void* stream);
int dinotrk_bb_mutual(const int* nn_st, const int* nn_ts, int n_pairs, int P, uint8_t* mutual, void* stream);
int dinotrk_bb_nms(const float* maps, int n_maps, const dinotrk_geom* g, float box_size, float iou_thresh, int topk,
                   float* peak_affs, float* r, void* stream);

typedef struct dinotrk_flow_video {
  const float* fwd;
  const float* bwd;
  int T, H, W;
} dinotrk_flow_video;
int dinotrk_flow_masks(const dinotrk_flow_video* fv, float threshold, uint8_t* masks, void* stream);
size_t dinotrk_traj_workspace_bytes(int T, int H, int W);
int dinotrk_traj_chain(const dinotrk_flow_video* fv, const uint8_t* masks, int s, float threshold, int min_len,
                       const float* direct_fwd, const float* direct_bwd, float direct_threshold, int* n_kept,
                       void* workspace, size_t workspace_bytes, void* stream);
int dinotrk_traj_emit(const dinotrk_flow_video* fv, int s, float* out, void* workspace, size_t workspace_bytes, void* stream);

size_t dinotrk_traj_nearest_workspace_bytes(int M, int T, int gh, int gw);
int dinotrk_traj_nearest(const float* traj, int M, int T, int gh, int gw, float start, float step, int* nearest,
                         void* workspace, size_t workspace_bytes, void* stream);
int dinotrk_of_filter(const float* traj, int M, int T, const int* nearest, int gh, int gw, int stride, const float* src_xy,
                      const float* tgt_xy, const int* pair_src, const int* pair_tgt, const int* offsets, int n_pairs, int n_pts,
                      uint8_t* keep, void* stream);

size_t dinotrk_pca_workspace_bytes(long long M, int C, int q);
int dinotrk_pca_stats(const float* a, long long M, int C, int normalize, float* s, float* c, void* workspace,
                      size_t workspace_bytes, void* stream);
int dinotrk_pca_power(const float* a, long long M, int C, int q, const float* s, const float* c, const float* P, float* X,
                      float* W, void* workspace, size_t workspace_bytes, void* stream);
int dinotrk_fg_mask(const float* a, int T, int h, int w, int C, int q, const float* s, const float* V, float threshold,
                    int H, int W, float* colors, uint8_t* token_mask, uint8_t* mask, void* workspace, size_t workspace_bytes,
                    void* stream);
int dinotrk_mask_upsample(const uint8_t* token_mask, int T, int h, int w, int H, int W, uint8_t* out, void* stream);
size_t dinotrk_traj_split_workspace_bytes(int N);
int dinotrk_traj_split_count(const float* traj, int N, int T, const uint8_t* masks, int Tm, int H, int W, int* n_fg,
                             void* workspace, size_t workspace_bytes, void* stream);
int dinotrk_traj_split_emit(const float* traj, int N, int T, float* fg, float* bg, void* workspace, size_t workspace_bytes,
                            void* stream);

int dinotrk_bb_contrastive_cos_stride(int P);
size_t dinotrk_bb_contrastive_forward_workspace_bytes(int N, int P, int C, int B, int n_groups);
int dinotrk_bb_contrastive_forward(const float* E, int N, int P, int C, const float* S, const float* U, int B,
                                   const int* grp_src, const int* grp_tgt, const int* grp_row0, const int* grp_rows, int n_groups,
                                   float tau, float* cos, float* out, void* workspace, size_t workspace_bytes, void* stream);
size_t dinotrk_bb_contrastive_backward_workspace_bytes(int N, int P, int C, int B, const int* grp_src, const int* grp_tgt,
                                                       const int* grp_row0, const int* grp_rows, int n_groups);
int dinotrk_bb_contrastive_backward(const float* E, int N, int P, int C, const float* S, const float* U, int B,
                                    const int* grp_src, const int* grp_tgt, const int* grp_row0, const int* grp_rows,
                                    int n_groups, float tau, const float* cos, const float* out, const float* g_st,
                                    const float* g_ts, const float* g_bbmean, const float* g_cmean, float* dS, float* dU,
                                    float* dE, void* workspace, size_t workspace_bytes, void* stream);

size_t dinotrk_sampler_workspace_bytes(int N);
int dinotrk_sampler_prepare_count(const float* traj, int N, int T, int* n_valid, void* workspace, size_t workspace_bytes,
                                  void* stream);
int dinotrk_sampler_prepare_emit(const float* traj, int N, int T, float* rows, uint32_t* bits, void* workspace,
                                 size_t workspace_bytes, void* stream);
int dinotrk_sampler_count(const uint32_t* bits, int N, int T, const int64_t* frames, int n_frames, int* n_cand,
                          void* workspace, size_t workspace_bytes, void* stream);
int dinotrk_sampler_select(const uint32_t* bits, int N, int T, const int64_t* frames, int n_frames, const int64_t* perm,
                           int m, int64_t* row_ids, float* mat, void* workspace, size_t workspace_bytes, void* stream);
int dinotrk_sampler_gather(const float* rows, int T, const int64_t* row_ids, const int64_t* draws, int m, float* t1,
                           float* t2, void* stream);

#define DINOTRK_CPU_RNG_STATE_BYTES 5056
int dinotrk_randperm_prefix(uint8_t* state, size_t state_bytes, int64_t n, int64_t k, int64_t* out);
size_t dinotrk_cycle_mask_workspace_bytes(int T, int P);
int dinotrk_cycle_mask_scan(const uint8_t* fg, int T, int P, int* off, int* n_fg, void* workspace, size_t workspace_bytes,
                            void* stream);
int dinotrk_cycle_select(const uint8_t* fg, int T, int H, int W, const int* off, const int* rows, int R, float* start,
                         float* there_pts, void* stream);
int dinotrk_cycle_unnorm(const float* there_out, const int* rows, int R, int H, int W, float* there_px, float* back_pts,
                         void* stream);
int dinotrk_cycle_keep(const float* start, const float* back_out, int R, int H, int W, float thresh, int* keep_rows,
                       float* cycle_px, int* n_keep, void* stream);

size_t dinotrk_emb_reg_workspace_bytes(int n, int P);
int dinotrk_emb_reg_forward(const float* E, const float* R, int n, int P, int C, float* out, float* aux, void* workspace,
                            size_t workspace_bytes, void* stream);
int dinotrk_emb_reg_backward(const float* E, const float* R, int n, int P, int C, const float* aux, const float* g_norm,
                             const float* g_angle, float* dE, void* stream);

enum {
  DINOTRK_RAFT_FNET = 0, DINOTRK_RAFT_CNET = 16, DINOTRK_RAFT_CONVCORR1 = 32, DINOTRK_RAFT_CONVCORR2, DINOTRK_RAFT_CONVFLOW1,
  DINOTRK_RAFT_CONVFLOW2, DINOTRK_RAFT_MOTION_CONV, DINOTRK_RAFT_GRU1_ZR, DINOTRK_RAFT_GRU1_Q, DINOTRK_RAFT_GRU2_ZR,
  DINOTRK_RAFT_GRU2_Q, DINOTRK_RAFT_FLOW_HEAD1, DINOTRK_RAFT_FLOW_HEAD2, DINOTRK_RAFT_MASK1, DINOTRK_RAFT_MASK2,
  DINOTRK_RAFT_NCONV
};
typedef struct {
  const void* w_hi[DINOTRK_RAFT_NCONV];
  const void* w_lo[DINOTRK_RAFT_NCONV];
  const float* bias[DINOTRK_RAFT_NCONV];
  float scale[DINOTRK_RAFT_NCONV];
} dinotrk_raft_weights;
size_t dinotrk_raft_encode_workspace_bytes(int H, int W);
int dinotrk_raft_encode(const float* frames, int T, int T_ctx, int H, int W, const dinotrk_raft_weights* w, float* fmap,
                        float* ctx, void* workspace, size_t workspace_bytes, void* stream);
size_t dinotrk_raft_flow_workspace_bytes(int H, int W, int n_pairs);
int dinotrk_raft_flow(const float* fmap, const void* fmap_hi, const void* fmap_lo, const float* ctx, int T, int T_ctx, int H,
                      int W, const int* pairs, int n_pairs, int num_flow_updates, const dinotrk_raft_weights* w, float* flows,
                      void* workspace, size_t workspace_bytes, void* stream);

int dinotrk_profile_classes(void);
const char* dinotrk_profile_class_name(int cls);
void dinotrk_profile_enable(int on);
int dinotrk_profile_collect(double* ms, unsigned long long* launches, int n);

unsigned long long dinotrk_launch_count(void);

#ifdef __cplusplus
}
#endif
#endif
```

Measured before the change: 11580.

## Shrink exact-window GEMM token boxes to the candidates' tight bounding extent

The cell planning kernel now records, per cell, the tight row and column extent of all fitting candidates, padded by the window size, alongside the fixed 21x21 box origin. The exact-window GEMM loads and multiplies only that sub-box, split into 128-token parts through a cached table of TMA tensor maps indexed by width and row count, and scatters results back into the 21-wide xbox layout. This cuts tensor-core and TMA traffic when candidate boxes are compact. In exchange it adds more pipeline stages, a larger prebuilt table of tensor maps, scalar scattered stores in place of float2 stores, and extra atomic counters that are copied to the host as statistics.

New measurement: 11990 (median of 6 runs). 3.6% higher.

```diff
diff --git a/dino_tracker_b200/_lib.py b/dino_tracker_b200/_lib.py
--- a/dino_tracker_b200/_lib.py
+++ b/dino_tracker_b200/_lib.py
@@ -92,6 +92,7 @@
     "dinotrk_xw_coarse_keys_i8": (c_int, [POINTER(Features), POINTER(Geom), _P, _P, _P, c_int, _P, _P, _P, c_int, _P, _P, _P, _P,
                                           c_size_t, _P]),
     "dinotrk_xw_box_gemm": (c_int, [POINTER(Features), POINTER(Geom), _P, _P, c_int, _P, _P, _P, _P, c_int, c_int, _P, _P]),
+    "dinotrk_xw_box_gemm_ext": (c_int, [POINTER(Features), POINTER(Geom), _P, _P, c_int, _P, _P, _P, _P, _P, c_int, c_int, _P, _P]),
     "dinotrk_infer_plan": (c_int, [c_int, c_int, c_int, _P, c_int, _P, _P, c_int, _P]),
     "dinotrk_infer_anchor_gcap": (c_int, [c_int, c_int]),
     "dinotrk_infer_plan_anchors": (c_int, [c_int, c_int, _P, _P, _P, c_int, c_int, _P, _P, c_int, _P]),
@@ -329,12 +330,13 @@
 
 
 def infer_stats():
-    a = (ctypes.c_longlong * 10)()
-    check(load().dinotrk_infer_last_stats(a, 10), "infer_last_stats")
+    a = (ctypes.c_longlong * 12)()
+    check(load().dinotrk_infer_last_stats(a, 12), "infer_last_stats")
     rho_f = struct.unpack("<f", struct.pack("<I", int(a[7])))[0]
     return {"anchor_maps": int(a[0]), "exact_window": int(a[1]), "full_map": int(a[2]), "pipeline": "exact-window" if a[3] else "full-map",
             "full_map_by_certificate": int(a[4]), "contraction": "fp16x3" if a[5] else "fp32",
-            "coarse": "int8" if a[6] else "fp16", "coarse_rho_f": rho_f, "desc_in_place": int(a[8]), "desc_gathered": int(a[9])}
+            "coarse": "int8" if a[6] else "fp16", "coarse_rho_f": rho_f, "desc_in_place": int(a[8]), "desc_gathered": int(a[9]),
+            "exact_box_cells": int(a[10]), "exact_box_tokens": int(a[11])}
 
 
 def launch_count():
diff --git a/dino_tracker_b200/csrc/inference.cu b/dino_tracker_b200/csrc/inference.cu
--- a/dino_tracker_b200/csrc/inference.cu
+++ b/dino_tracker_b200/csrc/inference.cu
@@ -434,7 +434,7 @@
 constexpr int XW_RING = 4;
 constexpr int XW_PROBE_MAPS = 4096;
 constexpr int INFER_A_COUNTED = 16;
-constexpr int XW_CNT_A = 2 * XW_RING, XW_CNT_MINNORM = XW_CNT_A + INFER_A_COUNTED;
+constexpr int XW_CNT_CHUNK = 4, XW_CNT_A = XW_CNT_CHUNK * XW_RING, XW_CNT_MINNORM = XW_CNT_A + INFER_A_COUNTED;
 struct XwAsync {
   int state;
   cudaEvent_t sample[XW_RING], done[XW_RING], freed[XW_RING];
@@ -459,7 +459,7 @@
 static int g_xw_coarse = -1;
 namespace infer_stat {
 enum { anchor_maps, exact_window, full_map, pipeline, full_map_by_certificate, contraction, coarse, coarse_rho_f,
-       desc_in_place, desc_gathered, count };
+       desc_in_place, desc_gathered, exact_box_cells, exact_box_tokens, count };
 }
 static long long g_infer_stats[infer_stat::count] = {};
 constexpr int XW_S8_PROBE_QUEUE_DIV = 16;
@@ -706,8 +706,10 @@
     InferWs& ws = c.ws;
     XwAsync* xa = choice.xa;
     DTK_CUDA(cudaEventSynchronize(xa->done[j % XW_RING]));
-    const int n_slow = xa->host_cnt[2 * (j % XW_RING)];
-    g_infer_stats[infer_stat::full_map_by_certificate] += xa->host_cnt[2 * (j % XW_RING) + 1];
+    const int* cnt = xa->host_cnt + XW_CNT_CHUNK * (j % XW_RING);
+    const int n_slow = cnt[0];
+    g_infer_stats[infer_stat::full_map_by_certificate] += cnt[1];
+    g_infer_stats[infer_stat::exact_box_tokens] += cnt[2]; g_infer_stats[infer_stat::exact_box_cells] += cnt[3];
     const ChunkMeta& cm = c.metas[j];
     const XwSet& x = ws.xr[j % XW_RING];
     const InferCtx::Grp gp = c.grp_of(j);
@@ -767,7 +769,8 @@
     if ((rc = launch_xw_head(c.fv, c.g, c.hw, cells, x.norm, gp.map0, cm.used, x.out_index, anchors, 2, 0, x.xc, st, cm.n_groups,
                              eps)))
       return rc;
-    DTK_CUDA(cudaMemcpyAsync(xa->host_cnt + 2 * (k % XW_RING), x.xc.slow_cnt + cm.n_groups, 2 * sizeof(int), cudaMemcpyDeviceToHost, st));
+    DTK_CUDA(cudaMemcpyAsync(xa->host_cnt + XW_CNT_CHUNK * (k % XW_RING), x.xc.slow_cnt + cm.n_groups, XW_CNT_CHUNK * sizeof(int),
+                             cudaMemcpyDeviceToHost, st));
     DTK_CUDA(cudaEventRecord(xa->done[k % XW_RING], st));
     if (k == 0 && choice.probe && c.metas.size() > 1) {
       if ((rc = pipe.finish(0))) return rc;
@@ -896,6 +899,7 @@
   stats[infer_stat::anchor_maps] = maps_C; stats[infer_stat::exact_window] = 0; stats[infer_stat::full_map] = 0;
   stats[infer_stat::pipeline] = choice.xw ? 1 : 0; stats[infer_stat::full_map_by_certificate] = 0;
   stats[infer_stat::contraction] = c.fv.tensor() ? 1 : 0; stats[infer_stat::desc_in_place] = 0; stats[infer_stat::desc_gathered] = 0;
+  stats[infer_stat::exact_box_cells] = 0; stats[infer_stat::exact_box_tokens] = 0;
   float rho_max = 0.f;
   for (float r : rho_f) rho_max = std::max(rho_max, r);
   int rc = choice.coarse_pass(c.fv, rho_max);
diff --git a/dino_tracker_b200/csrc/xwin.cu b/dino_tracker_b200/csrc/xwin.cu
--- a/dino_tracker_b200/csrc/xwin.cu
+++ b/dino_tracker_b200/csrc/xwin.cu
@@ -164,7 +164,7 @@
   const int lane = threadIdx.x & 31;
   const int gw = blockIdx.x * PLAN_WARPS + (threadIdx.x >> 5), nw = gridDim.x * PLAN_WARPS;
   if (gw == 0)
-    for (int i = lane; i <= n_groups + 1; i += 32) slow_cnt[i] = 0;
+    for (int i = lane; i <= n_groups + 3; i += 32) slow_cnt[i] = 0;
   for (int map = gw; map < n_maps; map += nw) {
     const unsigned long long* k1 = key1 + (size_t)map * n_tiles;
     const float* k2 = max2 + (size_t)map * n_tiles;
@@ -205,7 +205,7 @@
 
 __global__ void __launch_bounds__(PLAN_WARPS * 32)
 xw_cell_kernel(XwCells cells, int w, const int* __restrict__ cand, const int* __restrict__ pinfo, int* __restrict__ stat,
-               int* __restrict__ cell_of, int2* __restrict__ box_org) {
+               int* __restrict__ cell_of, int2* __restrict__ box_org, int4* __restrict__ box_ext, int* __restrict__ box_cnt) {
   __shared__ short s_r[PLAN_WARPS][XW_MAX_CELL], s_c[PLAN_WARPS][XW_MAX_CELL];
   __shared__ unsigned char s_ok[PLAN_WARPS][XW_MAX_CELL];
   const int lane = threadIdx.x & 31, wid = threadIdx.x >> 5;
@@ -246,10 +246,11 @@
         med_c = max(med_c, __shfl_xor_sync(0xffffffffu, med_c, o));
       }
     }
-    int n_fit = 0;
+    int n_fit = 0, lo_r = INT_MAX, hi_r = INT_MIN, lo_c = INT_MAX, hi_c = INT_MIN;
     for (int r = lane; r < m; r += 32) {
       const int map = row0 + r;
       bool fit = s_ok[wid][r] != 0;
+      int mr0 = INT_MAX, mr1 = INT_MIN, mc0 = INT_MAX, mc1 = INT_MIN;
       if (fit) {
         const int4 cd = __ldg(reinterpret_cast<const int4*>(cand) + map);
         const int ct[4] = {cd.x, cd.y, cd.z, cd.w};
@@ -258,15 +259,29 @@
           if (ct[q] >= 0) {
             const int tr = ct[q] / w, tc_ = ct[q] - tr * w;
             fit = fit && abs(tr - med_r) <= XW_SLACK && abs(tc_ - med_c) <= XW_SLACK;
+            mr0 = min(mr0, tr); mr1 = max(mr1, tr); mc0 = min(mc0, tc_); mc1 = max(mc1, tc_);
           }
       }
       stat[map] = fit ? 0 : 1;
       n_fit += fit ? 1 : 0;
-    }
-#pragma unroll
-    for (int o = 16; o > 0; o >>= 1) n_fit += __shfl_xor_sync(0xffffffffu, n_fit, o);
-    if (lane == 0)
-      box_org[cell] = n_fit > 0 ? make_int2(med_r - XW_BOX / 2, med_c - XW_BOX / 2) : make_int2(0, INT_MIN);
+      if (fit) { lo_r = min(lo_r, mr0); hi_r = max(hi_r, mr1); lo_c = min(lo_c, mc0); hi_c = max(hi_c, mc1); }
+    }
+#pragma unroll
+    for (int o = 16; o > 0; o >>= 1) {
+      n_fit += __shfl_xor_sync(0xffffffffu, n_fit, o);
+      lo_r = min(lo_r, __shfl_xor_sync(0xffffffffu, lo_r, o)); hi_r = max(hi_r, __shfl_xor_sync(0xffffffffu, hi_r, o));
+      lo_c = min(lo_c, __shfl_xor_sync(0xffffffffu, lo_c, o)); hi_c = max(hi_c, __shfl_xor_sync(0xffffffffu, hi_c, o));
+    }
+    if (lane == 0) {
+      const int org_r = med_r - XW_BOX / 2, org_c = med_c - XW_BOX / 2;
+      box_org[cell] = n_fit > 0 ? make_int2(org_r, org_c) : make_int2(0, INT_MIN);
+      if (n_fit > 0) {
+        const int4 e = make_int4(lo_r - WM / 2 - org_r, lo_c - WM / 2 - org_c, hi_r - lo_r + WM, hi_c - lo_c + WM);
+        box_ext[cell] = e;
+        atomicAdd(box_cnt, e.z * e.w);
+        atomicAdd(box_cnt + 1, 1);
+      }
+    }
     __syncwarp();
   }
 }
@@ -287,10 +302,19 @@
   DTK_LAUNCHED();
   grid = cdiv(cells.n_cells, PLAN_WARPS);
   if (grid > num_sms() * 8) grid = num_sms() * 8;
-  xw_cell_kernel<<<grid, PLAN_WARPS * 32, 0, st>>>(cells, g.w, xc.cand, xc.pinfo, xc.stat, xc.cell_of, xc.box_org);
+  xw_cell_kernel<<<grid, PLAN_WARPS * 32, 0, st>>>(cells, g.w, xc.cand, xc.pinfo, xc.stat, xc.cell_of, xc.box_org, xc.box_ext,
+                                                   xc.slow_cnt + n_groups + 2);
   DTK_LAUNCHED();
   return DINOTRK_OK;
 }
+
+constexpr int XW_EXT_MIN = WM;
+constexpr int XW_NW = XW_BOX - XW_EXT_MIN + 1;
+constexpr int XW_PART_TOK = 128;
+constexpr int XW_PART_ROWS = XW_PART_TOK / XW_EXT_MIN;
+
+template <bool HILO>
+struct XwTokMaps { CUtensorMap m[HILO ? 1 : 2][XW_NW][XW_PART_ROWS]; };
 
 template <int MB, bool HILO>
 struct XwCfg {
@@ -299,24 +323,40 @@
   static constexpr int kTokRow = HILO ? 2 * kRow : kRow;
   static constexpr int kBoxes = HILO ? 1 : 2;
   static constexpr int kDescBytes = MB * kRow;
-  static constexpr int kTok0Bytes = XW_N0 * kTokRow, kTok1Bytes = XW_N1 * kTokRow;
-  static constexpr int kTok0Tx = XW_ROWS0 * XW_BOX * kTokRow, kTok1Tx = XW_ROWS1 * XW_BOX * kTokRow;
+  static constexpr int kSlotBytes = XW_PART_TOK * kTokRow;
+  static constexpr int kParts = MB == 64 ? 2 : 1;
   static constexpr int kTokOff = 2 * kDescBytes;
-  static constexpr int kStageBytes = kTokOff + kBoxes * (MB == 64 ? kTok0Bytes + kTok1Bytes : kTok0Bytes);
-  static constexpr int kStages = MB == 64 ? 3 : 4;
+  static constexpr int kStageBytes = kTokOff + kParts * kBoxes * kSlotBytes;
+  static constexpr int kStages = MB == 64 ? 5 : 6;
   static constexpr int kSmem = kStages * kStageBytes + 1024 + 256;
   static_assert(kStages * kStageBytes + 1024 + 256 <= 227 * 1024, "shared-memory ring too large");
-  static_assert(kTokOff % 1024 == 0 && kTok0Bytes % 1024 == 0 && kTok1Bytes % 1024 == 0 && kStageBytes % 1024 == 0,
+  static_assert(kTokOff % 1024 == 0 && kSlotBytes % 1024 == 0 && kStageBytes % 1024 == 0,
                 "token boxes must start 1024-byte aligned");
 };
 
-template <int MB, bool HILO, int N>
+template <int MB>
+struct XwExt {
+  int y, x, bh, bw, n;
+  __device__ __forceinline__ XwExt(const int4* __restrict__ box_ext, int cell) {
+    const int4 e = box_ext ? __ldg(box_ext + cell) : make_int4(0, 0, XW_BOX, XW_BOX);
+    y = e.x; x = e.y; bh = e.z; bw = e.w;
+    const int rp = XW_PART_TOK / max(bw, 1);
+    n = ok() ? (bh + rp - 1) / rp : 0;
+    if (MB == 64) n += n & 1;
+  }
+  __device__ __forceinline__ bool ok() const {
+    return y >= 0 && x >= 0 && bh >= XW_EXT_MIN && bw >= XW_EXT_MIN && y + bh <= XW_BOX && x + bw <= XW_BOX;
+  }
+  __device__ __forceinline__ int rows(int i) const { return bh / n + (i < bh % n ? 1 : 0); }
+  __device__ __forceinline__ int row(int i) const { return y + i * (bh / n) + min(i, bh % n); }
+};
+
+template <int MB, bool HILO>
 __device__ __forceinline__ void xw_part(uint8_t* smem, uint64_t* full, uint64_t* empty, int& stage, int& phase, int KB,
                                         uint32_t d_off, uint32_t t_off, uint32_t t_half, float* __restrict__ xbox, int map0,
-                                        int r0, int m) {
+                                        int r0, int m, int ntok, int bw, int col0) {
   using Cfg = XwCfg<MB, HILO>;
-  constexpr int kTok = (N == XW_N0 ? XW_ROWS0 : XW_ROWS1) * XW_BOX;
-  constexpr int kCol0 = N == XW_N0 ? 0 : XW_ROWS0 * XW_BOX;
+  constexpr int N = XW_PART_TOK;
   const int warp = threadIdx.x >> 5, lane = threadIdx.x & 31, t = threadIdx.x & 127;
   float acc[N / 2];
 #pragma unroll
@@ -351,12 +391,15 @@
   for (int h = 0; h < 2; ++h) {
     const int r = r0 + fr + 8 * h;
     if (r >= m) continue;
-    float* dst = xbox + (size_t)(map0 + r) * XW_COLS + kCol0;
+    float* dst = xbox + (size_t)(map0 + r) * XW_COLS + col0;
+    int y = 0, x = fc;
 #pragma unroll
     for (int i = 0; i < N / 8; ++i) {
       const int j = 8 * i + fc;
-      if (j + 1 < kTok) *reinterpret_cast<float2*>(dst + j) = make_float2(acc[4 * i + 2 * h], acc[4 * i + 2 * h + 1]);
-      else if (j < kTok) dst[j] = acc[4 * i + 2 * h];
+      if (j < ntok) dst[y * XW_BOX + x] = acc[4 * i + 2 * h];
+      if (j + 1 < ntok) dst[x + 1 == bw ? (y + 1) * XW_BOX : y * XW_BOX + x + 1] = acc[4 * i + 2 * h + 1];
+      x += 8;
+      if (x >= bw) { x -= bw; ++y; }
     }
   }
 }
@@ -364,9 +407,8 @@
 template <int MB, bool HILO>
 __global__ void __launch_bounds__(TC_THREADS, 1)
 xw_gemm_kernel(const __grid_constant__ CUtensorMap tmD_hi, const __grid_constant__ CUtensorMap tmD_lo,
-               const __grid_constant__ CUtensorMap tm0_hi, const __grid_constant__ CUtensorMap tm0_lo,
-               const __grid_constant__ CUtensorMap tm1_hi, const __grid_constant__ CUtensorMap tm1_lo, XwCells cells,
-               const int2* __restrict__ box_org, float* __restrict__ xbox, int K) {
+               const __grid_constant__ XwTokMaps<HILO> tok, XwCells cells, const int2* __restrict__ box_org,
+               const int4* __restrict__ box_ext, float* __restrict__ xbox, int K) {
   using Cfg = XwCfg<MB, HILO>;
   extern __shared__ uint8_t smem_raw[];
   uint8_t* smem = reinterpret_cast<uint8_t*>((reinterpret_cast<uintptr_t>(smem_raw) + 1023) & ~(uintptr_t)1023);
@@ -377,10 +419,7 @@
   const int KB = (K + Cfg::kBK - 1) / Cfg::kBK;
 
   if (threadIdx.x == 0) {
-    tc::prefetch_tmap(&tmD_hi); tc::prefetch_tmap(&tmD_lo); tc::prefetch_tmap(&tm0_hi);
-    if (!HILO) tc::prefetch_tmap(&tm0_lo);
-    tc::prefetch_tmap(&tm1_hi);
-    if (!HILO) tc::prefetch_tmap(&tm1_lo);
+    tc::prefetch_tmap(&tmD_hi); tc::prefetch_tmap(&tmD_lo);
     for (int s = 0; s < Cfg::kStages; ++s) { tc::mbar_init(&full[s], 1); tc::mbar_init(&empty[s], 2); }
     tc::mbar_fence_init();
   }
@@ -393,25 +432,22 @@
       for (int cell = blockIdx.x; cell < cells.n_cells; cell += gridDim.x) {
         const int2 org = box_org[cell];
         if (org.y == INT_MIN) continue;
-        const int drow = cells.arow[cell], frame = cells.frame[cell];
-        for (int part = 0; part < (MB == 64 ? 1 : 2); ++part) {
+        const XwExt<MB> e(box_ext, cell);
+        const int drow = cells.arow[cell], frame = cells.frame[cell], col = org.y + e.x;
+        const int wi = e.bw - XW_EXT_MIN;
+        for (int p0 = 0; p0 < e.n; p0 += Cfg::kParts) {
+          int tok_rows = 0;
+          for (int q = 0; q < Cfg::kParts; ++q) tok_rows += e.rows(p0 + q) * e.bw;
           for (int kb = 0; kb < KB; ++kb) {
             const int k0 = kb * Cfg::kBK, kt = HILO ? 2 * k0 : k0;
             tc::mbar_wait(&empty[stage], phase ^ 1);
             uint8_t* st = smem + stage * Cfg::kStageBytes;
-            uint8_t* s0 = st + Cfg::kTokOff;
-            if constexpr (MB == 64) {
-              tc::mbar_expect_tx(&full[stage], 2 * Cfg::kDescBytes + Cfg::kBoxes * (Cfg::kTok0Tx + Cfg::kTok1Tx));
-              uint8_t* s1 = s0 + Cfg::kBoxes * Cfg::kTok0Bytes;
-              tc::tma_load_4d(&tm0_hi, &full[stage], s0, kt, org.y, org.x, frame);
-              if (!HILO) tc::tma_load_4d(&tm0_lo, &full[stage], s0 + Cfg::kTok0Bytes, kt, org.y, org.x, frame);
-              tc::tma_load_4d(&tm1_hi, &full[stage], s1, kt, org.y, org.x + XW_ROWS0, frame);
-              if (!HILO) tc::tma_load_4d(&tm1_lo, &full[stage], s1 + Cfg::kTok1Bytes, kt, org.y, org.x + XW_ROWS0, frame);
-            } else {
-              tc::mbar_expect_tx(&full[stage], 2 * Cfg::kDescBytes + Cfg::kBoxes * (part ? Cfg::kTok1Tx : Cfg::kTok0Tx));
-              const int by = org.x + (part ? XW_ROWS0 : 0);
-              tc::tma_load_4d(part ? &tm1_hi : &tm0_hi, &full[stage], s0, kt, org.y, by, frame);
-              if (!HILO) tc::tma_load_4d(part ? &tm1_lo : &tm0_lo, &full[stage], s0 + Cfg::kTok0Bytes, kt, org.y, by, frame);
+            tc::mbar_expect_tx(&full[stage], 2 * Cfg::kDescBytes + Cfg::kBoxes * tok_rows * Cfg::kTokRow);
+            for (int q = 0; q < Cfg::kParts; ++q) {
+              uint8_t* s = st + Cfg::kTokOff + q * Cfg::kBoxes * Cfg::kSlotBytes;
+              const int ri = e.rows(p0 + q) - 1, row = org.x + e.row(p0 + q);
+              tc::tma_load_4d(&tok.m[0][wi][ri], &full[stage], s, kt, col, row, frame);
+              if constexpr (!HILO) tc::tma_load_4d(&tok.m[1][wi][ri], &full[stage], s + Cfg::kSlotBytes, kt, col, row, frame);
             }
             tc::tma_load_2d(&tmD_hi, &full[stage], st, k0, drow);
             tc::tma_load_2d(&tmD_lo, &full[stage], st + Cfg::kDescBytes, k0, drow);
@@ -426,24 +462,54 @@
     int stage = 0, phase = 0;
     for (int cell = blockIdx.x; cell < cells.n_cells; cell += gridDim.x) {
       if (box_org[cell].y == INT_MIN) continue;
+      const XwExt<MB> e(box_ext, cell);
       const int m = cells.m[cell], map0 = cells.row0[cell];
-      if constexpr (MB == 64) {
-        if (cw == 0)
-          xw_part<MB, HILO, XW_N0>(smem, full, empty, stage, phase, KB, 0, Cfg::kTokOff, Cfg::kTok0Bytes, xbox, map0, 0, m);
-        else
-          xw_part<MB, HILO, XW_N1>(smem, full, empty, stage, phase, KB, 0, Cfg::kTokOff + Cfg::kBoxes * Cfg::kTok0Bytes,
-                                   Cfg::kTok1Bytes, xbox, map0, 0, m);
-      } else {
-        const uint32_t d_off = cw * 64 * Cfg::kRow;
-        xw_part<MB, HILO, XW_N0>(smem, full, empty, stage, phase, KB, d_off, Cfg::kTokOff, Cfg::kTok0Bytes, xbox, map0, 64 * cw, m);
-        xw_part<MB, HILO, XW_N1>(smem, full, empty, stage, phase, KB, d_off, Cfg::kTokOff, Cfg::kTok0Bytes, xbox, map0, 64 * cw, m);
-      }
-    }
-  }
+      for (int p0 = 0; p0 < e.n; p0 += Cfg::kParts) {
+        if constexpr (MB == 64) {
+          const int p = p0 + cw;
+          xw_part<MB, HILO>(smem, full, empty, stage, phase, KB, 0, Cfg::kTokOff + cw * Cfg::kBoxes * Cfg::kSlotBytes,
+                            Cfg::kSlotBytes, xbox, map0, 0, m, e.rows(p) * e.bw, e.bw, xw_col(e.row(p), e.x));
+        } else {
+          xw_part<MB, HILO>(smem, full, empty, stage, phase, KB, cw * 64 * Cfg::kRow, Cfg::kTokOff, Cfg::kSlotBytes, xbox,
+                            map0, 64 * cw, m, e.rows(p0) * e.bw, e.bw, xw_col(e.row(p0), e.x));
+        }
+      }
+    }
+  }
+}
+
+template <bool HILO>
+static int xw_tok_maps(const FeatView& fv, const dinotrk_geom& g, const XwTokMaps<HILO>*& out) {
+  struct Entry { const void* base[2]; uint64_t dims[4]; bool valid; XwTokMaps<HILO> maps; };
+  static PerDev<Entry> cache;
+  Entry& e = cache.get();
+  const void* base[2] = {HILO ? fv.hilo : fv.hi, HILO ? nullptr : fv.lo};
+  const uint64_t row = HILO ? (uint64_t)hilo_row(fv.C) : (uint64_t)fv.C;
+  const uint64_t dims[4] = {row, (uint64_t)g.w, (uint64_t)g.h, (uint64_t)fv.T};
+  if (!e.valid || memcmp(e.base, base, sizeof(base)) != 0 || memcmp(e.dims, dims, sizeof(dims)) != 0) {
+    e.valid = false;
+    const uint64_t strides[3] = {row * 2, (uint64_t)g.w * row * 2, (uint64_t)fv.P * row * 2};
+    constexpr int BK = XwCfg<64, HILO>::kBK;
+    const uint32_t ib = HILO ? 2 * BK : BK, tsw = HILO ? 128 : 2 * BK;
+    for (int o = 0; o < (HILO ? 1 : 2); ++o)
+      for (int wi = 0; wi < XW_NW; ++wi)
+        for (int ri = 0; ri < XW_PART_ROWS; ++ri) {
+          const uint32_t box[4] = {ib, (uint32_t)(XW_EXT_MIN + wi), (uint32_t)(1 + ri), 1};
+          if (int rc = make_tmap_4d(&e.maps.m[o][wi][ri], base[o], dims, strides, box, TMAP_F16, tsw)) return rc;
+        }
+    memcpy(e.base, base, sizeof(base));
+    memcpy(e.dims, dims, sizeof(dims));
+    e.valid = true;
+  }
+  out = &e.maps;
+  return DINOTRK_OK;
 }
 
 template <int MB, bool HILO>
-static int run_xw_gemm(const CUtensorMap (&tm)[6], const XwCells& cells, const XwChunk& xc, int C, cudaStream_t st) {
+static int run_xw_gemm(const FeatView& fv, const dinotrk_geom& g, const CUtensorMap (&tmD)[2], const XwCells& cells,
+                       const XwChunk& xc, cudaStream_t st) {
+  const XwTokMaps<HILO>* tok;
+  if (int rc = xw_tok_maps<HILO>(fv, g, tok)) return rc;
   static PerDev<bool> attr_dev;
   bool& attr = attr_dev.get();
   if (!attr) {
@@ -453,8 +519,8 @@
   const int sms = num_sms();
   const int grid = cells.n_cells < sms ? cells.n_cells : sms;
   ProfRange pr(PROF_XW_GEMM, st);
-  xw_gemm_kernel<MB, HILO><<<grid, TC_THREADS, XwCfg<MB, HILO>::kSmem, st>>>(tm[0], tm[1], tm[2], tm[3], tm[4], tm[5], cells,
-                                                                              xc.box_org, xc.xbox, C);
+  xw_gemm_kernel<MB, HILO><<<grid, TC_THREADS, XwCfg<MB, HILO>::kSmem, st>>>(tmD[0], tmD[1], *tok, cells, xc.box_org, xc.box_ext,
+                                                                              xc.xbox, fv.C);
   DTK_LAUNCHED();
   return DINOTRK_OK;
 }
@@ -465,25 +531,12 @@
   DTK_CHECK_ARG(fv.C % 8 == 0 && cells.max_m <= XW_MAX_CELL, "exact-window GEMM: bad sizes");
   const bool small = cells.max_m <= 64, hilo = fv.hilo != nullptr;
   constexpr int BK = XwCfg<64, false>::kBK, SW = 2 * BK;
-  CUtensorMap tm[6];
+  CUtensorMap tmD[2];
   int rc;
-  if ((rc = make_tmap_2d(&tm[0], desc_hi, desc_rows, fv.C, small ? 64 : 128, BK, TMAP_F16, 0, SW))) return rc;
-  if ((rc = make_tmap_2d(&tm[1], desc_lo, desc_rows, fv.C, small ? 64 : 128, BK, TMAP_F16, 0, SW))) return rc;
-  const uint64_t row = hilo ? (uint64_t)hilo_row(fv.C) : (uint64_t)fv.C;
-  const uint64_t dims[4] = {row, (uint64_t)g.w, (uint64_t)g.h, (uint64_t)fv.T};
-  const uint64_t strides[3] = {row * 2, (uint64_t)g.w * row * 2, (uint64_t)fv.P * row * 2};
-  const uint32_t ib = hilo ? 2 * BK : BK, tsw = hilo ? 128 : SW;
-  const uint32_t box0[4] = {ib, XW_BOX, XW_ROWS0, 1}, box1[4] = {ib, XW_BOX, XW_ROWS1, 1};
-  if ((rc = make_tmap_4d(&tm[2], hilo ? fv.hilo : fv.hi, dims, strides, box0, TMAP_F16, tsw))) return rc;
-  if ((rc = make_tmap_4d(&tm[4], hilo ? fv.hilo : fv.hi, dims, strides, box1, TMAP_F16, tsw))) return rc;
-  if (hilo) {
-    tm[3] = tm[2];
-    tm[5] = tm[4];
-    return small ? run_xw_gemm<64, true>(tm, cells, xc, fv.C, st) : run_xw_gemm<128, true>(tm, cells, xc, fv.C, st);
-  }
-  if ((rc = make_tmap_4d(&tm[3], fv.lo, dims, strides, box0, TMAP_F16, tsw))) return rc;
-  if ((rc = make_tmap_4d(&tm[5], fv.lo, dims, strides, box1, TMAP_F16, tsw))) return rc;
-  return small ? run_xw_gemm<64, false>(tm, cells, xc, fv.C, st) : run_xw_gemm<128, false>(tm, cells, xc, fv.C, st);
+  if ((rc = make_tmap_2d(&tmD[0], desc_hi, desc_rows, fv.C, small ? 64 : 128, BK, TMAP_F16, 0, SW))) return rc;
+  if ((rc = make_tmap_2d(&tmD[1], desc_lo, desc_rows, fv.C, small ? 64 : 128, BK, TMAP_F16, 0, SW))) return rc;
+  if (hilo) return small ? run_xw_gemm<64, true>(fv, g, tmD, cells, xc, st) : run_xw_gemm<128, true>(fv, g, tmD, cells, xc, st);
+  return small ? run_xw_gemm<64, false>(fv, g, tmD, cells, xc, st) : run_xw_gemm<128, false>(fv, g, tmD, cells, xc, st);
 }
 
 constexpr int XH_WARPS = 8;
@@ -971,20 +1024,29 @@
   return DINOTRK_OK;
 }
 
-int dinotrk_xw_box_gemm(const dinotrk_features* feat, const dinotrk_geom* g, const void* desc_hi, const void* desc_lo,
-                        int desc_rows, const int* cell_row0, const int* cell_m, const int* cell_frame, const int* box_org,
-                        int n_cells, int max_m, float* xbox, void* stream) {
+int dinotrk_xw_box_gemm_ext(const dinotrk_features* feat, const dinotrk_geom* g, const void* desc_hi, const void* desc_lo,
+                            int desc_rows, const int* cell_row0, const int* cell_m, const int* cell_frame, const int* box_org,
+                            const int* box_ext, int n_cells, int max_m, float* xbox, void* stream) {
   DTK_CHECK_ARG(feat && feat->hi && feat->lo && g && desc_hi && desc_lo && cell_row0 && cell_m && cell_frame && box_org && xbox,
                 "xw_box_gemm: null pointer (the fp16 split of the features is required)");
   DTK_CHECK_ARG(feat->T > 0 && feat->C > 0 && feat->C % 8 == 0 && desc_rows > 0 && n_cells >= 0 && max_m > 0 &&
                 max_m <= XW_MAX_CELL, "xw_box_gemm: bad sizes (C must be a multiple of 8, cells of 1..%d rows)", XW_MAX_CELL);
   DTK_CHECK_ARG(reinterpret_cast<uintptr_t>(box_org) % 8 == 0, "xw_box_gemm: box_org must be 8-byte aligned");
+  DTK_CHECK_ARG(reinterpret_cast<uintptr_t>(box_ext) % 16 == 0, "xw_box_gemm: box_ext must be 16-byte aligned");
   const FeatView fv = make_view(*feat, *g);
   const XwCells cells{cell_row0, cell_row0, cell_m, cell_frame, nullptr, n_cells, max_m};
   XwChunk xc{};
   xc.box_org = reinterpret_cast<int2*>(const_cast<int*>(box_org));
+  xc.box_ext = reinterpret_cast<int4*>(const_cast<int*>(box_ext));
   xc.xbox = xbox;
   return launch_xw_gemm(fv, *g, desc_hi, desc_lo, desc_rows, cells, xc, (cudaStream_t)stream);
 }
 
-}
+int dinotrk_xw_box_gemm(const dinotrk_features* feat, const dinotrk_geom* g, const void* desc_hi, const void* desc_lo,
+                        int desc_rows, const int* cell_row0, const int* cell_m, const int* cell_frame, const int* box_org,
+                        int n_cells, int max_m, float* xbox, void* stream) {
+  return dinotrk_xw_box_gemm_ext(feat, g, desc_hi, desc_lo, desc_rows, cell_row0, cell_m, cell_frame, box_org, nullptr, n_cells,
+                                 max_m, xbox, stream);
+}
+
+}
diff --git a/dino_tracker_b200/csrc/xwin.cuh b/dino_tracker_b200/csrc/xwin.cuh
--- a/dino_tracker_b200/csrc/xwin.cuh
+++ b/dino_tracker_b200/csrc/xwin.cuh
@@ -9,8 +9,6 @@
 constexpr float XW_EPS = 1.1e-3f;
 constexpr int XW_BOX = 21;
 constexpr int XW_SLACK = 3;
-constexpr int XW_ROWS0 = 12, XW_ROWS1 = XW_BOX - XW_ROWS0;
-constexpr int XW_N0 = 256, XW_N1 = 192;
 constexpr int XW_COLS = 448;
 constexpr int XW_MAX_CELL = 128;
 constexpr int XW_MAX_CAND = 4;
@@ -77,6 +75,7 @@
   int* stat;
   int* cell_of;
   int2* box_org;
+  int4* box_ext;
   float* xbox;
   int* slow_cnt;
   int* slow_list;
@@ -90,8 +89,9 @@
     cell_of = ar.take<int>(maps);
     slow_list = ar.take<int>(maps);
     box_org = ar.take<int2>(cells);
+    box_ext = ar.take<int4>(cells);
     xbox = ar.take<float>(maps * XW_COLS);
-    slow_cnt = ar.take<int>((size_t)n_groups + 2);
+    slow_cnt = ar.take<int>((size_t)n_groups + 4);
   }
 };
 
diff --git a/include/dinotrk.h b/include/dinotrk.h
--- a/include/dinotrk.h
+++ b/include/dinotrk.h
@@ -111,6 +111,9 @@
 int dinotrk_xw_box_gemm(const dinotrk_features* feat, const dinotrk_geom* g, const void* desc_hi, const void* desc_lo,
                         int desc_rows, const int* cell_row0, const int* cell_m, const int* cell_frame, const int* box_org,
                         int n_cells, int max_m, float* xbox, void* stream);
+int dinotrk_xw_box_gemm_ext(const dinotrk_features* feat, const dinotrk_geom* g, const void* desc_hi, const void* desc_lo,
+                            int desc_rows, const int* cell_row0, const int* cell_m, const int* cell_frame, const int* box_org,
+                            const int* box_ext, int n_cells, int max_m, float* xbox, void* stream);
 int dinotrk_infer(const dinotrk_features* feat, const dinotrk_geom* g,
                   const dinotrk_head_weights* hw, const float* query_points, int N,
                   float anchor_th, float cos_th, int frame_batch, int start_phase, int stop_after,
```
